# youngers2006/Dreamer

Measured on AMD Instinct MI355X. Metric: imagined latent-steps/sec (B×H) at 64×64 CarRacing, 1/2/4/8 MI355X, higher is better.
Workload: dtype f32; 1 GPU; Dreamer.train_Agent() with AC_epochs=1 (replay sample + warm start S/2 + H-step imagination + actor-critic update), B=256/GPU S=64 H=15 64x64x3, precision=fp32 (north-star batch per GPU); global_batch=256, seq_len=64, horizon=15, parallelism=dp1, precision=fp32

## Files before the change

dreamer_amd/_lib.py:

```python
import ctypes as C
import os

import torch

_HERE = os.path.dirname(os.path.abspath(__file__))
LIB_PATH = os.path.join(_HERE, "libdreamer_hip.so")
if os.environ.get("DREAMER_LIB_VARIANT"):
    LIB_PATH = os.path.join(os.path.dirname(_HERE), "tools", "variants",
                            f"libdreamer_hip_{os.environ['DREAMER_LIB_VARIANT']}.so")

fp = C.c_void_p


class dr_linear(C.Structure):
    _fields_ = [("w", fp), ("b", fp)]


class dr_mlp3(C.Structure):
    _fields_ = [("l0", dr_linear), ("n1", dr_linear), ("l3", dr_linear), ("n4", dr_linear), ("l6", dr_linear)]


DR_DISAG_MAX_MEMBERS = 16


class dr_ensemble(C.Structure):
    _fields_ = [("K", C.c_int), ("W", C.c_int), ("m", dr_mlp3 * DR_DISAG_MAX_MEMBERS)]


class dr_dims(C.Structure):
    _fields_ = [(n, C.c_int) for n in (
        "hidden", "rows", "cols", "action", "img_h", "img_w", "enc_f1", "enc_f2", "enc_hidden",
        "prior_h1", "prior_h2", "rew_h1", "rew_h2", "cont_h1", "cont_h2",
        "actor_h1", "actor_h2", "critic_h1", "critic_h2", "buckets", "dec_f1", "dec_f2", "dec_hidden", "precision", "obs_dim", "enc_depth",
        "launch_form")] + [("fault", fp), ("fault_host", fp)]

DR_MAX_DEPTH = 5


class dr_world_model(C.Structure):
    _fields_ = [("conv", dr_linear * DR_MAX_DEPTH), ("map0", dr_linear), ("map1", dr_linear), ("map3", dr_linear),
                ("w_ih", fp), ("w_hh", fp), ("b_ih", fp), ("b_hh", fp),
                ("prior", dr_mlp3), ("reward", dr_mlp3), ("cont", dr_mlp3), ("buckets_rew", fp)]


class dr_decoder(C.Structure):
    _fields_ = [("up0", dr_linear), ("up1", dr_linear), ("up3", dr_linear), ("convt", dr_linear * DR_MAX_DEPTH)]


class dr_wm_batch(C.Structure):
    _fields_ = [("actions", fp), ("act_sb", C.c_longlong), ("act_st", C.c_longlong), ("rewards", fp),
                ("continues", fp), ("rc_sb", C.c_longlong), ("rc_st", C.c_longlong)]


class dr_wm_loss_cfg(C.Structure):
    _fields_ = [("beta_pred", C.c_float), ("beta_dyn", C.c_float), ("beta_rep", C.c_float)]


class dr_actor(C.Structure):
    _fields_ = [("l0", dr_linear), ("n1", dr_linear), ("l3", dr_linear), ("n4", dr_linear),
                ("mu", dr_linear), ("ls", dr_linear)]


class dr_critic(C.Structure):
    _fields_ = [("net", dr_mlp3), ("buckets", fp)]


class dr_noise(C.Structure):
    _fields_ = [("q", fp), ("eps", fp), ("rng", fp), ("row0", C.c_int), ("stream", C.c_int)]


class dr_frames(C.Structure):
    _fields_ = [("ring", fp), ("ring_cap", C.c_longlong), ("starts", fp), ("obs", fp),
                ("stride_b", C.c_longlong), ("stride_t", C.c_longlong), ("raw255", C.c_int), ("t0", C.c_int)]


class dr_dream_outputs(C.Structure):
    _fields_ = [(n, fp) for n in (
        "R_lambda", "R_mc", "adv", "adv_norm", "weight", "logp", "base_entropy", "saturated",
        "reward_mean", "reward_std", "ret_mean", "ret_std", "logp_mean", "logp_std", "alive", "action_spread",
        "best", "worst", "n_finite")]


_P = C.POINTER
_sz = C.c_size_t
_i = C.c_int
_ll = C.c_longlong
_f = C.c_float
_d = C.c_double

_SIGS = {
    "dr_last_error": (C.c_char_p, []),
    "dr_version": (_i, []),
    "dr_encoder_workspace_bytes": (_sz, [_P(dr_dims), _i]),
    "dr_encoder_features": (_i, [_P(dr_dims), _P(dr_world_model), _P(dr_frames), _i, _i, fp, fp, _sz, fp]),
    "dr_observe_workspace_bytes": (_sz, [_P(dr_dims), _i]),
    "dr_observe_scan": (_i, [_P(dr_dims), _P(dr_world_model), _i, _i, fp, fp, _ll, _ll, fp, fp, dr_noise,
                             fp, fp, fp, fp, _sz, fp]),
    "dr_observe_trace_workspace_bytes": (_sz, [_P(dr_dims), _i, _i]),
    "dr_observe_trace": (_i, [_P(dr_dims), _P(dr_world_model), _i, _i, fp, fp, _ll, _ll, fp, fp, dr_noise,
                              fp, fp, fp, fp, fp, fp, fp, _sz, fp]),
    "dr_latent_stats": (_i, [_i, _i, _i, fp, fp, fp, fp, fp, fp, fp]),
    "dr_replay_returns": (_i, [_i, _i, fp, _ll, fp, _ll, _i, fp, _f, _f, fp, fp, fp, fp]),
    "dr_value_stats": (_i, [_i, _i, _i, _i, fp, _ll, fp, fp, fp, fp, fp, fp]),
    "dr_action_logprob": (_i, [_i, _i, _i, fp, fp, fp, _ll, _ll, fp, fp, fp, fp]),
    "dr_dream_stats": (_i, [_i, _i, _i, _i, fp, fp, fp, fp, fp, fp, fp, _f, _f, fp, _f, _P(dr_dream_outputs), fp]),
    "dr_actor_draws": (_i, [_i, _i, _i, dr_noise, fp, fp]),
    "dr_plan_sample": (_i, [_i, _i, _i, _i, _i, fp, fp, fp, dr_noise, fp, fp]),
    "dr_plan_update": (_i, [_i, _i, _i, _i, _i, fp, fp, fp, _f, _f, _f, _f, _f, fp, fp, fp, fp, fp, fp, fp, fp]),
    "dr_imagine_tape_bytes":(_sz, [_P(dr_dims), _i, _i]),
    "dr_imagine_workspace_bytes": (_sz, [_P(dr_dims), _i, _i]),
    "dr_imagine_fwd": (_i, [_P(dr_dims), _P(dr_world_model), _P(dr_actor), _i, _i, fp, fp, dr_noise, _i,
                            fp, fp, fp, fp, fp, fp, fp, fp, fp, _sz, fp]),
    "dr_imagine_actions_workspace_bytes": (_sz, [_P(dr_dims), _i, _i]),
    "dr_imagine_actions": (_i, [_P(dr_dims), _P(dr_world_model), _i, _i, fp, fp, fp, _ll, _ll, dr_noise,
                                fp, fp, fp, fp, fp, _sz, fp]),
    "dr_imagine_bwd": (_i, [_P(dr_dims), _P(dr_world_model), _P(dr_actor), _i, _i, fp, fp, fp, fp, fp,
                            fp, fp, fp, fp, _P(dr_actor), fp, _sz, fp]),
    "dr_imagine_bwd_prep": (_i, [_P(dr_dims), _P(dr_world_model), _P(dr_actor), _i, _i, fp, fp, fp, fp, _sz, fp]),
    "dr_imagine_bwd_main": (_i, [_P(dr_dims), _P(dr_world_model), _P(dr_actor), _i, _i, fp, fp, fp, fp, fp, _i,
                                 fp, _P(dr_actor), fp, _sz, fp]),
    "dr_step_workspace_bytes": (_sz, [_P(dr_dims), _i]),
    "dr_imagine_step": (_i, [_P(dr_dims), _P(dr_world_model), _i, fp, fp, fp, dr_noise, fp, fp, fp, fp,
                             fp, _sz, fp]),
    "dr_actor_act_workspace_bytes": (_sz, [_P(dr_dims), _i]),
    "dr_actor_act": (_i, [_P(dr_dims), _P(dr_actor), _i, fp, fp, dr_noise, _i, fp, fp, fp, fp, _sz, fp]),
    "dr_act_step_workspace_bytes": (_sz, [_P(dr_dims)]),
    "dr_act_step": (_i, [_P(dr_dims), _P(dr_world_model), _P(dr_actor), fp, _i, fp, fp, fp, dr_noise, _i,
                         fp, fp, fp, fp, fp, fp, fp, fp, _sz, fp]),
    "dr_act_batch_workspace_bytes": (_sz, [_P(dr_dims), _i]),
    "dr_act_batch": (_i, [_P(dr_dims), _P(dr_world_model), _P(dr_actor), _i, fp, fp, fp, fp, fp, dr_noise, _i,
                          fp, fp, fp, fp, fp, fp, fp, fp, _sz, fp]),
    "dr_act_vec_workspace_bytes": (_sz, [_P(dr_dims), _i]),
    "dr_act_vec": (_i, [_P(dr_dims), _P(dr_world_model), _P(dr_actor), _i, fp, fp, fp, fp, fp, dr_noise, _i,
                        fp, fp, fp, fp, fp, fp, fp, fp, _sz, fp]),
    "dr_gru_cell": (_i, [_P(dr_dims), _P(dr_world_model), _i, fp, fp, fp, fp, fp, _sz, fp]),
    "dr_categorical_sample": (_i, [_i, _i, _i, fp, dr_noise, fp, fp, fp, fp]),
    "dr_mlp3_fwd": (_i, [_P(dr_mlp3), _i, _i, fp, _ll, _i, fp, _ll, _i, _i, _i, fp, _ll, fp, _sz, fp]),
    "dr_bucket_value": (_i, [_i, _i, fp, fp, fp, fp]),
    "dr_critic_tape_bytes": (_sz, [_P(dr_dims), _i]),
    "dr_critic_workspace_bytes": (_sz, [_P(dr_dims), _i, _i]),
    "dr_critic_fwd": (_i, [_P(dr_dims), _P(dr_critic), _i, fp, _ll, fp, _ll, fp, fp, fp, fp, _sz, fp]),
    "dr_lambda_returns": (_i, [_i, _i, fp, fp, fp, _f, _f, fp, fp]),
    "dr_update_S": (_i, [_i, fp, fp, fp, fp, _sz, fp]),
    "dr_actor_loss_grad": (_i, [_i, _i, _i, fp, fp, fp, fp, fp, fp, _f, _f, fp, fp, fp, fp]),
    "dr_critic_loss_bwd": (_i, [_P(dr_dims), _P(dr_critic), _i, _i, fp, fp, fp, fp, _f, fp, _P(dr_critic),
                                fp, _sz, fp]),
    "dr_sqnorm": (_i, [_ll, fp, fp, fp]),
    "dr_sqnorm_multi": (_i, [_ll, fp, fp, fp, fp]),
    "dr_clip_stats": (_i, [_ll, fp, _ll, fp, _i, fp, fp, fp, fp, fp]),
    "dr_adamw": (_i, [_ll, fp, fp, fp, fp, fp, _f, _d, _d, _d, _d, _d, fp, fp, fp, fp]),
    "dr_ema": (_i, [_ll, fp, fp, _f, _f, fp, fp]),
    "dr_ac_optimiser_step": (_i, [_ll, fp, fp, fp, fp, fp, fp, _d, _d, _d, _d, _d,
                                  _ll, fp, fp, fp, fp, fp, fp, _d, _d, _d, _d, _d,
                                  _f, fp, _f, _f, _i, fp, fp, fp, fp, fp]),
    "dr_nonfinite": (_i, [_ll, fp, fp, fp]),
    "dr_replay_gather": (_i, [_ll, _i, _i, _i, _i, fp, fp, fp, fp, fp, fp, fp, fp, fp, fp]),
    "dr_replay_sample_workspace_bytes": (_sz, [_ll]),
    "dr_replay_sample": (_i, [_ll, _ll, _ll, _i, _i, fp, _d, fp, fp, _i, fp, fp, fp, _sz, fp]),
    "dr_replay_probabilities": (_i, [_ll, _ll, _ll, _i, fp, _d, fp, fp, _sz, fp]),
    "dr_replay_priority_update": (_i, [_ll, _i, fp, fp, _d, _d, _d, _d, _d, fp, fp, fp]),
    "dr_wm_window_scores": (_i, [_P(dr_dims), _i, _i, dr_wm_loss_cfg, fp, _sz, fp, fp]),
    "dr_disag_workspace_bytes": (_sz, [_i, _i, _i, _i, _i, _i]),
    "dr_disag_fwd": (_i, [_P(dr_ensemble), _i, _i, _i, fp, _ll, fp, fp, fp, _i, _i, _ll, _ll, _f, _f, fp, _sz, fp]),
    "dr_disag_train_grads": (_i, [_P(dr_ensemble), _i, _i, _i, fp, _ll, fp, _ll, _P(dr_ensemble), fp, fp, _sz, fp]),
    "dr_knn_workspace_bytes": (_sz, [_i, _i, _i, _i]),
    "dr_knn": (_i, [_i, _i, _i, fp, _ll, fp, _i, fp, _ll, fp, fp, fp, fp, _sz, fp]),
    "dr_state_entropy_fwd": (_i, [_i, _i, _i, fp, _ll, fp, _i, fp, _ll, fp, fp, fp, fp, fp, _i, _i, _ll, _ll, _f, _f,
                                  fp, _sz, fp]),
    "dr_rng_advance": (_i, [fp, C.c_ulonglong, fp]),
    "dr_persistent_kernels": (_i, [_P(dr_dims), _i, _i, _i]),
    "dr_stream_create_cumask": (_i, [_i, _P(C.c_uint), _P(fp)]),
    "dr_stream_destroy": (_i, [fp]),
    "dr_device_cus": (_i, [_P(_i)]),
    "dr_host_device_ptr": (_i, [fp, _P(fp)]),
    "dr_wm_train_workspace_bytes": (_sz, [_P(dr_dims), _i, _i]),
    "dr_decoder_workspace_bytes": (_sz, [_P(dr_dims), _i]),
    "dr_decoder_fwd": (_i, [_P(dr_dims), _P(dr_decoder), _i, fp, _ll, fp, _ll, fp, fp, _sz, fp]),
    "dr_frame_metrics": (_i, [_P(dr_dims), _i, _i, fp, _P(dr_frames), fp, fp, fp, fp]),
    "dr_frame_ssim": (_i, [_P(dr_dims), _i, _i, fp, _P(dr_frames), fp, fp, fp]),
    "dr_ensemble_metrics": (_i, [_P(dr_dims), _i, _i, _i, fp, _P(dr_frames), fp, fp, fp, fp, fp, fp]),
    "dr_occlude_workspace_bytes": (_sz, [_P(dr_dims), _i]),
    "dr_occlude_frames": (_i, [_P(dr_dims), _P(dr_frames), _i, _i, _i, fp, _i, fp, fp, fp, _sz, fp]),
    "dr_saliency_scores": (_i, [_i, _i, _i, _i, _i, fp, fp, fp, fp, fp, fp, fp, fp, fp, fp]),
    "dr_saliency_map": (_i, [_P(dr_dims), _i, _i, fp, fp, _P(dr_frames), _i, fp, fp, fp]),
    "dr_saliency_draws": (_i, [_i, _i, dr_noise, fp, fp]),
    "dr_wm_train_phase": (_i, [_P(dr_dims), _P(dr_world_model), _P(dr_decoder), _i, _i, _P(dr_frames),
                               _P(dr_wm_batch), dr_noise, dr_wm_loss_cfg, _i, fp, _i, fp, fp, _P(dr_world_model),
                               _P(dr_decoder), fp, fp, fp, fp, _sz, fp]),
    "dr_wm_train_grads": (_i, [_P(dr_dims), _P(dr_world_model), _P(dr_decoder), _i, _i, _P(dr_frames),
                               _P(dr_wm_batch), dr_noise, dr_wm_loss_cfg, fp, fp, _P(dr_world_model),
                               _P(dr_decoder), fp, fp, fp, fp, _sz, fp]),
}

EXPORTED = sorted(_SIGS)

_lib = None
_load_error = None


def load():
    global _lib, _load_error
    if _lib is not None:
        return _lib
    if not os.path.exists(LIB_PATH):
        _load_error = f"{LIB_PATH} not built (run: python -m dreamer_amd.build)"
        raise RuntimeError("dreamer_amd: HIP library missing: " + _load_error)
    lib = C.CDLL(LIB_PATH)
    for name, (res, args) in _SIGS.items():
        fn = getattr(lib, name)
        fn.restype = res
        fn.argtypes = args
    _lib = lib
    return lib


DR_E_INVALID, DR_E_HIP, DR_E_WORKSPACE, DR_E_UNSUPPORTED = 1001, 1002, 1003, 1004
DR_ACT_MAX_ENVS = 16
DR_ACT_VEC_MAX_OBS = 1023
DR_PLAN_MAX_CANDIDATES = 2048
DR_ENSEMBLE_MAX_SAMPLES = 64
DR_DREAM_STATS_MAX_DREAMS = 64
DR_DREAM_STATS_MAX_LDS_FLOATS = 15360
DR_KNN_MAX_K = 32
DR_PLAN_MAX_ELEMS = 1024
DR_SALIENCY_MAX_CELLS = 1024
DR_SALIENCY_MAX_RADIUS = 15


class HipError(RuntimeError):

    def __init__(self, name, code, msg):
        super().__init__(f"{name} failed ({code}): {msg}")
        self.code = code


def call(name, *args):
    lib = load()
    rc = getattr(lib, name)(*args)
    if rc != 0:
        msg = lib.dr_last_error().decode(errors="replace")
        raise HipError(name, rc, msg)


def query(name, *args):
    return getattr(load(), name)(*args)


def ptr(t):
    if t is None:
        return None
    if not t.is_cuda:
        raise RuntimeError("dreamer_amd: tensors must live on the GPU (this framework is MI355X-only)")
    return t.data_ptr()


def stream_ptr(device=None):
    return torch.cuda.current_stream(device).cuda_stream


def require_gpu(t):
    if not (isinstance(t, torch.Tensor) and t.is_cuda):
        raise RuntimeError("dreamer_amd: hot-path ops run only on the GPU (MI355X); "
                           "move the model and tensors to 'cuda'")
```

dreamer_amd/csrc/conv.h:

```cpp
#pragma once
#include "common.h"

extern thread_local const char* dr_conv_form_last;
const char* dr_conv_form(const char* fmt, ...);
#define DR_CONV_NOTE(...)                                  \
  do {                                                     \
    static const char* form_ = dr_conv_form(__VA_ARGS__);  \
    dr_conv_form_last = form_;                             \
  } while (0)

int op_conv_nhwc(int n, int cin, int ih, int iw, int cout, const float* in, const float* wr, const float* bias,
                 float* out, int out_nchw, hipStream_t s);
enum { CONV_EPI_FWD = 0, CONV_EPI_DSILU = 1 };
int op_conv_nhwc_ex(int n, int cin, int ih, int iw, int cout, const float* in, const float* wr, const float* bias,
                    float* out, int out_nchw, float* pre, int epi, hipStream_t s, float* csum = nullptr);
int op_frames_nhwc4(int n, int nb, int h, int w, const dr_frames* src, float* out, hipStream_t s, float pad = 0.0f);
int op_conv1_frames(int n, int nb, int ih, int iw, int cout, const dr_frames* src, const float* wr, const float* bias,
                    float* out, hipStream_t s);
int op_conv_repack_pad(int cout, int cin, int cin_pad, const float* w, float* wr, hipStream_t s);

int op_conv_repack_split3(int cout, int cin, const float* w, void* wr, hipStream_t s);
bool op_conv_split3_supported(int n, int cin, int ih, int iw, int cout);
int op_enc12_s1_bf16(int n, int nb, int h, int w, int c1, int c2, const dr_frames* src, const float* w1,
                     const float* b1, const float* w2, const float* b2, void* wr1, void* wr2, void* out,
                     hipStream_t s, int prepacked = 0);
int op_conv_s1_bf16(int n, int cin, int ih, int iw, int cout, const void* in, const void* wr, const float* bias,
                    void* out, int out_nchw, hipStream_t s);
bool op_conv_glds_bf16_supported(int n, int cin, int ih, int iw, int cout);
int op_conv_glds_s3(int n, int cin, int ih, int iw, int cout, const float* in, const void* wr, const float* bias,
                    float* out, int out_nchw, float* pre, int epi, hipStream_t s);
size_t op_gemm_nt_glds_part_floats(int M, int N, int K);
int op_gemm_nt_glds_bf16(int M, int N, int K, const void* X, int ldx, const void* W, int ldw, const float* bias,
                         float* Y, int ldy, float* part, size_t part_floats, hipStream_t s);
int op_conv_glds_bf16(int n, int cin, int ih, int iw, int cout, const void* in, const void* wr, const float* bias,
                      void* out, int out_nchw, hipStream_t s);
int op_conv_split3(int n, int cin, int ih, int iw, int cout, const float* in, const void* wr, const float* bias,
                   float* out, int out_nchw, hipStream_t s);
int op_conv_split3_ex(int n, int cin, int ih, int iw, int cout, const float* in, const void* wr, const float* bias,
                      float* out, int out_nchw, float* pre, int epi, hipStream_t s, int terms = 3);

size_t op_nt_split3_ws_bytes(int N, int K);
int op_nt_repack_split3(int N, int K, const float* W, int ldw, void* wr, hipStream_t s);
bool op_gemm_nt_split3_supported(int M, int N, int K, const float* A, int lda, const float* A2, int lda2, int ksA,
                                 int ldy);
int op_gemm_nt_split3(int M, int N, int K, const float* A, int lda, const float* A2, int lda2, int ksA, const void* wr,
                      const float* bias, int act, float* Y, int ldy, hipStream_t s);
size_t op_gemm_nt_split3_part_floats(int M, int N);
int op_gemm_nt_split3_sk(int M, int N, int K, const float* A, int lda, const float* A2, int lda2, int ksA,
                         const void* wr, const float* bias, int act, float* Y, int ldy, float* part,
                         size_t part_floats, hipStream_t s, int splits_fixed = 0);
int op_gemm_nt_split3_ex(int M, int N, int K, const float* A, int lda, const float* A2, int lda2, int ksA,
                         const void* wr, const float* bias, int act, float* Y, int ldy, int accumulate, float* Y2,
                         int ldy2, int nsplitY, float* part, size_t part_floats, hipStream_t s, int splits_fixed = 0);

int op_conv_repack_bf16(int cout, int cin, int cin_pad, const float* w, void* wr, hipStream_t s);
int op_to_bf16_2d(int rows, int cols, const float* x, long long ld, void* y, hipStream_t s);
int op_conv1_bf16(int n, int nb, int h, int w, int cout, const dr_frames* src, const void* wr, const float* bias,
                  void* out, hipStream_t s);
bool op_enc12_split3_ok(int n, int h, int w, int c1, int c2, const dr_frames* src);
int op_enc12_split3(int n, int nb, int h, int w, int c1, int c2, const dr_frames* src, const float* w1,
                    const float* b1, const float* w2, const float* b2, void* wr1, void* wr2, float* out,
                    hipStream_t s, int prepacked = 0);
int op_enc12_split3_ex(int n, int nb, int h, int w, int c1, int c2, const dr_frames* src, const float* w1,
                       const float* b1, const float* w2, const float* b2, void* wr1, void* wr2, float* out,
                       float* pre0, float* a0, float* pre1, hipStream_t s, int terms = 3, int prepacked = 0);
enum { RJ_CONV1 = 0, RJ_CONV = 1, RJ_NT = 2, RJ_BF16 = 3 };
struct RepackJob {
  int kind, a, b, c;
  const float* w;
  void* out;
  long long ld;
  long long total;
};
#define DR_RJ_MAX 6
RepackJob rj_conv1(int cout, const float* w, void* wr);
RepackJob rj_conv(int cout, int cin, const float* w, void* wr);
RepackJob rj_nt(int N, int K, const float* W, int ldw, void* wr);
RepackJob rj_bf16(int rows, int cols, const float* x, long long ld, void* y);
int op_repack_multi(const RepackJob* jobs, int n, hipStream_t s);
int op_enc12_bf16(int n, int nb, int h, int w, int c1, int c2, const dr_frames* src, const void* wr1, const float* b1,
                  const void* wr2, const float* b2, void* out, hipStream_t s);
int op_conv_bf16(int n, int cin, int ih, int iw, int cout, const void* in, const void* wr, const float* bias,
                 void* out, int out_nchw, hipStream_t s);
int op_gemm_nt_bf16(int M, int N, int K, const void* X, int ldx, const void* W, const float* bias, float* Y, int ldy,
                    hipStream_t s);

enum { CT_EPI_BIAS = 0, CT_EPI_DSILU = 1, CT_EPI_TANH_MSE = 2 };
struct ConvTArgs {
  int n, cin, h, w, cout;
  const float* in;
  int silu_in;
  const float* wq;
  const float* bias;
  float* out;
  float* out2;
  int silu_out;
  int ldc;
  const float* pre;
  const float* target;
  int tstride;
  const float* coef;
  float* part;
  float* bpart;
};
int op_convT_repack(int cin, int cout, const float* wt, float* wq, hipStream_t s);
int op_convT_nhwc(int epi, const ConvTArgs& a, hipStream_t s);
int op_convT_mse_parts(int h, int w);
int op_convT_out3_repack(int cin, const float* wt, float* wq, hipStream_t s);
int op_convT_out3(const ConvTArgs& a, hipStream_t s);
int op_convT_repack_split3(int cin, int cout, const float* wt, void* wr, hipStream_t s);
bool op_convT_split3_supported(int n, int cin, int h, int w, int cout, int terms = 3);
bool op_convT_cls_supported(int n, int cin, int h, int w, int cout);
int op_convT_split3(int epi, const ConvTArgs& a, const void* wr, hipStream_t s, int terms = 3);
bool op_convT_glds_s3_supported(const ConvTArgs& a, int epi);
int op_convT_glds_s3(int epi, const ConvTArgs& a, const void* wr, hipStream_t s);

size_t op_conv_wgrad_ws_floats(int n, int h, int w, int ca, int cb);
int op_wgrad_reduce(int ca, int cb, int cbo, int nsplit, const float* part, float* dw, float scale, int accumulate,
                    hipStream_t s);
bool op_wgrad_split3_supported(int n, int h, int w, int ca, int cb, int terms = 3);
size_t op_wgrad_split3_ws_floats(int n, int h, int w, int ca, int cb);
int op_wgrad_split3(int n, int h, int w, int ca, int cb, const float* lo, int lda, const float* hi, int ldb,
                    float* dw, int cbo, float scale, int accumulate, float* ws, size_t ws_floats, hipStream_t s,
                    int terms = 3);
int op_conv_wgrad(int n, int h, int w, int ca, int cb, const float* lo, int lda, int lo_silu, const float* hi, int ldb,
                  float* dw, int cbo, float scale, int accumulate, float* ws, size_t ws_floats, hipStream_t s,
                  float* bias_out = nullptr);
size_t op_chan_sum_ws_floats(long long rows, int C);
int op_chan_sum(long long rows, int C, const float* X, int ldx, float* out, int accumulate, float* ws, size_t ws_floats,
                hipStream_t s);
int op_chan_sum_final(int nb, int C, const float* part, float* out, int accumulate, hipStream_t s);

size_t op_gemm_tn_split3_ws_bytes(int M, int N, int K);
bool op_gemm_tn_split3_supported(int M, int N, int K);
int op_gemm_tn_split3(int M, int N, int K, const float* G, long long ldg, const float* X, long long ldx,
                      const float* X2, long long ldx2, int nsplitB, float* Y, long long ldy, int accumulate, void* ws,
                      size_t ws_bytes, hipStream_t s, int terms = 3);
struct TnProblem {
  int M, N, K;
  const float* G;
  long long ldg;
  const float* X;
  long long ldx;
  const float* X2;
  long long ldx2;
  int nsplitB;
  float* Y;
  long long ldy;
  int accumulate;
};
size_t op_gemm_tn_split3_multi_ws_bytes(const TnProblem* p, int n);
int op_gemm_tn_split3_multi(const TnProblem* p, int n, void* ws, size_t ws_bytes, hipStream_t s, int terms);
```

dreamer_amd/csrc/conv_hook.hip:

```cpp
#include <cstdarg>
#include <cstdio>
#include <cstring>

#include "conv.h"

thread_local const char* dr_conv_form_last = nullptr;

const char* dr_conv_form(const char* fmt, ...) {
  char buf[96];
  va_list ap;
  va_start(ap, fmt);
  vsnprintf(buf, sizeof buf, fmt, ap);
  va_end(ap);
  return strdup(buf);
}

enum {
  CV_OP, CV_N, CV_CA, CV_CB, CV_H, CV_W, CV_EPI, CV_NCHW, CV_TERMS, CV_LDA, CV_LDB, CV_LDC, CV_TSTRIDE, CV_CBO,
  CV_SILU_IN, CV_SILU_OUT, CV_LO_SILU, CV_FLAGS, CV_ACC, CV_WS_FLOATS, CV_CIN_RAW, CV_COUNT
};
enum {
  COP_CONV, COP_CONV_S3, COP_CONVT, COP_CONVT_S3, COP_CONVT_OUT3, COP_WGRAD, COP_WGRAD_S3, COP_CHAN_SUM,
  COP_CHAN_SUM_FINAL
};
enum {
  CF_BIAS = 1, CF_PRE = 2, CF_CSUM = 4, CF_OUT2 = 8, CF_TARGET = 16, CF_COEF = 32, CF_PART = 64, CF_BPART = 128,
  CF_BIAS_OUT = 256, CF_NO_REPACK = 512, CF_WS = 1024
};
enum {
  CP_IN, CP_W, CP_WR, CP_BIAS, CP_OUT, CP_PRE, CP_CSUM, CP_OUT2, CP_TARGET, CP_COEF, CP_PART, CP_BPART, CP_WS, CP_HI,
  CP_BIAS_OUT, CP_COUNT
};
enum { CN_SCALE, CN_PAD, CN_COUNT };

extern "C" int dr_internal_conv_run(const int* v, const double* num, void* const* ptrs, void* stream,
                                    long long* ws_need, char* form, int form_cap, char* msg, int msg_cap) {
  hipStream_t s = (hipStream_t)stream;
  if (form && form_cap > 0) form[0] = 0;
  if (msg && msg_cap > 0) msg[0] = 0;
  if (!v) return DR_E_INVALID;
  const int op = v[CV_OP], n = v[CV_N], ca = v[CV_CA], cb = v[CV_CB], h = v[CV_H], w = v[CV_W], fl = v[CV_FLAGS];
  long long need = 0;
  if (op == COP_WGRAD) need = (long long)op_conv_wgrad_ws_floats(n, h, w, ca, cb);
  else if (op == COP_WGRAD_S3) need = (long long)op_wgrad_split3_ws_floats(n, h, w, ca, cb);
  else if (op == COP_CHAN_SUM) need = (long long)op_chan_sum_ws_floats(n, ca);
  if (ws_need) *ws_need = need;
  if (!ptrs) return DR_OK;
  auto P = [&](int slot, int flag) { return !flag || (fl & flag) ? (float*)ptrs[slot] : nullptr; };
  const float* in = P(CP_IN, 0);
  const float* wraw = P(CP_W, 0);
  float* wr = P(CP_WR, 0);
  float* out = P(CP_OUT, 0);
  const bool repack = !(fl & CF_NO_REPACK);
  const float scale = num ? (float)num[CN_SCALE] : 1.0f;
  const size_t ws_floats = (size_t)v[CV_WS_FLOATS];
  dr_conv_form_last = nullptr;
  int rc = DR_OK;
  ConvTArgs a = {};
  a.n = n; a.cin = ca; a.h = h; a.w = w; a.cout = cb;
  a.in = in; a.silu_in = v[CV_SILU_IN]; a.wq = wr; a.bias = P(CP_BIAS, CF_BIAS);
  a.out = out; a.out2 = P(CP_OUT2, CF_OUT2); a.silu_out = v[CV_SILU_OUT]; a.ldc = v[CV_LDC];
  a.pre = P(CP_PRE, CF_PRE); a.target = P(CP_TARGET, CF_TARGET); a.tstride = v[CV_TSTRIDE];
  a.coef = P(CP_COEF, CF_COEF); a.part = P(CP_PART, CF_PART); a.bpart = P(CP_BPART, CF_BPART);
  switch (op) {
    case COP_CONV:
      if (repack) rc = op_conv_repack_pad(cb, v[CV_CIN_RAW] > 0 ? v[CV_CIN_RAW] : ca, ca, wraw, wr, s);
      if (rc == DR_OK)
        rc = op_conv_nhwc_ex(n, ca, h, w, cb, in, wr, P(CP_BIAS, CF_BIAS), out, v[CV_NCHW], P(CP_PRE, CF_PRE), v[CV_EPI],
                             s, P(CP_CSUM, CF_CSUM));
      break;
    case COP_CONV_S3:
      if (repack) rc = op_conv_repack_split3(cb, ca, wraw, wr, s);
      if (rc == DR_OK)
        rc = op_conv_split3_ex(n, ca, h, w, cb, in, wr, P(CP_BIAS, CF_BIAS), out, v[CV_NCHW], P(CP_PRE, CF_PRE),
                               v[CV_EPI], s, v[CV_TERMS]);
      break;
    case COP_CONVT:
      if (repack) rc = op_convT_repack(ca, cb, wraw, wr, s);
      if (rc == DR_OK) rc = op_convT_nhwc(v[CV_EPI], a, s);
      break;
    case COP_CONVT_S3:
      if (repack) rc = op_convT_repack_split3(ca, cb, wraw, wr, s);
      if (rc == DR_OK) rc = op_convT_split3(v[CV_EPI], a, wr, s, v[CV_TERMS]);
      break;
    case COP_CONVT_OUT3:
      if (repack) rc = op_convT_out3_repack(ca, wraw, wr, s);
      if (rc == DR_OK) rc = op_convT_out3(a, s);
      break;
    case COP_WGRAD:
      rc = op_conv_wgrad(n, h, w, ca, cb, in, v[CV_LDA], v[CV_LO_SILU], P(CP_HI, 0), v[CV_LDB], out, v[CV_CBO], scale,
                         v[CV_ACC], P(CP_WS, CF_WS), ws_floats, s, P(CP_BIAS_OUT, CF_BIAS_OUT));
      break;
    case COP_WGRAD_S3:
      rc = op_wgrad_split3(n, h, w, ca, cb, in, v[CV_LDA], P(CP_HI, 0), v[CV_LDB], out, v[CV_CBO], scale, v[CV_ACC],
                           P(CP_WS, CF_WS), ws_floats, s, v[CV_TERMS]);
      break;
    case COP_CHAN_SUM:
      rc = op_chan_sum(n, ca, in, v[CV_LDA], out, v[CV_ACC], P(CP_WS, CF_WS), ws_floats, s);
      break;
    case COP_CHAN_SUM_FINAL:
      rc = op_chan_sum_final(n, ca, in, out, v[CV_ACC], s);
      break;
    default:
      dr_set_error("dr_internal_conv_run: unknown op %d", op);
      rc = DR_E_INVALID;
  }
  if (form && form_cap > 0 && dr_conv_form_last) snprintf(form, form_cap, "%s", dr_conv_form_last);
  if (rc != DR_OK && msg && msg_cap > 0) snprintf(msg, msg_cap, "%s", dr_last_error());
  return rc;
}
```

dreamer_amd/csrc/conv_split.hip:

```cpp
#include "conv.h"

#include <algorithm>
#include <climits>
#include <type_traits>

namespace {
typedef unsigned short u16;
typedef __bf16 bf16x8 __attribute__((ext_vector_type(8)));
typedef unsigned u32x4 __attribute__((ext_vector_type(4)));
typedef unsigned u32x2 __attribute__((ext_vector_type(2)));

__device__ __forceinline__ f32x4 mfma_b16(u32x4 a, u32x4 b, f32x4 c) {
  return __builtin_amdgcn_mfma_f32_16x16x32_bf16(__builtin_bit_cast(bf16x8, a), __builtin_bit_cast(bf16x8, b), c, 0, 0,
                                                  0);
}
__device__ __forceinline__ unsigned b16bits(__bf16 v) { return (unsigned)__builtin_bit_cast(u16, v); }
__device__ __forceinline__ void split3(float x, unsigned& h, unsigned& m, unsigned& l) {
  const __bf16 bh = (__bf16)x;
  const float r1 = x - (float)bh;
  const __bf16 bm = (__bf16)r1;
  const float r2 = r1 - (float)bm;
  h = b16bits(bh);
  m = b16bits(bm);
  l = b16bits((__bf16)r2);
// ... 1821 lines not shown
  const int n = (int)(i / (KC * 32)), k = (int)(i - (long long)n * KC * 32);
  unsigned hh = 0, mm = 0, ll = 0;
  if (n < N && k < K) split3(W[(long long)n * ldw + k], hh, mm, ll);
  const long long plane = (long long)Np * 32;
  const long long base = ((long long)(k >> 5) * 3 * Np + n) * 32 + (k & 31);
  wr[base] = (u16)hh;
  wr[base + plane] = (u16)mm;
  wr[base + 2 * plane] = (u16)ll;
}
__global__ void k_nt_repack_split3(int N, int K, int Np, const float* __restrict__ W, int ldw, u16* __restrict__ wr) {
  const long long i = (long long)blockIdx.x * blockDim.x + threadIdx.x;
  if (i >= (long long)((K + 31) / 32) * 32 * Np) return;
  nt_repack_split3_elem(i, N, K, Np, W, ldw, wr);
}

struct RepackBatch {
  RepackJob j[DR_RJ_MAX];
  int blk0[DR_RJ_MAX + 1];
  int n;
};
__global__ __launch_bounds__(256) void k_repack_multi(RepackBatch b) {
  __shared__ __attribute__((aligned(16))) RepackJob J;
  int z = 0;
#pragma unroll
  for (int i = 1; i < DR_RJ_MAX; ++i)
    if ((int)blockIdx.x >= b.blk0[i]) z = i;
  dr_stage_args(b.j[z], J, threadIdx.x);
  const long long i = (long long)(blockIdx.x - b.blk0[z]) * 256 + threadIdx.x;
  if (i >= J.total) return;
  u16* out = static_cast<u16*>(J.out);
  switch (J.kind) {
    case RJ_CONV1: conv1_repack_split3_elem((int)i, J.a, J.w, out); break;
    case RJ_CONV: conv_repack_split3_elem((int)i, J.a, J.b, J.w, out); break;
    case RJ_NT: nt_repack_split3_elem(i, J.a, J.b, J.c, J.w, J.ld, out); break;
    default: {
      const int rr = (int)(i / J.b), cc = (int)(i - (long long)rr * J.b);
      out[i] = __builtin_bit_cast(u16, (__bf16)J.w[(long long)rr * J.ld + cc]);
    }
  }
}

RepackJob rj_conv1(int cout, const float* w, void* wr) { return {RJ_CONV1, cout, 0, 0, w, wr, 0, (long long)cout * 64}; }
RepackJob rj_conv(int cout, int cin, const float* w, void* wr) {
  return {RJ_CONV, cout, cin, 0, w, wr, 0, (long long)cout * 16 * cin};
}
RepackJob rj_nt(int N, int K, const float* W, int ldw, void* wr) {
  const int Np = (N + 127) / 128 * 128;
  return {RJ_NT, N, K, Np, W, wr, ldw, (long long)((K + 31) / 32) * 32 * Np};
}
RepackJob rj_bf16(int rows, int cols, const float* x, long long ld, void* y) {
  return {RJ_BF16, rows, cols, 0, x, y, ld, (long long)rows * cols};
}

int op_repack_multi(const RepackJob* jobs, int n, hipStream_t s) {
  if (n < 0 || n > DR_RJ_MAX) {
    dr_set_error("repack_multi: %d jobs (at most %d)", n, DR_RJ_MAX);
    return DR_E_INVALID;
  }
  if (n == 0) return DR_OK;
  RepackBatch b = {};
  int tot = 0;
  for (int i = 0; i < DR_RJ_MAX; ++i) {
    b.blk0[i] = tot;
    if (i < n) {
      b.j[i] = jobs[i];
      tot += (int)((jobs[i].total + 255) / 256);
    }
  }
  b.blk0[DR_RJ_MAX] = tot;
  b.n = n;
  hipLaunchKernelGGL(k_repack_multi, dim3((unsigned)tot), dim3(256), 0, s, b);
  return dr_check_launch("repack_multi");
}

static int s3_np(int N) { return (N + 127) / 128 * 128; }
size_t op_nt_split3_ws_bytes(int N, int K) {
  return (size_t)((K + 31) / 32) * 32 * 3 * s3_np(N) * sizeof(u16);
}
int op_nt_repack_split3(int N, int K, const float* W, int ldw, void* wr, hipStream_t s) {
  const int Np = s3_np(N);
  const long long total = (long long)((K + 31) / 32) * 32 * Np;
  hipLaunchKernelGGL(k_nt_repack_split3, dim3((unsigned)((total + 255) / 256)), dim3(256), 0, s, N, K, Np, W, ldw,
                     (u16*)wr);
  return dr_check_launch("nt_repack_split3");
}
bool op_gemm_nt_split3_supported(int M, int N, int K, const float* A, int lda, const float* A2, int lda2, int ksA,
                                 int ldy) {
  const bool seg = ksA < K;
  return M > 0 && N > 0 && N % 4 == 0 && ldy % 4 == 0 && K % 4 == 0 && lda % 4 == 0 && !((uintptr_t)A & 15) &&
         (!seg || (ksA % 4 == 0 && lda2 % 4 == 0 && A2 && !((uintptr_t)A2 & 15))) &&
         (long long)M * lda < (1LL << 31) && (!seg || (long long)M * lda2 < (1LL << 31));
}
size_t op_gemm_nt_split3_part_floats(int M, int N) { return (size_t)DR_S3_SPLITS * M * N; }

int op_gemm_nt_split3(int M, int N, int K, const float* A, int lda, const float* A2, int lda2, int ksA, const void* wr,
                      const float* bias, int act, float* Y, int ldy, hipStream_t s) {
  return op_gemm_nt_split3_sk(M, N, K, A, lda, A2, lda2, ksA, wr, bias, act, Y, ldy, nullptr, 0, s);
}

int op_gemm_nt_split3_sk(int M, int N, int K, const float* A, int lda, const float* A2, int lda2, int ksA,
                         const void* wr, const float* bias, int act, float* Y, int ldy, float* part,
                         size_t part_floats, hipStream_t s, int splits_fixed) {
  return op_gemm_nt_split3_ex(M, N, K, A, lda, A2, lda2, ksA, wr, bias, act, Y, ldy, 0, nullptr, 0, INT_MAX, part,
                              part_floats, s, splits_fixed);
}

int op_gemm_nt_split3_ex(int M, int N, int K, const float* A, int lda, const float* A2, int lda2, int ksA,
                         const void* wr, const float* bias, int act, float* Y, int ldy, int accumulate, float* Y2,
                         int ldy2, int nsplitY, float* part, size_t part_floats, hipStream_t s, int splits_fixed) {
  const bool y2 = nsplitY < N;
  if (!op_gemm_nt_split3_supported(M, N, K, A, lda, A2, lda2, ksA, ldy) || ((uintptr_t)Y & 15) ||
      (bias && ((uintptr_t)bias & 15)) || ((uintptr_t)part & 15) || splits_fixed < 0 ||
      splits_fixed > DR_S3_SPLITS || (splits_fixed > 1 && (!part || (size_t)splits_fixed * M * N > part_floats)) ||
      (y2 && (!Y2 || ((uintptr_t)Y2 & 15) || ldy2 % 4 || nsplitY % 4 || nsplitY < 0))) {
    dr_set_error("gemm_nt_split3: unsupported problem (M=%d N=%d K=%d)", M, N, K);
    return DR_E_INVALID;
  }
  GemmS3 g = {M, N, K, ksA < K ? ksA : K, lda, lda2, ldy, act, s3_np(N), A, A2, (const u16*)wr, bias, Y, 1, part,
              accumulate ? 1 : 0, ldy2, y2 ? nsplitY : INT_MAX, 0, Y2};
  auto tl = [&](int bm, int bn) { return ((M + bm - 1) / bm) * ((N + bn - 1) / bn); };
  auto waves = [&](int bm, int bn) { return (long long)tl(bm, bn) * (bm / 32); };
  const int nch = (K + 31) / 32;
  auto splits_for = [&](int bm, int bn) {
    if (splits_fixed > 0) return splits_fixed;
    int sp = 1;
    while (part && sp < DR_S3_SPLITS && waves(bm, bn) * sp < 2048 && nch / (2 * sp) >= 8 &&
           (size_t)(2 * sp) * M * N <= part_floats)
      sp *= 2;
    return sp;
  };
  const int shapes[5][2] = {{256, 128}, {256, 64}, {128, 128}, {128, 64}, {64, 64}};
  int pick = 4;
  for (int c = 0; c < 5; ++c) {
    if (waves(shapes[c][0], shapes[c][1]) * splits_for(shapes[c][0], shapes[c][1]) >= 2048) {
      pick = c;
      break;
    }
  }
  g.splits = splits_for(shapes[pick][0], shapes[pick][1]);
  const unsigned gy = (unsigned)g.splits;
  switch (pick) {
    case 0: hipLaunchKernelGGL((k_gemm_split3<256, 128>), dim3(dr_xcd_grid(tl(256, 128)), gy), dim3(512), 0, s, g); break;
    case 1: hipLaunchKernelGGL((k_gemm_split3<256, 64>), dim3(dr_xcd_grid(tl(256, 64)), gy), dim3(512), 0, s, g); break;
    case 2: hipLaunchKernelGGL((k_gemm_split3<128, 128>), dim3(dr_xcd_grid(tl(128, 128)), gy), dim3(256), 0, s, g); break;
    case 3: hipLaunchKernelGGL((k_gemm_split3<128, 64>), dim3(dr_xcd_grid(tl(128, 64)), gy), dim3(256), 0, s, g); break;
    default: hipLaunchKernelGGL((k_gemm_split3<64, 64>), dim3(dr_xcd_grid(tl(64, 64)), gy), dim3(128), 0, s, g); break;
  }
  DR_TRY(dr_check_launch("gemm_nt_split3"));
  if (g.splits > 1) {
    hipLaunchKernelGGL(k_s3_finish, dim3((unsigned)(((long long)M * (N / 4) + 255) / 256)), dim3(256), 0, s, g);
    DR_TRY(dr_check_launch("s3_finish"));
  }
  return DR_OK;
}

static int s3_pad(int n) { return (n + 127) / 128 * 128; }

struct KnRepack {
  int K, N, P, nsplit;
  const float* X;
  const float* X2;
  long long ldx, ldx2;
  u16* wr;
  long long pad_;
};

template <int TERMS>
__device__ __forceinline__ void kn_repack_body(int K, int N, int P, const float* __restrict__ X, long long ldx,
                                               const float* __restrict__ X2, long long ldx2, int nsplit,
                                               u16* __restrict__ wr) {
  const int n = blockIdx.x * 256 + threadIdx.x, kc = blockIdx.y;
  if (n >= P) return;
  const bool seg2 = n >= nsplit;
  const float* src = seg2 ? X2 : X;
  const long long ld = seg2 ? ldx2 : ldx;
  const int nn = seg2 ? n - nsplit : n;
  float v[32];
  const bool nok = n < N;
  const float* col = src + (nok ? nn : 0);
#pragma unroll
  for (int k = 0; k < 32; ++k) {
    const int kk = 32 * kc + k;
    const bool ok = nok && kk < K;
    const float t = col[ok ? (long long)kk * ld : 0LL];
    v[k] = ok ? t : 0.f;
  }
  u32x4* o = reinterpret_cast<u32x4*>(wr + (((long long)kc * 3) * P + n) * 32);
  if constexpr (TERMS == 1) {
#pragma unroll
    for (int u = 0; u < 4; ++u) {
      u32x4 h;
#pragma unroll
      for (int e = 0; e < 4; ++e) h[e] = pack_bf16x2(v[8 * u + 2 * e], v[8 * u + 2 * e + 1]);
      o[u] = h;
    }
    return;
  }
  u32x4 h[4], m[4], l[4];
#pragma unroll
  for (int u = 0; u < 4; ++u)
#pragma unroll
    for (int e = 0; e < 4; ++e) {
      unsigned hh, mm, ll;
      split3_pair(v[8 * u + 2 * e], v[8 * u + 2 * e + 1], hh, mm, ll);
      h[u][e] = hh;
      m[u][e] = mm;
      l[u][e] = ll;
    }
  const long long pl = (long long)P * 32 / 8;
#pragma unroll
  for (int u = 0; u < 4; ++u) {
    o[u] = h[u];
    o[pl + u] = m[u];
    o[2 * pl + u] = l[u];
  }
}

struct GemmPP {
  int M, N, K, Mp, Np, splits, accumulate, tiles;
  long long ldy;
  const u16* wa;
  const u16* wb;
  float* Y;
  float* part;
  long long pad_;
};

#define DR_TN_MAX 4
struct TnBatch {
  KnRepack r[2 * DR_TN_MAX];
  GemmPP g[DR_TN_MAX];
  int blk0[DR_TN_MAX + 1];
  int fin0[DR_TN_MAX + 1];
  int n, nrep, pad_[2];
};

template <int TERMS>
__global__ __launch_bounds__(256) void k_kn_repack_multi(TnBatch b) {
  __shared__ __attribute__((aligned(16))) KnRepack s;
  dr_stage_args(b.r[blockIdx.z], s, threadIdx.x);
  const int P = dr_uni(s.P), K = dr_uni(s.K);
  if ((int)blockIdx.x * 256 >= P || (int)blockIdx.y * 32 >= K) return;
  kn_repack_body<TERMS>(K, dr_uni(s.N), P, dr_uni(s.X), s.ldx, dr_uni(s.X2), s.ldx2, dr_uni(s.nsplit), dr_uni(s.wr));
}

__device__ __forceinline__ int tn_find(const int* blk0, int flat) {
  int z = 0;
#pragma unroll
  for (int i = 1; i < DR_TN_MAX; ++i)
    if (flat >= blk0[i]) z = i;
  return z;
}

template <int BM, int BN, int TERMS = 3>
__global__ __launch_bounds__(BM * 2) void k_gemm_pp_multi(TnBatch b) {
  constexpr int NT = BM * 2;
  constexpr int WTN = BN / 2, FM = 4, FN = WTN / 16;
  constexpr int AU = TERMS * BM * 4, BU = TERMS * BN * 4;
  constexpr int APT = (AU + NT - 1) / NT, BPT = (BU + NT - 1) / NT;
  static_assert(FN >= 1 && BM % 64 == 0 && (TERMS == 1 || TERMS == 3), "gemm_pp tile");
  __shared__ __attribute__((aligned(16))) u32x4 As[2][TERMS][BM][4];
  __shared__ __attribute__((aligned(16))) u32x4 Bs[2][TERMS][BN][4];
  __shared__ __attribute__((aligned(16))) GemmPP s_g;
  const int flat = dr_xcd_tile(blockIdx.x, b.blk0[DR_TN_MAX]);
  if (flat < 0) return;
  const int z = tn_find(b.blk0, flat);
  dr_stage_args(b.g[z], s_g, threadIdx.x);
  const int M = dr_uni(s_g.M), N = dr_uni(s_g.N), Mp = dr_uni(s_g.Mp), Np = dr_uni(s_g.Np);
  const int tiles = dr_uni(s_g.tiles), splits = dr_uni(s_g.splits);
  const int local = flat - b.blk0[z];
  const int split = local / tiles, lt = local - split * tiles;
  const int tiles_n = (N + BN - 1) / BN;
  const int m0 = (lt / tiles_n) * BM, n0 = (lt % tiles_n) * BN;
  const DR_GLOBAL u16* wa = dr_g(dr_uni(s_g.wa));
  const DR_GLOBAL u16* wb = dr_g(dr_uni(s_g.wb));
  const int tid = threadIdx.x, wave = tid >> 6, lane = tid & 63, r = lane & 15, q = lane >> 4;
  const int NCH = (dr_uni(s_g.K) + 31) / 32;
  const int per = (NCH + splits - 1) / splits;
  const int c0 = min(NCH, split * per), c1 = min(NCH, c0 + per);
  u32x4 ra0[APT], ra1[APT], rb0[BPT], rb1[BPT];
  auto load = [&](int c, auto slot) __attribute__((always_inline)) {
    u32x4* ra = decltype(slot)::value == 0 ? ra0 : ra1;
    u32x4* rb = decltype(slot)::value == 0 ? rb0 : rb1;
#pragma unroll
    for (int j = 0; j < APT; ++j) {
      const int e = tid + NT * j;
      if (AU % NT == 0 || e < AU) {
        const int pl = e / (BM * 4), rm = e - pl * BM * 4, row = rm >> 2, u = rm & 3;
        ra[j] = *reinterpret_cast<const DR_GLOBAL u32x4*>(wa + (((long long)c * 3 + pl) * Mp + m0 + row) * 32 + 8 * u);
      }
    }
#pragma unroll
    for (int j = 0; j < BPT; ++j) {
      const int e = tid + NT * j;
      if (BU % NT == 0 || e < BU) {
        const int pl = e / (BN * 4), rm = e - pl * BN * 4, row = rm >> 2, u = rm & 3;
        rb[j] = *reinterpret_cast<const DR_GLOBAL u32x4*>(wb + (((long long)c * 3 + pl) * Np + n0 + row) * 32 + 8 * u);
      }
    }
  };
  auto store = [&](auto slot, int buf) __attribute__((always_inline)) {
    const u32x4* ra = decltype(slot)::value == 0 ? ra0 : ra1;
    const u32x4* rb = decltype(slot)::value == 0 ? rb0 : rb1;
#pragma unroll
    for (int j = 0; j < APT; ++j) {
      const int e = tid + NT * j;
// ... 211 lines not shown
```

dreamer_amd/csrc/engine.hip:

```cpp
#include "engine_util.h"
#include "scan.h"
#include "dream.h"
#include "bptt.h"


static bool s3_first_layer(const dr_dims* d, int M, int N, const float* h, long long ldh, const float* z,
                           long long ldz) {
  return d->precision != DR_PREC_BF16 && M >= 1024 && ldh < INT_MAX && ldz < INT_MAX &&
         op_gemm_nt_split3_supported(M, N, d->hidden + latent(d), h, (int)ldh, z, (int)ldz, d->hidden, N);
}

struct EncWs {
  float *x0, *a[DR_MAX_DEPTH], *wr[DR_MAX_DEPTH], *sk;
  long long sk_n;
  void* wproj;
  void* s3proj;
  float* s3part;
  size_t s3part_n;
};

static void enc_carve(Carve& c, const dr_dims* d, int n, EncWs& w) {
  memset(&w, 0, sizeof(w));
  if (d->obs_dim > 0) {
    const int F = enc_feat_dim(d);
// ... 415 lines not shown
  w.wst = c.f((long long)2 * A * d->actor_h2);
  w.bst = c.f((long long)2 * A);
  w.idx[0] = c.i(2 * Bl * d->rows);
  w.idx[1] = c.i(2 * Bl * d->rows);
  w.tl6p = c.f((long long)L * d->prior_h2);
  w.tl3p = c.f((long long)d->prior_h2 * d->prior_h1);
  w.tl0p = c.f((long long)d->prior_h1 * Hd);
  w.twhh = c.f((long long)3 * Hd * Hd);
  w.thead = c.f((long long)2 * A * d->actor_h2);
  w.tl3a = c.f((long long)d->actor_h2 * d->actor_h1);
  w.tl0a = c.f((long long)d->actor_h1 * (Hd + L));
  w.gH = c.f(B1 * Hd);
  w.gZ = c.f(B1 * L);
  w.gA = c.f(BH * A);
  w.glog = c.f(Bl * L);
  w.gx2 = c.f(Bl * d->prior_h2);
  w.gp2 = c.f(Bl * d->prior_h2);
  w.gx1 = c.f(Bl * d->prior_h1);
  w.gp1 = c.f(Bl * d->prior_h1);
  w.ggi = c.f(Bl * 3 * Hd);
  w.ggh = c.f(Bl * 3 * Hd);
  w.ggi16 = (unsigned short*)c.raw(sizeof(unsigned short) * Bl * 3 * Hd);
  w.ggh16 = (unsigned short*)c.raw(sizeof(unsigned short) * Bl * 3 * Hd);
  w.gheads = c.f(BH * 2 * A);
  w.gx2a = c.f(Bl * d->actor_h2);
  w.gpre2a = c.f(BH * d->actor_h2);
  w.gy2a = c.f(BH * d->actor_h2);
  w.xh2a = c.f(BH * d->actor_h2);
  w.gx1a = c.f(Bl * d->actor_h1);
  w.gpre1a = c.f(BH * d->actor_h1);
  w.gpre1a16 = (unsigned short*)c.raw(sizeof(unsigned short) * BH * d->actor_h1);
  w.gy1a = c.f(BH * d->actor_h1);
  w.xh1a = c.f(BH * d->actor_h1);
  w.hcat = c.f(BH * Hd);
  w.zcat = c.f(BH * L);
  w.sk_n = splitk_floats(d->actor_h1, Hd + L) + splitk_floats(d->actor_h2, d->actor_h1) +
           2 * splitk_floats(A, d->actor_h2);
  w.sk = c.f(w.sk_n);
  const int BHi = (int)BH;
  w.tn_bytes = op_gemm_tn_split3_ws_bytes(d->actor_h1, Hd + L, BHi) +
               op_gemm_tn_split3_ws_bytes(d->actor_h2, d->actor_h1, BHi) +
               2 * op_gemm_tn_split3_ws_bytes(A, d->actor_h2, BHi);
  w.tn = c.raw(w.tn_bytes);
  w.pd = c.raw(op_pdream_ws_bytes(d, B, H));
  w.pb = c.raw(op_pbptt_ws_bytes(d, B, H));
}

extern "C" size_t dr_imagine_workspace_bytes(const dr_dims* d, int B, int H) {
  Carve c(nullptr);
  ImWs w;
  imws_carve(c, d, B, H, w);
  return c.off;
}

static int imagine_heads(const dr_dims* d, const dr_world_model* wm, int B, int H, const float* latents,
                         const float* hiddens, float* rewards, float* continues, ImWs& w, hipStream_t s,
                         bool keep0 = false);

static int imagine_launch_form(const dr_dims* d, const dr_world_model* wm, const dr_actor* ac, int B, int H,
                               const dr_noise& noise, const dr_noise& nq, int deterministic, float* latents,
                               float* hiddens, float* actions, float* mus, float* sigmas, const Tape& tp, ImWs& w,
                               bool split_gru, bool zg, hipStream_t s) {
  const int L = latent(d), Hd = d->hidden, A = d->action, a1 = d->actor_h1, a2 = d->actor_h2;
  const long long ldH = (long long)(H + 1) * Hd, ldL = (long long)(H + 1) * L, ldA = (long long)H * A;
  const long long lda1 = (long long)H * a1, lda2 = (long long)H * a2;
  const bool planes = split_gru && H > 1 && Hd % 8 == 0;
  const bool a16 = planes && d->precision == DR_PREC_BF16;
  if (planes) {
    DR_TRY(split_planes(d->prior_h1, Hd, wm->prior.l0.w, Hd, w.s3p0, s));
    if (zg) DR_TRY(split_planes(a1, Hd, ac->l0.w, Hd + L, w.s3a0, s));
    DR_TRY(split_planes(3 * Hd, Hd, wm->w_hh, Hd, w.s3whh, s));
  }

  {
    DR_TRY(run(G_NT, AM_PLAIN, lin2(B, a1, hiddens, ldH, Hd, latents, ldL, L, ac->l0.w, ac->l0.b, tp.pre1a, lda1), s));
    GemmArgs g = lin_ln(B, a2, a1, tp.pre1a, lda1, ac->n1, ac->l3.w, ac->l3.b, tp.pre2a, lda2);
    g.a_out = tp.x1a; g.ld_aout = lda1;
    DR_TRY(run(G_NT, AM_LNSILU, g, s));
  }
  DR_TRY(stack_heads(ac, A, a2, w.wst, w.bst, s));
  {
    GemmArgs h = lin_ln(B, 2 * A, a2, tp.pre2a, lda2, ac->n4, w.wst, w.bst, nullptr, 0);
    h.a_out = tp.x2a; h.ld_aout = lda2;
    with_actor_head(h, A, noise, 0, deterministic, actions, ldA, mus, ldA, sigmas, ldA, tp.eps, tp.ls_raw, ldA);
    DR_TRY(run(G_NT, AM_LNSILU, h, s));
  }
  for (int t = 0; t < H; ++t) {
    const long long hb = (long long)Hd * B * t;
    float* h_t = hiddens + (long long)t * Hd;
    float* h_n = hiddens + (long long)(t + 1) * Hd;
    float* z_t = latents + (long long)t * L;
    float* z_n = latents + (long long)(t + 1) * L;
    unsigned short* h_n16 = a16 ? w.hid16 + (long long)(t + 1) * Hd : nullptr;
    DR_TRY(gru_onehot(d, wm, B, w.idx[t & 1], actions + (long long)t * A, ldA, h_t, ldH, h_n, ldH, w.wt,
                      tp.r + hb, tp.u + hb, tp.n + hb, tp.ghn + hb, s, z_t, ldL, w.gh, split_gru && t > 0, h_n16));
    float* p1 = tp.pre1p + (long long)t * B * d->prior_h1;
    float* p2 = tp.pre2p + (long long)t * B * d->prior_h2;
    {
      const bool more = t + 1 < H;
      GemmArgs p[3];
      int np = 0;
      p[np] = lin(B, d->prior_h1, Hd, h_n, ldH, wm->prior.l0.w, Hd, wm->prior.l0.b, p1, d->prior_h1);
      if (planes) wplanes(p[np], w.s3p0);
      ++np;
      if (more && zg) {
        p[np] = lin(B, a1, Hd, h_n, ldH, ac->l0.w, Hd + L, ac->l0.b, w.hpart, a1);
        if (planes) wplanes(p[np], w.s3a0);
        ++np;
      }
      if (more && split_gru) {
        p[np] = lin(B, 3 * Hd, Hd, h_n, ldH, wm->w_hh, Hd, wm->b_hh, w.gh, 3 * Hd);
        if (planes) wplanes(p[np], w.s3whh);
        ++np;
      }
      for (int i = 0; i < np; ++i) {
        if (!planes) p[i].bf16 = 0;
        p[i].A16 = h_n16;
      }
      DR_TRY(gemm_launch(G_NT, AM_PLAIN, p, np, s));
    }
    DR_TRY(run(G_NT, AM_LNSILU, lin_ln(B, d->prior_h2, d->prior_h1, p1, d->prior_h1, wm->prior.n1, wm->prior.l3.w,
                                       wm->prior.l3.b, p2, d->prior_h2), s));
    GemmArgs g = lin_ln(B, L, d->prior_h2, p2, d->prior_h2, wm->prior.n4, wm->prior.l6.w, wm->prior.l6.b, nullptr, 0);
    with_sampler(g, d, nq, t, z_n, ldL, w.idx[(t + 1) & 1], tp.soft + (long long)t * B * L, L);
    DR_TRY(run(G_NT, AM_LNSILU, g, s));
    if (t + 1 < H) {
      const long long o1 = (long long)(t + 1) * a1, o2 = (long long)(t + 1) * a2, o = (long long)(t + 1) * A;
      if (zg) {
        int* ix = w.idx[(t + 1) & 1];
        DR_TRY(op_zgather_add(B, a1, d->rows, d->cols, ix, onehot_vals(ix, B, d->rows), z_n, ldL,
                              w.tl0f + (long long)Hd * a1, a1, w.hpart, a1, tp.pre1a + o1, lda1, s));
      } else {
        DR_TRY(run(G_NT, AM_PLAIN, lin2(B, a1, h_n, ldH, Hd, z_n, ldL, L, ac->l0.w, ac->l0.b, tp.pre1a + o1, lda1), s));
      }
      GemmArgs g3 = lin_ln(B, a2, a1, tp.pre1a + o1, lda1, ac->n1, ac->l3.w, ac->l3.b, tp.pre2a + o2, lda2);
      g3.a_out = tp.x1a + o1;
      g3.ld_aout = lda1;
      DR_TRY(run(G_NT, AM_LNSILU, g3, s));
      GemmArgs hd = lin_ln(B, 2 * A, a2, tp.pre2a + o2, lda2, ac->n4, w.wst, w.bst, nullptr, 0);
      hd.a_out = tp.x2a + o2;
      hd.ld_aout = lda2;
      with_actor_head(hd, A, noise, t + 1, deterministic, actions + o, ldA, mus + o, ldA, sigmas + o, ldA,
                      tp.eps + (long long)(t + 1) * B * A, tp.ls_raw + o, ldA);
      DR_TRY(run(G_NT, AM_LNSILU, hd, s));
    }
  }
  return DR_OK;
}

extern "C" int dr_imagine_fwd(const dr_dims* d, const dr_world_model* wm, const dr_actor* ac, int B, int H,
                              const float* z0, const float* h0, dr_noise noise, int deterministic, float* latents,
                              float* hiddens, float* actions, float* rewards, float* continues, float* mus,
                              float* sigmas, void* tape, void* ws, size_t ws_bytes, hipStream_t s) {
  DR_REQUIRE(d && wm && ac && z0 && h0 && latents && hiddens && actions && rewards && continues && mus && sigmas &&
                 tape && B > 0 && H > 0,
             "null argument or empty batch");
  DR_TRY(dims_envelope(__func__, d, ENV_GRU | ENV_SAMPLER | ENV_ACTOR));
  GemmBf16Scope bf16_scope(d->precision == DR_PREC_BF16);
  Carve c(ws);
  ImWs w;
  imws_carve(c, d, B, H, w);
  WS_CHECK(c, ws_bytes);
  Carve ct(tape);
  Tape tp;
  tape_carve(ct, d, B, H, tp);
  const int L = latent(d), Hd = d->hidden, A = d->action, a1 = d->actor_h1, a2 = d->actor_h2;
  const long long ldH = (long long)(H + 1) * Hd, ldL = (long long)(H + 1) * L, ldA = (long long)H * A;
  const long long lda1 = (long long)H * a1, lda2 = (long long)H * a2;
  {
    const Copy2dJob cj[2] = {{latents, ldL, z0, L, L, B}, {hiddens, ldH, h0, Hd, Hd, B}};
    DR_TRY(op_copy2d_multi(cj, 2, s));
  }
  dr_noise nq = noise;
  nq.stream += 65536;
  const bool split_gru = B >= 128;
  const bool zg = d->rows <= 32 && a1 % 4 == 0;
  {
    TransposeJob tj[2] = {{3 * Hd, L + A, 3 * Hd, wm->w_ih, w.wt}, {a1, Hd + L, a1, ac->l0.w, w.tl0f}};
    DR_TRY(op_transpose_multi(tj, zg ? 2 : 1, s));
  }
  DR_TRY(op_onehot_index(B, d->rows, d->cols, latents, ldL, w.idx[0], onehot_vals(w.idx[0], B, d->rows), s));

  bool unrolled = false;
  if (zg && op_pdream_supported(d, B, H, A)) {
    const PDreamTape pt = {tp.eps, tp.ls_raw, tp.pre1a, tp.x1a, tp.pre2a, tp.x2a, tp.r, tp.u, tp.n, tp.ghn,
                           tp.pre1p, tp.pre2p, tp.soft};
    const int rc = op_pdream(d, wm, ac, B, H, w.wt, w.tl0f + (long long)Hd * a1, w.idx[0], noise, nq, deterministic,
                             latents, hiddens, actions, mus, sigmas, pt, w.pd, s);
    if (rc != DR_E_UNSUPPORTED && rc != DR_OK) return rc;
    unrolled = rc == DR_OK;
  }
  if (!unrolled) DR_TRY(imagine_launch_form(d, wm, ac, B, H, noise, nq, deterministic, latents, hiddens, actions, mus,
                                            sigmas, tp, w, split_gru, zg, s));
  return imagine_heads(d, wm, B, H, latents, hiddens, rewards, continues, w, s);
}

static int imagine_heads(const dr_dims* d, const dr_world_model* wm, int B, int H, const float* latents,
                         const float* hiddens, float* rewards, float* continues, ImWs& w, hipStream_t s, bool keep0) {
  const int L = latent(d), Hd = d->hidden;
  {
    const int M1 = B * (H + 1);
    GemmArgs p[2];
    if (s3_first_layer(d, M1, d->rew_h1, hiddens, Hd, latents, L) &&
        s3_first_layer(d, M1, d->cont_h1, hiddens, Hd, latents, L)) {
      DR_TRY(op_nt_repack_split3(d->rew_h1, Hd + L, wm->reward.l0.w, Hd + L, w.s3r, s));
      DR_TRY(op_nt_repack_split3(d->cont_h1, Hd + L, wm->cont.l0.w, Hd + L, w.s3c, s));
      DR_TRY(op_gemm_nt_split3_sk(M1, d->rew_h1, Hd + L, hiddens, Hd, latents, L, Hd, w.s3r, wm->reward.l0.b, 0,
                                  w.p1r, d->rew_h1, w.s3part, w.s3part_n, s));
      DR_TRY(op_gemm_nt_split3_sk(M1, d->cont_h1, Hd + L, hiddens, Hd, latents, L, Hd, w.s3c, wm->cont.l0.b, 0,
                                  w.p1c, d->cont_h1, w.s3part, w.s3part_n, s));
    } else {
      p[0] = lin2(M1, d->rew_h1, hiddens, Hd, Hd, latents, L, L, wm->reward.l0.w, wm->reward.l0.b, w.p1r, d->rew_h1);
      p[1] = lin2(M1, d->cont_h1, hiddens, Hd, Hd, latents, L, L, wm->cont.l0.w, wm->cont.l0.b, w.p1c, d->cont_h1);
      DR_TRY(gemm_launch(G_NT, AM_PLAIN, p, 2, s));
    }
    p[0] = lin_ln(M1, d->buckets, d->rew_h2, w.p2r, d->rew_h2, wm->reward.n4, wm->reward.l6.w, wm->reward.l6.b, w.rlog,
                  d->buckets);
    p[1] = lin_ln(M1, 1, d->cont_h2, w.p2c, d->cont_h2, wm->cont.n4, wm->cont.l6.w, wm->cont.l6.b, w.clog, 1);
    p[1].act = 2;
    Mlp2Args m2[2];
    {
      const float* x1[2] = {w.p1r, w.p1c};
      const dr_mlp3* hm[2] = {&wm->reward, &wm->cont};
      const int k1[2] = {d->rew_h1, d->cont_h1}, k2[2] = {d->rew_h2, d->cont_h2};
      for (int i = 0; i < 2; ++i) {
        memset(&m2[i], 0, sizeof(Mlp2Args));
        m2[i].M = M1; m2[i].K1 = k1[i]; m2[i].K2 = k2[i];
        m2[i].X = x1[i]; m2[i].ldx = k1[i];
        m2[i].ln1_g = hm[i]->n1.w; m2[i].ln1_b = hm[i]->n1.b;
        m2[i].W3 = hm[i]->l3.w; m2[i].b3 = hm[i]->l3.b;
        m2[i].ln4_g = hm[i]->n4.w; m2[i].ln4_b = hm[i]->n4.b;
        m2[i].e = p[i];
        m2[i].e.A = nullptr;
      }
    }
    if (mlp2_ok(m2[0]) && mlp2_ok(m2[1])) {
      DR_TRY(mlp2_launch(m2, 2, s));
    } else {
      GemmArgs q[2];
      q[0] = lin_ln(M1, d->rew_h2, d->rew_h1, w.p1r, d->rew_h1, wm->reward.n1, wm->reward.l3.w, wm->reward.l3.b, w.p2r,
                    d->rew_h2);
      q[1] = lin_ln(M1, d->cont_h2, d->cont_h1, w.p1c, d->cont_h1, wm->cont.n1, wm->cont.l3.w, wm->cont.l3.b, w.p2c,
                    d->cont_h2);
      DR_TRY(gemm_launch(G_NT, AM_LNSILU, q, 2, s));
      DR_TRY(gemm_launch(G_NT, AM_LNSILU, p, 2, s));
    }
    DR_TRY(op_bucket_value(M1, d->buckets, w.rlog, d->buckets, wm->buckets_rew, w.rval, 1, s));
    const int k0 = keep0 ? 0 : 1, Ho = H + 1 - k0;
    const Copy2dJob cj[2] = {{rewards, Ho, w.rval + k0, H + 1, Ho, B}, {continues, Ho, w.clog + k0, H + 1, Ho, B}};
    DR_TRY(op_copy2d_multi(cj, 2, s));
  }
  return DR_OK;
}

struct ImActWs {
  ImWs w;
  float *p1, *p2;
};
static void imact_carve(Carve& c, const dr_dims* d, int B, int H, ImActWs& a) {
  const long long Bl = B, B1 = (long long)B * (H + 1);
  const int L = latent(d), Hd = d->hidden, A = d->action;
  ImWs& w = a.w;
  memset(&w, 0, sizeof(w));
  w.gh = c.f(Bl * 3 * Hd);
  w.wt = c.f((long long)(L + A) * 3 * Hd);
  w.hid16 = (unsigned short*)c.raw(sizeof(unsigned short) * B1 * Hd);
  w.s3p0 = c.raw(op_nt_split3_ws_bytes(d->prior_h1, Hd));
  w.s3whh = c.raw(op_nt_split3_ws_bytes(3 * Hd, Hd));
  w.idx[0] = c.i(2 * Bl * d->rows);
  w.idx[1] = c.i(2 * Bl * d->rows);
  a.p1 = c.f(Bl * d->prior_h1);
  a.p2 = c.f(Bl * d->prior_h2);
  w.p1r = c.f(B1 * d->rew_h1);
  w.p1c = c.f(B1 * d->cont_h1);
  w.p2r = c.f(B1 * d->rew_h2);
  w.p2c = c.f(B1 * d->cont_h2);
  w.rlog = c.f(B1 * d->buckets);
  w.clog = c.f(B1);
  w.rval = c.f(B1);
  w.s3r = c.raw(op_nt_split3_ws_bytes(d->rew_h1, Hd + L));
  w.s3c = c.raw(op_nt_split3_ws_bytes(d->cont_h1, Hd + L));
  w.s3part_n = op_gemm_nt_split3_part_floats((int)B1, std::max(d->rew_h1, d->cont_h1));
  w.s3part = c.f((long long)w.s3part_n);
}

extern "C" size_t dr_imagine_actions_workspace_bytes(const dr_dims* d, int B, int H) {
  if (!d || B <= 0 || H <= 0) return 0;
  Carve c(nullptr);
  ImActWs a;
  imact_carve(c, d, B, H, a);
  return c.off;
}

extern "C" int dr_imagine_actions(const dr_dims* d, const dr_world_model* wm, int B, int H, const float* z0,
                                  const float* h0, const float* actions, long long act_sb, long long act_st,
                                  dr_noise noise, float* latents, float* hiddens, float* rewards, float* continues,
                                  void* ws, size_t ws_bytes, hipStream_t s) {
  DR_REQUIRE(d && wm && z0 && h0 && actions && latents && hiddens && rewards && continues && ws && B > 0 && H > 0,
             "null argument or empty batch");
  DR_REQUIRE(wm->w_ih && wm->w_hh && wm->b_ih && wm->b_hh, "GRU weights required");
  DR_TRY(dims_envelope(__func__, d, ENV_GRU | ENV_SAMPLER));
  GemmBf16Scope bf16_scope(d->precision == DR_PREC_BF16);
  Carve c(ws);
  ImActWs a;
  imact_carve(c, d, B, H, a);
  WS_CHECK(c, ws_bytes);
  ImWs& w = a.w;
  const int L = latent(d), Hd = d->hidden, A = d->action;
  const long long ldH = (long long)(H + 1) * Hd, ldL = (long long)(H + 1) * L;
  {
    const Copy2dJob cj[2] = {{latents, ldL, z0, L, L, B}, {hiddens, ldH, h0, Hd, Hd, B}};
    DR_TRY(op_copy2d_multi(cj, 2, s));
  }
  const bool split_gru = B >= 128;
  const bool planes = split_gru && H > 1 && Hd % 8 == 0;
  const bool a16 = planes && d->precision == DR_PREC_BF16;
  DR_TRY(op_transpose(3 * Hd, L + A, wm->w_ih, w.wt, s));
  DR_TRY(op_onehot_index(B, d->rows, d->cols, latents, ldL, w.idx[0], onehot_vals(w.idx[0], B, d->rows), s));
  if (planes) {
    DR_TRY(split_planes(d->prior_h1, Hd, wm->prior.l0.w, Hd, w.s3p0, s));
    DR_TRY(split_planes(3 * Hd, Hd, wm->w_hh, Hd, w.s3whh, s));
  }
  for (int t = 0; t < H; ++t) {
    float* h_t = hiddens + (long long)t * Hd;
    float* h_n = hiddens + (long long)(t + 1) * Hd;
    float* z_t = latents + (long long)t * L;
    float* z_n = latents + (long long)(t + 1) * L;
    unsigned short* h_n16 = a16 ? w.hid16 + (long long)(t + 1) * Hd : nullptr;
    DR_TRY(gru_onehot(d, wm, B, w.idx[t & 1], actions + (long long)t * act_st, act_sb, h_t, ldH, h_n, ldH, w.wt,
                      nullptr, nullptr, nullptr, nullptr, s, z_t, ldL, w.gh, split_gru && t > 0, h_n16));
    {
      GemmArgs p[2];
      int np = 0;
      p[np] = lin(B, d->prior_h1, Hd, h_n, ldH, wm->prior.l0.w, Hd, wm->prior.l0.b, a.p1, d->prior_h1);
      if (planes) wplanes(p[np], w.s3p0);
      ++np;
      if (t + 1 < H && split_gru) {
        p[np] = lin(B, 3 * Hd, Hd, h_n, ldH, wm->w_hh, Hd, wm->b_hh, w.gh, 3 * Hd);
        if (planes) wplanes(p[np], w.s3whh);
        ++np;
      }
      for (int i = 0; i < np; ++i) {
        if (!planes) p[i].bf16 = 0;
        p[i].A16 = h_n16;
      }
      DR_TRY(gemm_launch(G_NT, AM_PLAIN, p, np, s));
    }
    DR_TRY(run(G_NT, AM_LNSILU, lin_ln(B, d->prior_h2, d->prior_h1, a.p1, d->prior_h1, wm->prior.n1, wm->prior.l3.w,
                                       wm->prior.l3.b, a.p2, d->prior_h2), s));
    GemmArgs g = lin_ln(B, L, d->prior_h2, a.p2, d->prior_h2, wm->prior.n4, wm->prior.l6.w, wm->prior.l6.b, nullptr, 0);
    with_sampler(g, d, noise, t, z_n, ldL, w.idx[(t + 1) & 1], nullptr, 0);
    DR_TRY(run(G_NT, AM_LNSILU, g, s));
  }
  return imagine_heads(d, wm, B, H, latents, hiddens, rewards, continues, w, s);
}

static int imagine_bwd_impl(const dr_dims* d, const dr_world_model* wm, const dr_actor* ac, int B, int H,
                            const float* latents, const float* hiddens, const float* actions,
                            const float* g_mus, const float* g_sigmas,
                            const float* g_actions, const float* g_latents, const float* g_hiddens,
                            const void* tape, const dr_actor* gr, void* ws, size_t ws_bytes, hipStream_t s,
                            bool do_prep, bool do_main);

extern "C" int dr_imagine_bwd(const dr_dims* d, const dr_world_model* wm, const dr_actor* ac, int B, int H,
                              const float* latents, const float* hiddens, const float* actions,
                              const float* g_mus, const float* g_sigmas,
                              const float* g_actions, const float* g_latents, const float* g_hiddens,
                              const void* tape, const dr_actor* gr, void* ws, size_t ws_bytes, hipStream_t s) {
// ... 70 lines not shown
      DR_TRY(split_planes(Hd, 3 * Hd, w.twhh, 3 * Hd, w.s3twhh, s));
      if (d->actor_h1 % 8 == 0) DR_TRY(split_planes(Hd + L, d->actor_h1, w.tl0a, d->actor_h1, w.s3tl0a, s));
    }
  }
  }
  const bool planes = B >= 128 && (3 * Hd) % 8 == 0;
  if (!do_main) return DR_OK;

  bool looped = false;
  if (op_pbptt_supported(d, B, H, A)) {
    const PBpttIO io = {w.tl6p, w.tl3p, w.tl0p, w.wt, w.twhh, w.thead, w.tl3a, w.tl0a,
                        tp.soft, tp.pre2p, tp.pre1p, tp.r, tp.u, tp.n, tp.ghn, tp.pre2a, tp.pre1a, tp.ls_raw, tp.eps,
                        hiddens, actions, g_mus, g_sigmas, w.gH, w.gZ, w.gA,
                        w.gheads, w.gpre2a, w.gy2a, w.xh2a, w.gpre1a, w.gy1a, w.xh1a};
    const int rc = op_pbptt(d, wm, ac, B, H, io, w.pb, s);
    if (rc != DR_E_UNSUPPORTED && rc != DR_OK) return rc;
    looped = rc == DR_OK;
  }
  for (int t = H - 1; t >= 0 && !looped; --t) {
    const long long hb = (long long)Hd * B * t;
    float* gH_t = w.gH + (long long)t * Hd;
    float* gH_n = w.gH + (long long)(t + 1) * Hd;
    float* gZ_t = w.gZ + (long long)t * L;
    float* gZ_n = w.gZ + (long long)(t + 1) * L;
    const bool state_grad = upstream_state || t < H - 1;
    if (state_grad) {
      const int h1 = d->prior_h1, h2 = d->prior_h2;
      GemmArgs g = bwd_nt(B, h2, L, gZ_n, ldL, w.tl6p, w.gx2, h2, 0);
      g.pre = tp.soft + (long long)t * B * L;
      g.ld_pre = L;
      g.C = d->cols;
      const GemmPlan pl = gemm_plan(G_NT, AM_STEBWD, &g, 1);
      if (gemm_bwd_fusable(pl)) {
        DR_TRY(gemm_run(pl, &g, 1, s));
      } else {
        DR_TRY(op_softmax_ste_bwd(B, d->rows, d->cols, gZ_n, ldL, tp.soft + (long long)t * B * L, L, w.glog, s));
        DR_TRY(run(G_NT, AM_PLAIN, bwd_nt(B, h2, L, w.glog, L, w.tl6p, w.gx2, h2, 0), s));
      }
      DR_TRY(lnbwd_nt(B, h1, h2, w.gx2, h2, tp.pre2p + (long long)t * B * h2, h2, wm->prior.n4, w.tl3p, w.gx1, h1, 0,
                      w.gp2, h2, nullptr, nullptr, nullptr, 0, INT_MAX, s));
      GruBwdEpi ge;
      memset(&ge, 0, sizeof(ge));
      ge.h = hiddens + (long long)t * Hd; ge.ldh = ldH;
      ge.r = tp.r + hb; ge.u = tp.u + hb; ge.n = tp.n + hb; ge.ghn = tp.ghn + hb;
      ge.gi = w.ggi; ge.gh = w.ggh; ge.ho = gH_t; ge.ldo = ldH; ge.Hd = Hd;
      const bool a16 = planes && d->precision == DR_PREC_BF16;
      if (a16) {
        ge.gi16 = w.ggi16;
        ge.gh16 = w.ggh16;
      }
      DR_TRY(lnbwd_nt(B, Hd, h1, w.gx1, h1, tp.pre1p + (long long)t * B * h1, h1, wm->prior.n1, w.tl0p, gH_n, ldH, 1,
                      w.gp1, h1, nullptr, nullptr, nullptr, 0, INT_MAX, s, &ge));
      if (t > 0) {
        GemmArgs p[2];
        p[0] = bwd_nt(B, L + A, 3 * Hd, w.ggi, 3 * Hd, w.wt, gZ_t, ldL, 1);
        p[0].Y2 = w.gA + (long long)t * A; p[0].ldy2 = ldA; p[0].nsplitY = L;
        p[1] = bwd_nt(B, Hd, 3 * Hd, w.ggh, 3 * Hd, w.twhh, gH_t, ldH, 1);
        if (planes) {
          wplanes(p[0], w.s3wt);
          wplanes(p[1], w.s3twhh);
        }
        if (a16) {
          p[0].A16 = w.ggi16;
          p[1].A16 = w.ggh16;
        }
        DR_TRY(gemm_launch(G_NT, AM_PLAIN, p, 2, s));
      } else {
        DR_TRY(run(G_NT, AM_PLAIN, bwd_nt(B, A, 3 * Hd, w.ggi, 3 * Hd, w.wt + (long long)L * 3 * Hd, w.gA, ldA, 1), s));
      }
    }
    const long long ot = (long long)t * A;
    float* gh_t = w.gheads + (long long)t * 2 * A;
    const long long o2 = (long long)t * a2, o1 = (long long)t * a1;
    DR_TRY(op_actor_head_bwd_x(B, A, a2, w.gA + ot, ldA, g_mus ? g_mus + ot : nullptr,
                               g_sigmas ? g_sigmas + ot : nullptr, ldA, actions + ot, ldA, tp.ls_raw + ot, ldA,
                               tp.eps + (long long)t * B * A, gh_t, (long long)H * 2 * A, w.thead, w.gx2a, a2, s));
    DR_TRY(lnbwd_nt(B, a1, a2, w.gx2a, a2, tp.pre2a + o2, lda2, ac->n4, w.tl3a, w.gx1a, a1, 0, w.gpre2a + o2, lda2,
                    w.gy2a + o2, w.xh2a + o2, nullptr, 0, INT_MAX, s));
    if (t > 0 && planes && a1 % 8 == 0) {
      const bool a16 = d->precision == DR_PREC_BF16 && lda1 % 8 == 0;
      DR_TRY(op_ln_silu_bwd(B, a1, w.gx1a, a1, tp.pre1a + o1, lda1, ac->n1.w, ac->n1.b, w.gpre1a + o1, lda1,
                            w.gy1a + o1, w.xh1a + o1, s, a16 ? w.gpre1a16 + o1 : nullptr));
      GemmArgs g = bwd_nt(B, Hd + L, a1, w.gpre1a + o1, lda1, w.tl0a, gH_t, ldH, 1);
      if (a16) g.A16 = w.gpre1a16 + o1;
      g.Y2 = gZ_t; g.ldy2 = ldL; g.nsplitY = Hd;
      wplanes(g, w.s3tl0a);
      DR_TRY(run(G_NT, AM_PLAIN, g, s));
    } else if (t > 0) {
      DR_TRY(lnbwd_nt(B, Hd + L, a1, w.gx1a, a1, tp.pre1a + o1, lda1, ac->n1, w.tl0a, gH_t, ldH, 1, w.gpre1a + o1,
                      lda1, w.gy1a + o1, w.xh1a + o1, gZ_t, ldL, Hd, s));
    } else {
      DR_TRY(op_ln_silu_bwd(B, a1, w.gx1a, a1, tp.pre1a + o1, lda1, ac->n1.w, ac->n1.b, w.gpre1a + o1, lda1,
                            w.gy1a + o1, w.xh1a + o1, s));
    }
  }
  {
    const Copy2dJob cj[2] = {{w.hcat, (long long)H * Hd, hiddens, ldH, (long long)H * Hd, B},
                             {w.zcat, (long long)H * L, latents, ldL, (long long)H * L, B}};
    DR_TRY(op_copy2d_multi(cj, 2, s));
  }
  {
    GemmArgs p[4];
    p[0] = bwd_w(a1, Hd + L, BH, w.gpre1a, a1, w.hcat, Hd, gr->l0.w);
    p[0].W2 = w.zcat; p[0].ldb2 = L; p[0].nsplitB = Hd;
    p[1] = bwd_w(a2, a1, BH, w.gpre2a, a2, tp.x1a, a1, gr->l3.w);
    p[2] = bwd_w(A, a2, BH, w.gheads, 2 * A, tp.x2a, a2, gr->mu.w);
    p[3] = bwd_w(A, a2, BH, w.gheads + A, 2 * A, tp.x2a, a2, gr->ls.w);
    float* sk = w.sk;
    long long skn = w.sk_n;
    for (int i = 0; i < 4; ++i) give_splitk(p[i], sk, skn);
    DR_TRY(tn_launch(p, 4, w.tn, w.tn_bytes, s, d->precision == DR_PREC_BF16 ? 1 : 3));
  }
  {
    ColsumJob cj[8] = {
        {a1, w.gpre1a, a1, nullptr, 0, gr->l0.b}, {a1, w.gy1a, a1, w.xh1a, a1, gr->n1.w},
        {a1, w.gy1a, a1, nullptr, 0, gr->n1.b},   {a2, w.gpre2a, a2, nullptr, 0, gr->l3.b},
        {a2, w.gy2a, a2, w.xh2a, a2, gr->n4.w},   {a2, w.gy2a, a2, nullptr, 0, gr->n4.b},
        {A, w.gheads, 2 * A, nullptr, 0, gr->mu.b}, {A, w.gheads + A, 2 * A, nullptr, 0, gr->ls.b},
    };
    DR_TRY(op_colsum_multi(BH, cj, 8, s));
  }
  return DR_OK;
}

struct CTape {
  float *pre1, *x1, *pre2, *x2, *logits;
};
static void ctape_carve(Carve& c, const dr_dims* d, int M, CTape& t) {
  t.pre1 = c.f((long long)M * d->critic_h1);
  t.x1 = c.f((long long)M * d->critic_h1);
  t.pre2 = c.f((long long)M * d->critic_h2);
  t.x2 = c.f((long long)M * d->critic_h2);
  t.logits = c.f((long long)M * d->buckets);
}

extern "C" size_t dr_critic_tape_bytes(const dr_dims* d, int M) {
  Carve c(nullptr);
  CTape t;
  ctape_carve(c, d, M, t);
  return c.off;
}

static size_t critic_ws_bytes(const dr_dims* d, int M) {
  Carve c(nullptr);
  CTape t;
  ctape_carve(c, d, M, t);
  c.f(splitk_floats(M, d->critic_h1));
  c.raw(op_nt_split3_ws_bytes(d->critic_h1, d->hidden + latent(d)));
  c.f((long long)op_gemm_nt_split3_part_floats(M, d->critic_h1));
  return c.off + 256;
}


extern "C" int dr_critic_fwd(const dr_dims* d, const dr_critic* cr, int M, const float* h, long long ldh,
                             const float* z, long long ldz, float* logits, float* values, void* tape, void* ws,
                             size_t ws_bytes, hipStream_t s) {
  DR_REQUIRE(d && cr && h && z && M > 0, "null argument or empty batch");
  GemmBf16Scope bf16_scope(d->precision == DR_PREC_BF16);
  CTape t;
  float* sk = nullptr;
  long long skn = 0;
  void* s3w = nullptr;
  float* s3part = nullptr;
  size_t s3part_n = 0;
  if (tape) {
    Carve c(tape);
    ctape_carve(c, d, M, t);
  }
  if (ws) {
    Carve c(ws);
    CTape tw;
    ctape_carve(c, d, M, tw);
    if (!tape) {
      t = tw;
      WS_CHECK(c, ws_bytes);
    }
    const long long want = splitk_floats(M, d->critic_h1);
    if (c.off + (size_t)want * sizeof(float) + 256 <= ws_bytes) {
      skn = want;
      sk = c.f(skn);
      const size_t pb = op_nt_split3_ws_bytes(d->critic_h1, d->hidden + latent(d));
      if (c.off + pb + 256 <= ws_bytes) s3w = c.raw(pb);
      const size_t pn = op_gemm_nt_split3_part_floats(M, d->critic_h1);
      if (s3w && c.off + pn * sizeof(float) + 256 <= ws_bytes) {
        s3part = c.f((long long)pn);
        s3part_n = pn;
      }
    }
  }
  DR_REQUIRE(tape || ws, "dr_critic_fwd needs a tape or a workspace");
  const int L = latent(d), Hd = d->hidden, c1 = d->critic_h1, c2 = d->critic_h2, nb = d->buckets;
  if (s3w && s3_first_layer(d, M, c1, h, ldh, z, ldz)) {
    DR_TRY(op_nt_repack_split3(c1, Hd + L, cr->net.l0.w, Hd + L, s3w, s));
    DR_TRY(op_gemm_nt_split3_sk(M, c1, Hd + L, h, (int)ldh, z, (int)ldz, Hd, s3w, cr->net.l0.b, 0, t.pre1, c1,
                                s3part, s3part_n, s));
  } else {
    GemmArgs g1 = lin2(M, c1, h, ldh, Hd, z, ldz, L, cr->net.l0.w, cr->net.l0.b, t.pre1, c1);
    give_splitk(g1, sk, skn);
    DR_TRY(run(G_NT, AM_PLAIN, g1, s));
  }
  GemmArgs g2 = lin_ln(M, c2, c1, t.pre1, c1, cr->net.n1, cr->net.l3.w, cr->net.l3.b, t.pre2, c2);
  g2.a_out = t.x1; g2.ld_aout = c1;
  DR_TRY(run(G_NT, AM_LNSILU, g2, s));
  float* lg = logits ? logits : t.logits;
  GemmArgs g3 = lin_ln(M, nb, c2, t.pre2, c2, cr->net.n4, cr->net.l6.w, cr->net.l6.b, lg, nb);
  g3.a_out = t.x2; g3.ld_aout = c2;
  DR_TRY(run(G_NT, AM_LNSILU, g3, s));
  if (tape && logits && logits != t.logits) DR_TRY(copy2d(t.logits, nb, logits, nb, nb, M, s));
  if (values) DR_TRY(op_bucket_value(M, nb, lg, nb, cr->buckets, values, 1, s));
  return DR_OK;
}

struct CBws {
  float *row_loss, *glog, *gx2, *gp2, *gy2, *xh2, *gx1, *gp1, *gy1, *xh1;
  float *tl6, *tl3;
  float* sk;
  long long sk_n;
  void* tn;
  size_t tn_bytes;
};
static void cbws_carve(Carve& c, const dr_dims* d, int B, int H, CBws& w) {
  const long long M = (long long)B * (H + 1);
  w.tn_bytes = op_gemm_tn_split3_ws_bytes(d->buckets, d->critic_h2, (int)M) +
               op_gemm_tn_split3_ws_bytes(d->critic_h2, d->critic_h1, (int)M) +
               op_gemm_tn_split3_ws_bytes(d->critic_h1, d->hidden + latent(d), (int)M);
  w.tn = c.raw(w.tn_bytes);
  w.row_loss = c.f((long long)B * H);
  w.sk_n = splitk_floats(d->buckets, d->critic_h2) + splitk_floats(d->critic_h2, d->critic_h1) +
           splitk_floats(d->critic_h1, d->hidden + latent(d));
  w.sk = c.f(w.sk_n);
  w.tl6 = c.f((long long)d->buckets * d->critic_h2);
  w.tl3 = c.f((long long)d->critic_h2 * d->critic_h1);
  w.glog = c.f(M * d->buckets);
  w.gx2 = c.f(M * d->critic_h2);
  w.gp2 = c.f(M * d->critic_h2);
  w.gy2 = c.f(M * d->critic_h2);
  w.xh2 = c.f(M * d->critic_h2);
  w.gx1 = c.f(M * d->critic_h1);
  w.gp1 = c.f(M * d->critic_h1);
  w.gy1 = c.f(M * d->critic_h1);
  w.xh1 = c.f(M * d->critic_h1);
}

extern "C" size_t dr_critic_workspace_bytes(const dr_dims* d, int B, int H) {
  Carve c(nullptr);
  CBws w;
  cbws_carve(c, d, B, H, w);
  const size_t a = c.off, b = critic_ws_bytes(d, B * (H + 1));
  return a > b ? a : b;
}

extern "C" int dr_critic_loss_bwd(const dr_dims* d, const dr_critic* cr, int B, int H, const float* hiddens,
                                  const float* latents, const float* R, const void* tape, float scale,
                                  float* loss_out, const dr_critic* gr, void* ws, size_t ws_bytes, hipStream_t s) {
  DR_REQUIRE(d && cr && hiddens && latents && R && tape && loss_out && gr && B > 0 && H > 0, "null argument");
  GemmBf16Scope bf16_scope(d->precision == DR_PREC_BF16);
  Carve c(ws);
  CBws w;
  cbws_carve(c, d, B, H, w);
  WS_CHECK(c, ws_bytes);
  const int M = B * (H + 1);
  Carve ct((void*)tape);
  CTape t;
  ctape_carve(ct, d, M, t);
  const int L = latent(d), Hd = d->hidden, c1 = d->critic_h1, c2 = d->critic_h2, nb = d->buckets;
  DR_TRY(op_critic_ce(B, H, nb, t.logits, R, cr->buckets, scale, w.row_loss, w.glog, s));
  DR_TRY(op_mean(B * H, w.row_loss, loss_out, s));
  {
    TransposeJob tj[2] = {{nb, c2, nb, cr->net.l6.w, w.tl6}, {c2, c1, c2, cr->net.l3.w, w.tl3}};
    DR_TRY(op_transpose_multi(tj, 2, s));
  }
  DR_TRY(run(G_NT, AM_PLAIN, bwd_nt(M, c2, nb, w.glog, nb, w.tl6, w.gx2, c2, 0), s));
  DR_TRY(lnbwd_nt(M, c1, c2, w.gx2, c2, t.pre2, c2, cr->net.n4, w.tl3, w.gx1, c1, 0, w.gp2, c2, w.gy2, w.xh2, nullptr,
                  0, INT_MAX, s));
  DR_TRY(op_ln_silu_bwd(M, c1, w.gx1, c1, t.pre1, c1, cr->net.n1.w, cr->net.n1.b, w.gp1, c1, w.gy1, w.xh1, s));
  {
    GemmArgs p[3];
    p[0] = bwd_w(nb, c2, M, w.glog, nb, t.x2, c2, gr->net.l6.w);
    p[1] = bwd_w(c2, c1, M, w.gp2, c2, t.x1, c1, gr->net.l3.w);
    p[2] = bwd_w(c1, Hd + L, M, w.gp1, c1, hiddens, Hd, gr->net.l0.w);
    p[2].W2 = latents; p[2].ldb2 = L; p[2].nsplitB = Hd;
    float* sk = w.sk;
    long long skn = w.sk_n;
    for (int i = 0; i < 3; ++i) give_splitk(p[i], sk, skn);
    DR_TRY(tn_launch(p, 3, w.tn, w.tn_bytes, s, d->precision == DR_PREC_BF16 ? 1 : 3));
  }
  {
    ColsumJob cj[7] = {
        {nb, w.glog, nb, nullptr, 0, gr->net.l6.b}, {c2, w.gp2, c2, nullptr, 0, gr->net.l3.b},
        {c2, w.gy2, c2, w.xh2, c2, gr->net.n4.w},   {c2, w.gy2, c2, nullptr, 0, gr->net.n4.b},
        {c1, w.gp1, c1, nullptr, 0, gr->net.l0.b},  {c1, w.gy1, c1, w.xh1, c1, gr->net.n1.w},
        {c1, w.gy1, c1, nullptr, 0, gr->net.n1.b},
    };
    DR_TRY(op_colsum_multi(M, cj, 7, s));
  }
  return DR_OK;
}

static size_t step_ws(const dr_dims* d, int B) {
  Carve c(nullptr);
  c.f((long long)B * 3 * d->hidden);
  c.f((long long)B * 3 * d->hidden);
  c.f((long long)B * latent(d));
  const int mx = d->prior_h1 > d->rew_h1 ? d->prior_h1 : d->rew_h1;
  c.f((long long)B * (mx > d->actor_h1 ? mx : d->actor_h1) * 2);
  c.f((long long)B * (d->buckets + 8) * 2);
  return c.off;
}

extern "C" size_t dr_step_workspace_bytes(const dr_dims* d, int B) { return step_ws(d, B) + 4096; }

static int mlp3(const dr_mlp3& m, int M, int in_h, const float* h, long long ldh, int in_z, const float* z,
                long long ldz, int h1, int h2, int n_out, float* out, long long ldo, float* p1, float* p2,
                hipStream_t s) {
  GemmArgs g = in_z ? lin2(M, h1, h, ldh, in_h, z, ldz, in_z, m.l0.w, m.l0.b, p1, h1)
                    : lin(M, h1, in_h, h, ldh, m.l0.w, in_h, m.l0.b, p1, h1);
  DR_TRY(run(G_NT, AM_PLAIN, g, s));
  DR_TRY(run(G_NT, AM_LNSILU, lin_ln(M, h2, h1, p1, h1, m.n1, m.l3.w, m.l3.b, p2, h2), s));
  return run(G_NT, AM_LNSILU, lin_ln(M, n_out, h2, p2, h2, m.n4, m.l6.w, m.l6.b, out, ldo), s);
}

extern "C" int dr_mlp3_fwd(const dr_mlp3* m, int M, int in_h, const float* h, long long ldh, int in_z,
                           const float* z, long long ldz, int h1, int h2, int n_out, float* out, long long ldo,
                           void* ws, size_t ws_bytes, hipStream_t s) {
  DR_REQUIRE(m && h && out && M > 0 && h1 > 0 && h2 > 0 && n_out > 0, "null argument or bad widths");
  Carve c(ws);
  float* p1 = c.f((long long)M * h1);
  float* p2 = c.f((long long)M * h2);
  WS_CHECK(c, ws_bytes);
  return mlp3(*m, M, in_h, h, ldh, in_z, z, ldz, h1, h2, n_out, out, ldo, p1, p2, s);
}

struct TraceWs {
  ObsWs o;
  float *zc, *zl;
  int* idxl;
  float *p1, *p2;
  ImWs w;
};
static void trace_carve(Carve& c, const dr_dims* d, int B, int T, TraceWs& a) {
  const long long BT = (long long)B * T;
  const int L = latent(d), Hd = d->hidden;
  obs_carve(c, d, B, a.o);
  a.zc = c.f((long long)B * L);
  a.zl = c.f((long long)B * L);
  a.idxl = c.i(2LL * B * d->rows);
  a.p1 = c.f(BT * d->prior_h1);
  a.p2 = c.f(BT * d->prior_h2);
  ImWs& w = a.w;
  memset(&w, 0, sizeof(w));
  w.p1r = c.f(BT * d->rew_h1);
  w.p1c = c.f(BT * d->cont_h1);
  w.p2r = c.f(BT * d->rew_h2);
  w.p2c = c.f(BT * d->cont_h2);
  w.rlog = c.f(BT * d->buckets);
  w.clog = c.f(BT);
  w.rval = c.f(BT);
  w.s3r = c.raw(op_nt_split3_ws_bytes(d->rew_h1, Hd + L));
  w.s3c = c.raw(op_nt_split3_ws_bytes(d->cont_h1, Hd + L));
  w.s3part_n = op_gemm_nt_split3_part_floats((int)BT, std::max(d->rew_h1, d->cont_h1));
  w.s3part = c.f((long long)w.s3part_n);
}

// ... 126 lines not shown
```

dreamer_amd/csrc/gemm.h:

```cpp
#pragma once
#include "common.h"

enum { AM_PLAIN = 0, AM_LNSILU = 1, AM_CONV = 2, AM_CONV_SRC = 3, AM_LNBWD = 4, AM_STEBWD = 5 };

struct GruBwdEpi {
  const float* h; long long ldh;
  const float *r, *u, *n, *ghn;
  float *gi, *gh;
  float* ho; long long ldo;
  int Hd, pad_;
  unsigned short *gi16, *gh16;
};

struct alignas(16) GemmArgs {
  int M, N, K;
  const float* A; long long lda;
  const float* A2; long long lda2; int ksplitA;
  const float* ln_g; const float* ln_b;
  float* a_out; long long ld_aout;
  const float* pre; long long ld_pre;
  float* splitk_ws; long long splitk_floats;
  float* sv_gy; float* sv_xh; long long ld_sv;
  int cin, ih, iw, oh, ow;
  dr_frames src;
  int nb;
  const float* W; long long ldb;
  const float* W2; long long ldb2; int ksplitB; int nsplitB;
  const float* bias; const float* addend; long long ld_add;
  float* Y; long long ldy;
  float* Y2; long long ldy2; int nsplitY;
  int accumulate, act, out_conv;
  float alpha;
  int epi;
  dr_noise noise; int step;
  int R, C; float unimix;
  float* z_out; long long ldz; int* idx_out; float* soft_out; long long ld_soft;
  float* zval_out;
  int na, det;
  float* act_out; long long ld_act; float* mu_out; long long ld_mu; float* sig_out; long long ld_sig;
  float* eps_save; float* ls_save; long long ld_ls;
  int bf16;
  GruBwdEpi gb;
  const unsigned short* wsplit; int wsplit_np, pad2_;
  const unsigned short* A16;
};

enum { EPI_NONE = 0, EPI_SAMPLE = 1, EPI_ACTOR = 2 };

enum GemmLayout { G_NT = 0, G_NN = 1, G_TN = 2 };

GemmArgs gemm_args();
struct GemmBf16Scope {
  explicit GemmBf16Scope(bool on);
  ~GemmBf16Scope();
  int prev;
};
int gemm_launch(GemmLayout lay, int amode, const GemmArgs* probs, int count, hipStream_t s);

enum GemmFamily {
  GF_LEGACY = 0,
  GF_SKINNY,
  GF_TILE,
  GF_TILE_B16,
  GF_WK,
  GF_WKS3,
  GF_LN_SAMPLE,
  GF_S3_TALL,
  GF_LN_ROWS,
  GF_SPLITK_FINISH
};
struct GemmStep {
  int family, bm, bn, kc, nw, amode, a_km, b_kn, vec, epi, bf16, a16;
  int mask;
  int gx, gy, gz, block, lds;
  int splits, npack, no_ws;
};
struct GemmPlan {
  int rc; char err[192];
  int ln_pre, nsteps;
  GemmStep step[10];
};
GemmPlan gemm_plan(GemmLayout lay, int amode, const GemmArgs* probs, int count);
int gemm_run(const GemmPlan& pl, const GemmArgs* probs, int count, hipStream_t s);
int gemm_bwd_fusable(const GemmPlan& pl);

struct alignas(16) Mlp2Args {
  int M, K1, K2, pad_;
  const float* X; long long ldx;
  const float* ln1_g; const float* ln1_b;
  const float* W3; const float* b3;
  const float* ln4_g; const float* ln4_b;
  float* a1_out; long long ld_a1;
  float* pre2; long long ld_pre2;
  float* a2_out; long long ld_a2;
  GemmArgs e;
};
bool mlp2_ok(const Mlp2Args& a);
int mlp2_launch(const Mlp2Args* probs, int count, hipStream_t s);
```

dreamer_amd/csrc/gemm.hip:

```cpp
#include <limits.h>
#include <stdarg.h>
#include <stdio.h>
#include <stdlib.h>
#include <stdint.h>
#include <string.h>

#include "gemm.h"
#include "conv.h"

#include <algorithm>

#define BK 32
#define LDS_K (BK + 2)

struct GemmBatch {
  GemmArgs p[4];
};

template <int BM, int BN>
__device__ __forceinline__ int dr_pack_tile(const GemmBatch& gb, int npack, int& z) {
  z = blockIdx.z;
  if (npack <= 0) return -2;
  int tot = 0;
  for (int i = 0; i < npack; ++i) tot += ((gb.p[i].M + BM - 1) / BM) * ((gb.p[i].N + BN - 1) / BN);
// ... 1752 lines not shown
      for (int j = 0; j < FN; ++j) {
        const unsigned e = (unsigned)((c * 3 + p) * Np) * 32u + ob[j];
        rb[sl][p][j] = *(const DR_GLOBAL wk_u32x4*)((const DR_GLOBAL char*)wr + (e << 1));
      }
  };
  constexpr int NA = 1;
  f32x4 acc[NA][FM][FN];
#pragma unroll
  for (int a3 = 0; a3 < NA; ++a3)
#pragma unroll
    for (int i = 0; i < FM; ++i)
#pragma unroll
      for (int j = 0; j < FN; ++j) acc[a3][i][j] = (f32x4){0.f, 0.f, 0.f, 0.f};
#pragma unroll
  for (int u = 0; u < D; ++u) load(min(c0 + u, clast), u);
  const int ncw = c1 - c0;
  for (int cc = 0; cc < ncw; cc += D) {
#pragma unroll
    for (int u = 0; u < D; ++u) {
      if (cc + u >= ncw) break;
      const int c = c0 + cc + u;
      const bool kin = 32 * c + 8 * q < K;
      wk_u32x4 a[NTP][FM];
#pragma unroll
      for (int i = 0; i < FM; ++i) {
        if constexpr (A16) {
          a[0][i] = kin ? ra16[u][i] : (wk_u32x4){0u, 0u, 0u, 0u};
          continue;
        }
        f32x4 x0 = ra[A16 ? 0 : u][i][0], x1 = ra[A16 ? 0 : u][i][1];
        if (!kin) x0 = x1 = (f32x4){0.f, 0.f, 0.f, 0.f};
        if constexpr (NTP == 3) {
          unsigned h[4], m[4], l[4];
          split3_pair(x0[0], x0[1], h[0], m[0], l[0]);
          split3_pair(x0[2], x0[3], h[1], m[1], l[1]);
          split3_pair(x1[0], x1[1], h[2], m[2], l[2]);
          split3_pair(x1[2], x1[3], h[3], m[3], l[3]);
          a[0][i] = (wk_u32x4){h[0], h[1], h[2], h[3]};
          a[1 % NTP][i] = (wk_u32x4){m[0], m[1], m[2], m[3]};
          a[2 % NTP][i] = (wk_u32x4){l[0], l[1], l[2], l[3]};
        } else {
          a[0][i] = (wk_u32x4){wk_pack_rne(x0[0], x0[1]), wk_pack_rne(x0[2], x0[3]), wk_pack_rne(x1[0], x1[1]),
                               wk_pack_rne(x1[2], x1[3])};
        }
      }
#define DR_WK3(PA, PB, X)                        \
  _Pragma("unroll") for (int i = 0; i < FM; ++i) _Pragma("unroll") for (int j = 0; j < FN; ++j) acc[X][i][j] = \
      wk_mfma(rb[u][PB][j], a[PA][i], acc[X][i][j]);
      if constexpr (NTP == 3) {
        DR_WK3(2 % NTP, 0, 0)
        DR_WK3(1 % NTP, 1 % NTP, 0)
        DR_WK3(0, 2 % NTP, 0)
        DR_WK3(1 % NTP, 0, 0)
        DR_WK3(0, 1 % NTP, 0)
      }
      DR_WK3(0, 0, 0)
#undef DR_WK3
      load(min(c + D, clast), u);
    }
  }
  {
#pragma unroll
    for (int i = 0; i < FM; ++i)
#pragma unroll
      for (int j = 0; j < FN; ++j) {
        const f32x4 v = acc[0][i][j];
#pragma unroll
        for (int e = 0; e < 4; ++e) red[wave][(i * FN + j) * 4 + e][lane] = v[e];
      }
  }
  __syncthreads();
#pragma unroll
  for (int ii = 0; ii < NEPI; ++ii) {
    const int x = tid + NTH * ii;
    if (x >= NT4) break;
    const int l = x & 63, e = (x >> 6) & 3, tj = x >> 8;
    float v = 0.f;
#pragma unroll
    for (int w = 0; w < NW; ++w) v += red[w][tj * 4 + e][l];
    const int t = tj / FN, j = tj - t * FN;
    const int m = m0 + t * 16 + (l & 15), n = n0 + j * 16 + 4 * (l >> 4) + e;
    if (m >= M || n >= N) continue;
    epilogue_store_b(g, m, n, v, ebias[ii]);
  }
}

__global__ __launch_bounds__(256) void k_splitk_finish(GemmBatch gb, int splits) {
  __shared__ GemmArgs s_args;
  dr_stage_args(gb.p[blockIdx.z], s_args, threadIdx.x);
  const GemmArgs& g = s_args;
  const long long MN = (long long)g.M * g.N;
  const long long i = (long long)blockIdx.x * 256 + threadIdx.x;
  if (i >= MN) return;
  float v = 0.f;
  for (int sp = 0; sp < splits; ++sp) v += dr_g(g.splitk_ws)[sp * MN + i];
  const int m = (int)(i / g.N), n = (int)(i - (long long)m * g.N);
  epilogue_store(g, m, n, v);
}

#define MLP2_KMAX 208
#define MLP2_NC 128
struct Mlp2Batch {
  Mlp2Args p[3];
};

__device__ __forceinline__ float4 mlp2_ln_silu(float4 x, bool ok, int K, const float* gam, const float* bet, int k) {
  const float mean = wave_sum(ok ? (x.x + x.y) + (x.z + x.w) : 0.f) / (float)K;
  float sq = 0.f;
  if (ok) {
    const float dx = x.x - mean, dy = x.y - mean, dz = x.z - mean, dw = x.w - mean;
    sq = (dx * dx + dy * dy) + (dz * dz + dw * dw);
  }
  const float rstd = 1.0f / sqrtf(wave_sum(sq) / (float)K + 1e-5f);
  if (!ok) return make_float4(0.f, 0.f, 0.f, 0.f);
  const float4 gv = dr_ld4(gam, (unsigned)k), bv = dr_ld4(bet, (unsigned)k);
  return make_float4(dr_silu_fast((x.x - mean) * rstd * gv.x + bv.x), dr_silu_fast((x.y - mean) * rstd * gv.y + bv.y),
                     dr_silu_fast((x.z - mean) * rstd * gv.z + bv.z), dr_silu_fast((x.w - mean) * rstd * gv.w + bv.w));
}

#define MLP2_KS (MLP2_KMAX / 16)
__device__ __forceinline__ void mlp2_wload(float4 (&wv)[MLP2_KS], const float* W, int ldw, int n, bool nok, int K,
                                           int q) {
  const int ks = (K + 15) >> 4;
#pragma unroll
  for (int s = 0; s < MLP2_KS; ++s) {
    const int k = 16 * s + 4 * q;
    const bool ok = s < ks && nok && k < K;
    wv[s] = dr_ld4(W, ok ? (unsigned)(n * ldw + k) : 0u);
    if (!ok) wv[s] = make_float4(0.f, 0.f, 0.f, 0.f);
  }
}
template <int LP>
__device__ __forceinline__ f32x4 mlp2_tile(const float (*ys)[LP], const float4 (&wv)[MLP2_KS], int K, int r, int q) {
  const int ks = (K + 15) >> 4;
  f32x4 c[4];
#pragma unroll
  for (int j = 0; j < 4; ++j) c[j] = (f32x4){0.f, 0.f, 0.f, 0.f};
#pragma unroll
  for (int s = 0; s < MLP2_KS; ++s) {
    if (s < ks) {
      const float4 a = *reinterpret_cast<const float4*>(&ys[r][16 * s + 4 * q]);
      c[s & 3] = __builtin_amdgcn_mfma_f32_16x16x4f32(a.x, wv[s].x, c[s & 3], 0, 0, 0);
      c[s & 3] = __builtin_amdgcn_mfma_f32_16x16x4f32(a.y, wv[s].y, c[s & 3], 0, 0, 0);
      c[s & 3] = __builtin_amdgcn_mfma_f32_16x16x4f32(a.z, wv[s].z, c[s & 3], 0, 0, 0);
      c[s & 3] = __builtin_amdgcn_mfma_f32_16x16x4f32(a.w, wv[s].w, c[s & 3], 0, 0, 0);
    }
  }
  f32x4 o;
#pragma unroll
  for (int e = 0; e < 4; ++e) o[e] = (c[0][e] + c[1][e]) + (c[2][e] + c[3][e]);
  return o;
}

__global__ __launch_bounds__(512) void k_mlp2_tail(Mlp2Batch mb) {
  __shared__ Mlp2Args s_a;
  dr_stage_args(mb.p[blockIdx.z], s_a, threadIdx.x);
  const Mlp2Args& a = s_a;
  const GemmArgs& g = a.e;
  const int M = dr_uni(a.M), K1 = dr_uni(a.K1), K2 = dr_uni(a.K2), N = dr_uni(g.N);
  const int n0 = blockIdx.x * MLP2_NC, m0 = blockIdx.y * 16;
  if (n0 >= N || m0 >= M) return;
  const int tid = threadIdx.x, wave = tid >> 6, lane = tid & 63;
  const int r = lane & 15, q = lane >> 4;
  constexpr int LP = MLP2_KMAX + 8;
  __shared__ __attribute__((aligned(16))) float ys[16][LP];
  __shared__ __attribute__((aligned(16))) float hs[16][LP];
  __shared__ float so[16][MLP2_NC + 1];
  const bool c0 = blockIdx.x == 0;
  const int k = 4 * lane;
  const int ncols = min(MLP2_NC, N - n0);
  const float* X = dr_uni(a.X);
  const int ldx = dr_uni((int)a.ldx);
  float4 xr[2];
#pragma unroll
  for (int i = 0; i < 2; ++i) {
    const int m = m0 + wave + 8 * i;
    const bool ok = m < M && k < K1;
    xr[i] = dr_ld4(X, ok ? (unsigned)(m * ldx + k) : 0u);
  }
  const int nt3 = (K2 + 15) >> 4;
  float4 w3[2][MLP2_KS];
#pragma unroll
  for (int i = 0; i < 2; ++i) {
    const int n = (wave + 8 * i) * 16 + r;
    mlp2_wload(w3[i], a.W3, K1, n, wave + 8 * i < nt3 && n < K2, K1, q);
  }
  const int ntd = (ncols + 15) >> 4;
  float4 w6[MLP2_KS];
  {
    const int nl = wave * 16 + r;
    mlp2_wload(w6, dr_uni(g.W), dr_uni((int)g.ldb), n0 + nl, wave < ntd && nl < ncols, K2, q);
  }

  {
    const int KP = (K1 + 15) & ~15;
#pragma unroll
    for (int i = 0; i < 2; ++i) {
      const int rr = wave + 8 * i, m = m0 + rr;
      const bool ok = m < M && k < K1;
      const float4 y = mlp2_ln_silu(xr[i], ok, K1, a.ln1_g, a.ln1_b, k);
      if (k < KP) *reinterpret_cast<float4*>(&ys[rr][k]) = y;
      if (c0 && a.a1_out && ok) dr_st4(a.a1_out, (unsigned)(m * a.ld_a1 + k), y);
    }
  }
  __syncthreads();
#pragma unroll
  for (int i = 0; i < 2; ++i) {
    const int tj = wave + 8 * i;
    if (tj < nt3) {
      const int n = tj * 16 + r;
      const f32x4 acc = mlp2_tile<LP>(ys, w3[i], K1, r, q);
      const float bv = (n < K2 && a.b3) ? dr_ld1(a.b3, (unsigned)n) : 0.f;
#pragma unroll
      for (int e = 0; e < 4; ++e) {
        const int ml = 4 * q + e, m = m0 + ml;
        const float v = (n < K2) ? acc[e] + bv : 0.f;
        hs[ml][n] = v;
        if (c0 && a.pre2 && m < M && n < K2) dr_g(a.pre2)[(long long)m * a.ld_pre2 + n] = v;
      }
    }
  }
  __syncthreads();
  {
    const int KP = (K2 + 15) & ~15;
    for (int rr = wave; rr < 16; rr += 8) {
      const int m = m0 + rr;
      const bool ok = k < K2;
      float4 x = ok ? *reinterpret_cast<const float4*>(&hs[rr][k]) : make_float4(0.f, 0.f, 0.f, 0.f);
      float4 y = mlp2_ln_silu(x, ok, K2, a.ln4_g, a.ln4_b, k);
      if (m >= M) y = make_float4(0.f, 0.f, 0.f, 0.f);
      if (k < KP) *reinterpret_cast<float4*>(&ys[rr][k]) = y;
      if (c0 && a.a2_out && ok && m < M) dr_st4(a.a2_out, (unsigned)(m * a.ld_a2 + k), y);
    }
  }
  __syncthreads();
  if (wave < ntd) {
    const int nl = wave * 16 + r, n = n0 + nl;
    const f32x4 acc = mlp2_tile<LP>(ys, w6, K2, r, q);
    const float bv = (nl < ncols && g.bias) ? dr_ld1(g.bias, (unsigned)n) : 0.f;
#pragma unroll
    for (int e = 0; e < 4; ++e) so[4 * q + e][nl] = acc[e] + bv;
  }
  __syncthreads();
  if (g.epi == EPI_SAMPLE) {
    const int C = g.C;
    int W = 1;
    while (W < C) W <<= 1;
    const int gpr = ncols / C, npairs = 16 * gpr, per_wave = 64 / W;
    for (int pbase = wave * per_wave; pbase < npairs; pbase += 8 * per_wave) {
      const int pidx = pbase + lane / W, c = lane % W;
      const bool valid = pidx < npairs;
      const int ml = valid ? pidx / gpr : 0, gl = valid ? pidx - ml * gpr : 0;
      const int m = m0 + ml, grp = (n0 / C) + gl;
      const bool act = valid && c < C && m < M;
      const float x = act ? so[ml][gl * C + c] : -INFINITY;
      if (act && g.Y) dr_g(g.Y)[(long long)m * g.ldy + n0 + gl * C + c] = x;
      const float mx = group_max(x, W);
      const float ex = act ? expf(x - mx) : 0.0f;
      const float se = group_sum(ex, W);
      const float p = ex / se;
      const float pu = act ? (0.99f * p + g.unimix) : 0.0f;
      const float sp = group_sum(pu, W);
      const float ph = pu / sp;
      float qv = 1.0f;
      const int Rg = g.R;
      if (act) {
        if (g.noise.q) qv = dr_g(g.noise.q)[((long long)g.step * M * Rg + (long long)m * Rg + grp) * C + c];
        else qv = dr_exp1(g.noise.rng, (uint32_t)(g.noise.stream + g.step), (uint32_t)(g.noise.row0 + m),
                          (uint32_t)(grp * C + c));
      }
      float best = act ? ph / qv : -INFINITY;
      int bi = act ? c : 0x7fffffff;
      group_argmax(best, bi, W);
      if (act) {
        dr_g(g.z_out)[(long long)m * g.ldz + grp * C + c] = (c == bi) ? ((1.0f + pu) - pu) : 0.0f;
        if (g.soft_out) dr_g(g.soft_out)[(long long)m * g.ld_soft + grp * C + c] = p;
        if (g.idx_out && c == 0) dr_g(g.idx_out)[m * Rg + grp] = bi;
        if (g.zval_out && c == bi) dr_g(g.zval_out)[m * Rg + grp] = (1.0f + pu) - pu;
      }
    }
  } else if (g.epi == EPI_ACTOR) {
    const int A = g.na;
    for (int x = tid; x < 16 * A; x += 512) {
      const int ml = x / A, i = x - ml * A, m = m0 + ml;
      if (m >= M) continue;
      const float muv = so[ml][i];
      const float lr = so[ml][A + i];
      const float ls = fminf(fmaxf(lr, -5.0f), 2.0f);
      const float sg = dr_softplus(ls) + 1e-3f;
      float av;
      if (g.det) {
        av = tanhf(muv);
      } else {
        float e;
        if (g.noise.eps) e = dr_g(g.noise.eps)[((long long)g.step * M + m) * A + i];
        else e = dr_normal(g.noise.rng, (uint32_t)(g.noise.stream + g.step), (uint32_t)(g.noise.row0 + m),
                           (uint32_t)i);
        if (g.eps_save) dr_g(g.eps_save)[(long long)m * A + i] = e;
        av = tanhf(muv + e * sg);
      }
      if (g.act_out) dr_g(g.act_out)[(long long)m * g.ld_act + i] = av;
      if (g.mu_out) dr_g(g.mu_out)[(long long)m * g.ld_mu + i] = muv;
      if (g.sig_out) dr_g(g.sig_out)[(long long)m * g.ld_sig + i] = sg;
      if (g.ls_save) dr_g(g.ls_save)[(long long)m * g.ld_ls + i] = lr;
    }
  } else {
    for (int x = tid; x < 16 * ncols; x += 512) {
      const int ml = x / ncols, nl = x - ml * ncols, m = m0 + ml;
      if (m >= M) continue;
      dr_g(g.Y)[(long long)m * g.ldy + n0 + nl] = epi_act(g, so[ml][nl]);
    }
  }
}

bool mlp2_ok(const Mlp2Args& a) {
  const GemmArgs& g = a.e;
  const bool al = !(((uintptr_t)a.X | (uintptr_t)a.W3 | (uintptr_t)g.W | (uintptr_t)a.ln1_g | (uintptr_t)a.ln1_b |
                     (uintptr_t)a.ln4_g | (uintptr_t)a.ln4_b) & 15) &&
                  !((uintptr_t)a.a1_out & 15) && !((uintptr_t)a.a2_out & 15);
  return !(a.M < 1 || a.K1 < 4 || a.K2 < 4 || a.K1 > MLP2_KMAX || a.K2 > MLP2_KMAX || a.K1 % 4 || a.K2 % 4 ||
           a.ldx % 4 || g.ldb % 4 || a.ld_a1 % 4 || a.ld_a2 % 4 || g.K != a.K2 || g.N < 1 || !al ||
           (g.epi == EPI_SAMPLE && (g.C < 1 || g.C > 32 || 32 % g.C != 0 || MLP2_NC % g.C != 0)) ||
           (g.epi == EPI_ACTOR && (g.N != 2 * g.na || g.N > 16)) || (g.epi == EPI_NONE && !g.Y) ||
           g.accumulate || g.addend || g.alpha != 1.0f);
}

int mlp2_launch(const Mlp2Args* probs, int count, hipStream_t s) {
  if (count < 1 || count > 3) {
    dr_set_error("mlp2_launch: bad problem count %d", count);
    return DR_E_INVALID;
  }
  Mlp2Batch mb;
  int gx = 1, gy = 1;
  for (int i = 0; i < count; ++i) {
    const Mlp2Args& a = probs[i];
    const GemmArgs& g = a.e;
    if (!mlp2_ok(a)) {
      dr_set_error("mlp2_launch: unsupported problem (M=%d K1=%d K2=%d N=%d epi=%d)", a.M, a.K1, a.K2, g.N, g.epi);
      return DR_E_INVALID;
    }
    mb.p[i] = a;
    gx = std::max(gx, dr_cdiv(g.N, MLP2_NC));
    gy = std::max(gy, dr_cdiv(a.M, 16));
  }
  hipLaunchKernelGGL(k_mlp2_tail, dim3(gx, gy, count), dim3(512), 0, s, mb);
  return dr_check_launch("mlp2_tail");
}


template <int LNV>
__global__ __launch_bounds__(256) void k_ln_silu_rows(int M, int K, const float* __restrict__ X, int ldx,
                                                      const float* __restrict__ gam, const float* __restrict__ bet,
                                                      float* __restrict__ Y, int ldy) {
  const int wave = threadIdx.x >> 6, lane = threadIdx.x & 63;
  const int m = blockIdx.x * 4 + wave;
  if (m >= M) return;
  const int K4 = K >> 2;
  float4 xv[LNV], gv[LNV], bv[LNV];
#pragma unroll
  for (int i = 0; i < LNV; ++i) {
    const int k4 = lane + 64 * i;
    const bool ok = k4 < K4;
    xv[i] = ok ? *reinterpret_cast<const float4*>(X + (long long)m * ldx + 4 * k4) : make_float4(0.f, 0.f, 0.f, 0.f);
    gv[i] = ok ? *reinterpret_cast<const float4*>(gam + 4 * k4) : make_float4(0.f, 0.f, 0.f, 0.f);
    bv[i] = ok ? *reinterpret_cast<const float4*>(bet + 4 * k4) : make_float4(0.f, 0.f, 0.f, 0.f);
  }
  float sm = 0.f;
#pragma unroll
  for (int i = 0; i < LNV; ++i) sm += (xv[i].x + xv[i].y) + (xv[i].z + xv[i].w);
  const float mean = wave_sum(sm) / (float)K;
  float sq = 0.f;
#pragma unroll
  for (int i = 0; i < LNV; ++i) {
    if (lane + 64 * i < K4) {
      const float dx = xv[i].x - mean, dy = xv[i].y - mean, dz = xv[i].z - mean, dw = xv[i].w - mean;
      sq += (dx * dx + dy * dy) + (dz * dz + dw * dw);
    }
  }
  const float rstd = 1.0f / sqrtf(wave_sum(sq) / (float)K + 1e-5f);
#pragma unroll
  for (int i = 0; i < LNV; ++i) {
    const int k4 = lane + 64 * i;
    if (k4 < K4) {
      float4 y;
      y.x = dr_silu_fast((xv[i].x - mean) * rstd * gv[i].x + bv[i].x);
      y.y = dr_silu_fast((xv[i].y - mean) * rstd * gv[i].y + bv[i].y);
      y.z = dr_silu_fast((xv[i].z - mean) * rstd * gv[i].z + bv[i].z);
      y.w = dr_silu_fast((xv[i].w - mean) * rstd * gv[i].w + bv[i].w);
      *reinterpret_cast<float4*>(Y + (long long)m * ldy + 4 * k4) = y;
    }
  }
}

static bool aligned16(const void* p) { return ((uintptr_t)p & 15) == 0; }
struct PlanProbs {
  const GemmArgs* p[4];
  int mask = 0, n = 0;
  void add(const GemmArgs* g, int i) { p[n++] = g; mask |= 1 << i; }
  const GemmArgs& operator[](int i) const { return *p[i]; }
};
static void plan_fail(GemmPlan& pl, const char* fmt, ...) {
  va_list ap;
  va_start(ap, fmt);
  vsnprintf(pl.err, sizeof(pl.err), fmt, ap);
  va_end(ap);
  pl.rc = DR_E_INVALID;
}
static GemmStep& plan_step(GemmPlan& pl, int family, int mask, int gx, int gy, int gz, int block) {
  GemmStep& st = pl.step[pl.nsteps++] = GemmStep{};
  st.family = family; st.mask = mask; st.gx = gx; st.gy = gy; st.gz = gz; st.block = block;
  return st;
}
static bool rows_aligned(const GemmArgs& g, int kq, bool a, bool w) {
  if (a && (g.K % kq != 0 || g.lda % 4 != 0 || !aligned16(g.A))) return false;
  if (a && g.ksplitA < g.K && (g.ksplitA % kq != 0 || g.lda2 % 4 != 0 || !aligned16(g.A2))) return false;
  return !w || (g.ldb % 4 == 0 && aligned16(g.W));
}
struct TileCount { int maxt, tot; bool ws; int maxM, minK; };
static TileCount tile_count(const PlanProbs& q, int bm, int bn) {
  TileCount c = {0, 0, true, 0, 1 << 30};
  for (int i = 0; i < q.n; ++i) {
    const int t = dr_cdiv(q[i].M, bm) * dr_cdiv(q[i].N, bn);
    c.maxt = std::max(c.maxt, t);
    c.tot += t;
    c.ws = c.ws && q[i].splitk_ws != nullptr;
    c.maxM = std::max(c.maxM, q[i].M);
    c.minK = std::min(c.minK, q[i].K);
  }
  return c;
}
static int splitk_count(const PlanProbs& q, int tot, int kc) {
  int nch = 1 << 30;
  for (int i = 0; i < q.n; ++i) nch = std::min(nch, dr_cdiv(q[i].K, kc));
  int splits = std::max(1, std::min(DR_TILE_SPLITS, dr_cdiv(512, tot)));
  splits = std::min(splits, std::max(1, nch / 2));
  for (int i = 0; i < q.n; ++i)
    while (splits > 1 && (long long)splits * q[i].M * q[i].N > q[i].splitk_floats) --splits;
  return splits;
}

static bool skinny_offsets_ok(const GemmArgs& g, bool b_kn) {
  const long long lim = 1LL << 30;
  return (long long)g.M * g.lda < lim && (long long)g.M * g.lda2 < lim && (long long)(b_kn ? g.K : g.N) * g.ldb < lim &&
         !(g.W2 && (long long)(g.K + g.N) * g.ldb2 >= lim) && !(g.a_out && (long long)g.M * g.ld_aout >= lim);
}

static int skinny_tile_rows(const PlanProbs& q, int amode, int maxM, bool sample) {
  if (maxM <= 64) return 16;
  if (amode != AM_PLAIN && amode != AM_LNSILU && amode != AM_LNBWD && amode != AM_STEBWD) return 64;
  return tile_count(q, 16, sample ? 32 : 16).tot <= 640 ? 16 : 64;
}

static bool plan_skinny(GemmPlan& pl, const PlanProbs& q, int amode, bool b_kn) {
  int maxM = 0, epi = EPI_NONE;
  bool vec = true;
  for (int i = 0; i < q.n; ++i) {
    const GemmArgs& g = q[i];
    if (g.out_conv) return false;
    if ((g.epi == EPI_SAMPLE) != (q[0].epi == EPI_SAMPLE)) return false;
    if (g.epi != EPI_NONE) epi = g.epi;
    maxM = g.M > maxM ? g.M : maxM;
    if (!skinny_offsets_ok(g, b_kn)) return false;
    vec = vec && rows_aligned(g, 4, true, !b_kn);
  }
  if (maxM > (epi == EPI_NONE ? (1 << 20) : 4096)) return false;
  const int mt = skinny_tile_rows(q, amode, maxM, epi == EPI_SAMPLE);
  bool wide = mt == 16 && tile_count(q, 16, 16).tot > 256;
  bool wide48 = false;
  if (amode == AM_LNBWD && epi == EPI_NONE && wide && vec) {
    const int t32 = tile_count(q, 16, 32).tot;
    wide48 = t32 > 256 && t32 < 512 && tile_count(q, 16, 48).tot <= 256;
    for (int i = 0; i < q.n; ++i) wide48 = wide48 && sk_staged(amode, 16, 48, q[i].K, vec, b_kn);
  }
  const bool bwd = amode == AM_LNBWD || amode == AM_STEBWD;
  if (bwd && wide && !wide48 && epi != EPI_SAMPLE)
    for (int i = 0; i < q.n; ++i) wide = wide && sk_staged(amode, 16, 32, q[i].K, vec, b_kn);
  const int nt = epi == EPI_SAMPLE ? 32 : (epi == EPI_ACTOR || mt == 64) ? 16 : wide48 ? 48 : wide ? 32 : 16;
  int lds = 0;
  for (int i = 0; i < q.n; ++i) {
    if (bwd && !sk_staged(amode, mt, nt, q[i].K, vec, b_kn)) return false;
    lds = std::max(lds, sk_lds_floats(amode, mt, nt, q[i].K, vec, b_kn));
  }
  const TileCount tc = tile_count(q, mt, nt);
  if (tc.maxt == 0) return true;
  const int npack = q.n > 1 ? q.n : 0;
  GemmStep& st =
      plan_step(pl, GF_SKINNY, q.mask, dr_xcd_grid(npack ? tc.tot : tc.maxt), 1, npack ? 1 : q.n, 64 * DR_SKW);
  st.bm = mt; st.bn = nt; st.amode = amode; st.b_kn = b_kn; st.vec = vec; st.epi = epi; st.npack = npack;
  st.lds = lds * (int)sizeof(float);
  return true;
}

static void plan_tile(GemmPlan& pl, const PlanProbs& q, int family, int bm, int bn, int kc, int nw, bool a_km,
                      bool b_kn, bool no_ws) {
  const TileCount tc = tile_count(q, bm, bn);
  if (tc.maxt == 0) return;
  const bool b16 = family == GF_TILE_B16;
  long long maxMN = 0;
  bool vec = true;
// ... 435 lines not shown
```

dreamer_amd/engine.py:

```python
import contextlib
import gc

import numpy as np

import torch

from . import _lib as L
from . import hip

WARM_STREAM = 1 << 24
DREAM_STREAM = 2 << 24
_CU_STREAMS = {}


@contextlib.contextmanager
def _no_gc():
    enabled = gc.isenabled()
    gc.collect()
    gc.disable()
    try:
        yield
    finally:
        if enabled:
            gc.enable()


def cu_mask_words(n_cus, fraction):
    keep = max(1, min(n_cus, int(round(n_cus * fraction))))
    words = [0] * ((n_cus + 31) // 32)
    for i in range(keep):
        words[i // 32] |= 1 << (i % 32)
    return words


class ImaginationEngine:
    def __init__(self, dreamer, B=None, world=None, use_graph=True):
        self.dr = dreamer
        self.dev = dreamer.device
        self.B = int(B or dreamer.batch_size)
        self.S = int(dreamer.sequence_length)
        self.H = int(dreamer.horizon)
        self.T = self.S // 2
        self.world = world
        self.rank = world[0] if world else 0
        self.wsize = world[1] if world else 1
        self.dp = world is not None
        self.use_graph = use_graph
        self.graph = None
        self.graph_key = None
        self.side = torch.cuda.Stream(self.dev)
        self.chunks = [(0, self.T)]
        mode = getattr(dreamer, "explore", "none")
        self.explorer = dreamer.explorer if mode == "disagreement" else None
        self.entropy = mode == "entropy"
        if mode != "none" and world is not None:
            raise ValueError(f"explore = {mode!r} is not supported under data parallelism")
        if self.explorer is not None:
            self.explorer._ensure_flat()
        self._alloc()
    @staticmethod
    def warm_chunks(T, size=8):
        return [(t0, min(T, t0 + size)) for t0 in range(0, T, size)]

    def dims(self):
        return self.dr.world_model.dims(self.dr.agent)

    def _alloc(self):
        d = self.dims()
        self.d = d
        B, H, T = self.B, self.H, self.T
        L_ = d.rows * d.cols
        dev = self.dev
        f = lambda *s: torch.zeros(*s, device=dev)
        self.starts = torch.zeros(B, dtype=torch.int64, device=dev)
        self.starts_host = [torch.zeros(B, dtype=torch.int64).pin_memory() for _ in range(2)]
        self.copy_ev = [None, None]
        self.epochs = 0
        self.act_win = f(B, self.S, d.action)
        self.feat = f(T * B, d.enc_hidden)
        self.z0, self.h0 = f(B, L_), f(B, d.hidden)
        self.latents, self.hiddens = f(B, H + 1, L_), f(B, H + 1, d.hidden)
        self.actions, self.mus, self.sigmas = f(B, H, d.action), f(B, H, d.action), f(B, H, d.action)
        self.rewards, self.continues = f(B, H), f(B, H)
        self.V_t, self.V_c = f(B, H + 1), f(B, H + 1)
        self.R = f(B, H)
        self.R_all = f(self.wsize * B, H) if self.dp else self.R
        self.norm = f(1)
        self.loss_a = f(1 + B * H)
        self.g_mu, self.g_sig = f(B, H, d.action), f(B, H, d.action)
        self.sq = f(2)
        self.skip = torch.zeros(1, dtype=torch.int32, device=dev)
        M = B * (H + 1)
        self.ws_enc = hip.workspace(dev).get("e_enc", L.query("dr_encoder_workspace_bytes", d, T * B))
        self.ws_obs = hip.workspace(dev).get("e_obs", L.query("dr_observe_workspace_bytes", d, B))
        self.tape = torch.zeros(L.query("dr_imagine_tape_bytes", d, B, H), dtype=torch.uint8, device=dev)
        self.ws_im = hip.workspace(dev).get("e_im", L.query("dr_imagine_workspace_bytes", d, B, H))
        self.ctape = torch.zeros(L.query("dr_critic_tape_bytes", d, M), dtype=torch.uint8, device=dev)
        self.ws_cr = hip.workspace(dev).get("e_cr", L.query("dr_critic_workspace_bytes", d, B, H))
        self.ws_cr2 = hip.workspace(dev).get("e_cr2", L.query("dr_critic_workspace_bytes", d, B, H))
        self.rng = hip.rng(dev)
        if self.explorer is not None:
            ex = self.explorer
            n = L.query("dr_disag_workspace_bytes", ex.members, ex.width, d.hidden, L_, M, 0)
            self.ws_disag = torch.empty(max(int(n), 256), dtype=torch.uint8, device=dev)
        if self.entropy:
            row = torch.arange(M, dtype=torch.int32, device=dev)
            self.knn_groups = row // (H + 1) if self.dr.explore_knn_exclude == "dream" else row
            n = L.query("dr_knn_workspace_bytes", M, M, d.hidden, self.dr.explore_knn)
            self.ws_knn = torch.empty(max(int(n), 256), dtype=torch.uint8, device=dev)

    def encode_and_warm(self, frames, noise_q=None):
        d, st = self.d, hip.stream()
        wm = self.dr.world_model.packed()
        L.call("dr_encoder_features", d, wm, frames, self.B, self.T, L.ptr(self.feat), L.ptr(self.ws_enc),
               self.ws_enc.numel(), st)
        if noise_q is not None:
            nz = hip.explicit_noise(q=noise_q, device=self.dev)
        else:
            nz = L.dr_noise(None, None, self.rng.state.data_ptr(), self.rank * self.B, WARM_STREAM)
        A = d.action
        L.call("dr_observe_scan", d, wm, self.B, self.T, L.ptr(self.feat), L.ptr(self.act_win), self.S * A, A, None,
               None, nz, L.ptr(self.z0), L.ptr(self.h0), None, L.ptr(self.ws_obs), self.ws_obs.numel(), st)

    def imagine(self, eps=None, q=None, deterministic=False, z0=None, h0=None, d=None):
        d = self.d if d is None else d
        z0 = self.z0 if z0 is None else z0
        h0 = self.h0 if h0 is None else h0
        if eps is not None or q is not None:
            nz = hip.explicit_noise(q=q, eps=eps, device=self.dev)
        else:
            nz = L.dr_noise(None, None, self.rng.state.data_ptr(), self.rank * self.B, DREAM_STREAM)
        L.call("dr_imagine_fwd", d, self.dr.world_model.packed(), self.dr.agent.actor_struct(), self.B, self.H,
               L.ptr(z0), L.ptr(h0), nz, int(deterministic), L.ptr(self.latents), L.ptr(self.hiddens),
               L.ptr(self.actions), L.ptr(self.rewards), L.ptr(self.continues), L.ptr(self.mus),
               L.ptr(self.sigmas), L.ptr(self.tape), L.ptr(self.ws_im), self.ws_im.numel(), hip.stream())

    def returns(self):
        ag, d, st = self.dr.agent, self.d, hip.stream()
        M = self.B * (self.H + 1)
        L_ = d.rows * d.cols
        if self.explorer is not None:
            dr = self.dr
            L.call("dr_disag_fwd", self.explorer.struct(), d.hidden, L_, M, L.ptr(self.hiddens), d.hidden, None, None,
                   L.ptr(self.rewards), self.H + 1, 1, self.H, 1, dr.explore_extrinsic, dr.explore_scale,
                   L.ptr(self.ws_disag), self.ws_disag.numel(), st)
        if self.entropy:
            dr, g = self.dr, L.ptr(self.knn_groups)
            L.call("dr_state_entropy_fwd", d.hidden, dr.explore_knn, M, L.ptr(self.hiddens), d.hidden, g, M,
                   L.ptr(self.hiddens), d.hidden, g, None, None, None, L.ptr(self.rewards), self.H + 1, 1, self.H, 1,
                   dr.explore_extrinsic, dr.explore_scale, L.ptr(self.ws_knn), self.ws_knn.numel(), st)
        L.call("dr_critic_fwd", d, ag.critic_struct(target=True), M, L.ptr(self.hiddens), d.hidden,
               L.ptr(self.latents), L_, None, L.ptr(self.V_t), None, L.ptr(self.ws_cr), self.ws_cr.numel(), st)
        L.call("dr_lambda_returns", self.B, self.H, L.ptr(self.rewards), L.ptr(self.continues), L.ptr(self.V_t),
               ag.gamma, ag.lambda_, L.ptr(self.R), st)

    def losses_and_grads(self, fork=True):
        ag, d = self.dr.agent, self.d
        main = torch.cuda.current_stream(self.dev)
        st = main.cuda_stream
        B, H = self.B, self.H
        M = B * (H + 1)
        L_ = d.rows * d.cols
        scale = 1.0 / float(B * self.wsize * H)
        L.call("dr_critic_fwd", d, ag.critic_struct(), M, L.ptr(self.hiddens), d.hidden, L.ptr(self.latents), L_,
               None, L.ptr(self.V_c), L.ptr(self.ctape), L.ptr(self.ws_cr), self.ws_cr.numel(), st)
        critic_args = (d, ag.critic_struct(), B, H, L.ptr(self.hiddens), L.ptr(self.latents), L.ptr(self.R),
                       L.ptr(self.ctape), scale, L.ptr(ag.loss_slot(1)), ag.critic_struct(grad=True),
                       L.ptr(self.ws_cr), self.ws_cr.numel())
        if fork:
            self.side.wait_stream(main)
            L.call("dr_critic_loss_bwd", *critic_args, self.side.cuda_stream)
        L.call("dr_update_S", self.R_all.numel(), L.ptr(self.R_all), L.ptr(ag.S_dev), L.ptr(self.norm), None, 0, st)
        L.call("dr_actor_loss_grad", B, H, d.action, L.ptr(self.mus), L.ptr(self.sigmas), L.ptr(self.actions),
               L.ptr(self.R), L.ptr(self.V_c), L.ptr(self.norm), ag.nu, scale, L.ptr(self.loss_a), L.ptr(self.g_mu),
               L.ptr(self.g_sig), st)
        if not fork:
            L.call("dr_critic_loss_bwd", *critic_args, st)
        L.call("dr_imagine_bwd", d, self.dr.world_model.packed(), ag.actor_struct(), B, H, L.ptr(self.latents),
               L.ptr(self.hiddens), L.ptr(self.actions), L.ptr(self.g_mu), L.ptr(self.g_sig), None, None, None,
               L.ptr(self.tape), ag.actor_struct(grad=True), L.ptr(self.ws_im), self.ws_im.numel(), st)
        ag.loss_slot(0).copy_(self.loss_a[0:1])
        if fork:
            main.wait_stream(self.side)

    def _x_critic_fwd_and_prep(self):
        ag, d, st = self.dr.agent, self.d, hip.stream()
        M = self.B * (self.H + 1)
        L.call("dr_critic_fwd", d, ag.critic_struct(), M, L.ptr(self.hiddens), d.hidden, L.ptr(self.latents),
               d.rows * d.cols, None, L.ptr(self.V_c), L.ptr(self.ctape), L.ptr(self.ws_cr2), self.ws_cr2.numel(),
               st)
        L.call("dr_imagine_bwd_prep", d, self.dr.world_model.packed(), ag.actor_struct(), self.B, self.H, None,
               None, None, L.ptr(self.ws_im), self.ws_im.numel(), st)

    def _actor_loss(self):
        ag, d, st = self.dr.agent, self.d, hip.stream()
        B, H = self.B, self.H
        scale = 1.0 / float(B * self.wsize * H)
        L.call("dr_update_S", self.R_all.numel(), L.ptr(self.R_all), L.ptr(ag.S_dev), L.ptr(self.norm), None, 0, st)
        L.call("dr_actor_loss_grad", B, H, d.action, L.ptr(self.mus), L.ptr(self.sigmas), L.ptr(self.actions),
               L.ptr(self.R), L.ptr(self.V_c), L.ptr(self.norm), ag.nu, scale, L.ptr(self.loss_a), L.ptr(self.g_mu),
               L.ptr(self.g_sig), st)

    def _x_critic_bwd(self):
        ag, d = self.dr.agent, self.d
        B, H = self.B, self.H
        scale = 1.0 / float(B * self.wsize * H)
        L.call("dr_critic_loss_bwd", d, ag.critic_struct(), B, H, L.ptr(self.hiddens), L.ptr(self.latents),
               L.ptr(self.R), L.ptr(self.ctape), scale, L.ptr(ag.loss_slot(1)), ag.critic_struct(grad=True),
               L.ptr(self.ws_cr2), self.ws_cr2.numel(), hip.stream())

    def _bptt(self, d=None):
        ag, d = self.dr.agent, (self.d if d is None else d)
        L.call("dr_imagine_bwd_main", d, self.dr.world_model.packed(), ag.actor_struct(), self.B, self.H,
               L.ptr(self.latents), L.ptr(self.hiddens), L.ptr(self.actions), L.ptr(self.g_mu), L.ptr(self.g_sig),
               0, L.ptr(self.tape), ag.actor_struct(grad=True), L.ptr(self.ws_im), self.ws_im.numel(), hip.stream())
        ag.loss_slot(0).copy_(self.loss_a[0:1])

    def optimise(self):
        self.dr.agent.fused_optimiser_step(self.sq, self.skip)

    def _encode_chunk(self, t0, t1, stream_ptr):
        d = self.d
        fr = self.dr.buffer.frames_struct(self.starts)
        fr.t0 = t0
        off = t0 * self.B * d.enc_hidden * 4
        L.call("dr_encoder_features", d, self.dr.world_model.packed(), fr, self.B, t1 - t0,
               L.ptr(self.feat) + off, L.ptr(self.ws_enc), self.ws_enc.numel(), stream_ptr)

    def _scan_chunk(self, t0, t1, stream_ptr):
        d, A = self.d, self.d.action
        nz = L.dr_noise(None, None, self.rng.state.data_ptr(), self.rank * self.B, WARM_STREAM + t0)
        feat = L.ptr(self.feat) + t0 * self.B * d.enc_hidden * 4
        if t0 == 0:
            acts, zi, hi = L.ptr(self.act_win), None, None
        else:
            acts, zi, hi = L.ptr(self.act_win) + (t0 - 1) * A * 4, L.ptr(self.z0), L.ptr(self.h0)
        L.call("dr_observe_scan", d, self.dr.world_model.packed(), self.B, t1 - t0, feat, acts, self.S * A, A,
               hi, zi, nz, L.ptr(self.z0), L.ptr(self.h0), None, L.ptr(self.ws_obs), self.ws_obs.numel(),
               stream_ptr)

    def _ph_encwarm(self):
        main = torch.cuda.current_stream(self.dev)
        self.dr.buffer.gather_actions(self.starts, self.act_win)
        self.side.wait_stream(main)
        done = []
        with torch.cuda.stream(self.side):
            for t0, t1 in self.chunks:
                self._encode_chunk(t0, t1, self.side.cuda_stream)
                ev = torch.cuda.Event()
                ev.record(self.side)
                done.append(ev)
        for (t0, t1), ev in zip(self.chunks, done):
            main.wait_event(ev)
            self._scan_chunk(t0, t1, main.cuda_stream)

    def time_encoder(self, reps=5):
        st = torch.cuda.current_stream(self.dev)
        for t0, t1 in self.chunks:
            self._encode_chunk(t0, t1, st.cuda_stream)
        a, b = torch.cuda.Event(enable_timing=True), torch.cuda.Event(enable_timing=True)
        a.record(st)
        for _ in range(reps):
            for t0, t1 in self.chunks:
                self._encode_chunk(t0, t1, st.cuda_stream)
        b.record(st)
        b.synchronize()
        return a.elapsed_time(b) / reps

    def _ph_update(self):
        self.losses_and_grads(fork=False)

    def _ph_optim(self):
        self.optimise()
        L.call("dr_rng_advance", self.rng.state.data_ptr(), 1, hip.stream())

    def phases(self):
        ph = [("encwarm", self._ph_encwarm, None), ("imagine", self.imagine, None),
              ("returns", self.returns, self._allgather_R if self.dp else None),
              ("update", self._ph_update, self._allreduce_grads if self.dp else None),
              ("optim", self._ph_optim, None)]
        if self.dp and not self.persistent_bptt():
            ph[3:4] = [("critic", self._ph_critic, self._allreduce_critic_async),
                       ("actor", self._ph_actor, self._allreduce_actor)]
        return ph

    def persistent_chain(self):
        return bool(L.query("dr_persistent_kernels", self.d, self.B, self.T, self.H) & 2)

    def persistent_bptt(self):
        return bool(L.query("dr_persistent_kernels", self.d, self.B, self.T, self.H) & 4)

    def check_faults(self, wait=True):
        h, _ = self.dr.agent.fault_host()
        if wait:
            torch.cuda.current_stream(self.dev).synchronize()
        if int(h[0]) != 0:
            self._on_fault()

    def _on_fault(self):
        ag = self.dr.agent
        torch.cuda.synchronize(self.dev)
        ag.fault_slot().zero_()
        ag.fault_host()[0][0] = 0
        ag.persistent_ok = False
        self.d = self.dims()
        self.graph, self.graph_key, self._pipe = None, None, None
        raise RuntimeError("dreamer_amd: a persistent kernel (posterior scan / imagination unroll / BPTT) timed out "
                           "waiting on another workgroup (not every workgroup was resident, e.g. other work held "
                           "CUs); its outputs were NaN and that epoch's actor-critic update was skipped. Every "
                           "later epoch runs the launch form.")

    def _ph_critic(self):
        ag, d, st = self.dr.agent, self.d, hip.stream()
        B, H = self.B, self.H
        M = B * (H + 1)
        scale = 1.0 / float(B * self.wsize * H)
        L.call("dr_critic_fwd", d, ag.critic_struct(), M, L.ptr(self.hiddens), d.hidden, L.ptr(self.latents),
               d.rows * d.cols, None, L.ptr(self.V_c), L.ptr(self.ctape), L.ptr(self.ws_cr), self.ws_cr.numel(), st)
        self._actor_loss()
        L.call("dr_critic_loss_bwd", d, ag.critic_struct(), B, H, L.ptr(self.hiddens), L.ptr(self.latents),
               L.ptr(self.R), L.ptr(self.ctape), scale, L.ptr(ag.loss_slot(1)), ag.critic_struct(grad=True),
               L.ptr(self.ws_cr), self.ws_cr.numel(), st)
        ag.loss_slot(0).copy_(self.loss_a[0:1])

    def _ph_actor(self):
        ag, d = self.dr.agent, self.d
        L.call("dr_imagine_bwd", d, self.dr.world_model.packed(), ag.actor_struct(), self.B, self.H,
               L.ptr(self.latents), L.ptr(self.hiddens), L.ptr(self.actions), L.ptr(self.g_mu), L.ptr(self.g_sig),
               None, None, None, L.ptr(self.tape), ag.actor_struct(grad=True), L.ptr(self.ws_im), self.ws_im.numel(),
               hip.stream())

    def epoch_body(self):
        for _, body, coll in self.phases():
            body()
            if coll is not None:
                coll()

    def _allgather_R(self):
        import torch.distributed as dist
        parts = list(self.R_all.view(self.wsize, self.B, self.H).unbind(0))
        dist.all_gather(parts, self.R, group=self.world[2])

    def _allreduce_grads(self):
        import torch.distributed as dist
        ag = self.dr.agent
        dist.all_reduce(ag.grad_buffer, op=dist.ReduceOp.SUM, group=self.world[2])
        ag.loss_buffer.div_(self.wsize)

    def _allreduce_critic_async(self):
        import torch.distributed as dist
        ag = self.dr.agent
        na = ag.fa.grad.numel()
        self._critic_work = dist.all_reduce(ag.grad_buffer[na:], op=dist.ReduceOp.SUM, group=self.world[2],
                                            async_op=True)

    def _allreduce_actor(self):
        import torch.distributed as dist
        ag = self.dr.agent
        na = ag.fa.grad.numel()
        dist.all_reduce(ag.grad_buffer[:na], op=dist.ReduceOp.SUM, group=self.world[2])
        self._critic_work.wait()
        self._critic_work = None
        ag.loss_buffer.div_(self.wsize)

    def _graph_key(self):
        key = (self.dr.agent.params_key(), self.dr.world_model.params_key(), self.dr.buffer.device_key())
        if self.explorer is not None:
            key += (self.explorer.params_key(), self.dr.explore_extrinsic, self.dr.explore_scale)
        if self.entropy:
            key += ("entropy", self.dr.explore_knn, self.dr.explore_knn_exclude, self.dr.explore_extrinsic,
                    self.dr.explore_scale)
        return key

    def run(self, starts_np, timing=False):
        self.check_faults(wait=False)
        if isinstance(starts_np, torch.Tensor) and starts_np.is_cuda:
            if starts_np.dtype != torch.int64 or tuple(starts_np.shape) != tuple(self.starts.shape):
                raise ValueError(f"device starts must be int64 of shape {tuple(self.starts.shape)}")
            self.starts.copy_(starts_np)
        else:
            i = self.epochs & 1
            if self.copy_ev[i] is not None:
                self.copy_ev[i].synchronize()
            self.starts_host[i].copy_(torch.from_numpy(np.asarray(starts_np, dtype=np.int64)))
            self.starts.copy_(self.starts_host[i], non_blocking=True)
            self.copy_ev[i] = torch.cuda.Event()
            self.copy_ev[i].record()
        self.epochs += 1
        ag = self.dr.agent
        key = self._graph_key()
        if self.use_graph and (self.graph is None or self.graph_key != key):
            self._capture(key)
        evs = [torch.cuda.Event(enable_timing=True)] if timing else None
        if evs:
            evs[0].record()
        for k, (name, body, coll) in enumerate(self.phases()):
            if self.use_graph:
                self.graph[k].replay()
            else:
                body()
            if coll is not None:
                coll()
            if evs:
                e = torch.cuda.Event(enable_timing=True)
                e.record()
                evs.append(e)
        self.last_events = evs
        return ag.loss_slot(0), ag.loss_slot(1)

    def phase_ms(self):
        names = [p[0] for p in self.phases()]
        ev = self.last_events
        return {n: ev[k].elapsed_time(ev[k + 1]) for k, n in enumerate(names)}

    def warm_stream(self, cu_fraction=None):
        import ctypes
        import os
        if cu_fraction is None:
            cu_fraction = float(os.environ.get("DREAMER_WARM_CUS", "0.875"))
        if not 0.0 < cu_fraction < 1.0:
            return torch.cuda.Stream(self.dev)
        n = ctypes.c_int(0)
        with torch.cuda.device(self.dev):
            L.call("dr_device_cus", ctypes.byref(n))
            words = cu_mask_words(n.value, cu_fraction)
            ck = (torch.device(self.dev).index, tuple(words))
            h = _CU_STREAMS.get(ck)
            if h is None:
                mask = (ctypes.c_uint * len(words))(*words)
                h = ctypes.c_void_p()
                L.call("dr_stream_create_cumask", len(words), mask, ctypes.byref(h))
                _CU_STREAMS[ck] = h
        return torch.cuda.ExternalStream(h.value, device=self.dev)

    def _pipe_capture(self, key):
        dev, B, H = self.dev, self.B, self.H
        if getattr(self, "_pipe", None) is None:
            self._pipe = dict(
                stream=self.warm_stream(), side=torch.cuda.Stream(dev),
                rng=torch.zeros(2, dtype=torch.int64, device=dev),
                z0=[self.z0, torch.zeros_like(self.z0)],
                h0=[self.h0, torch.zeros_like(self.h0)],
                key=None)
        P = self._pipe
        if P["key"] == key:
            return P
        d, A = self.d, self.d.action
        dw = L.dr_dims.from_buffer_copy(d)
        dw.launch_form = 1

        def warm(s):
            st = torch.cuda.current_stream(dev).cuda_stream
            self.dr.buffer.gather_actions(self.starts, self.act_win)
            self._encode_chunk(0, self.T, st)
            nz = L.dr_noise(None, None, P["rng"].data_ptr(), self.rank * B, WARM_STREAM)
            L.call("dr_observe_scan", dw, self.dr.world_model.packed(), B, self.T, L.ptr(self.feat),
                   L.ptr(self.act_win), self.S * A, A, None, None, nz, L.ptr(P["z0"][s]), L.ptr(P["h0"][s]), None,
                   L.ptr(self.ws_obs), self.ws_obs.numel(), st)
            L.call("dr_rng_advance", P["rng"].data_ptr(), 1, st)

        cs = torch.cuda.Stream(dev)
        cs.wait_stream(torch.cuda.current_stream(dev))
        graphs = {}
        with _no_gc(), torch.cuda.stream(cs):
            for s in (0, 1):
                for name, body in (("warm", lambda s=s: warm(s)),
                                   ("imagine", lambda s=s: self.imagine(z0=P["z0"][s], h0=P["h0"][s], d=dw))):
                    g = torch.cuda.CUDAGraph()
                    with torch.cuda.graph(g, stream=cs):
                        body()
                    graphs[(name, s)] = g
# ... 119 lines not shown
```

include/dreamer_hip.h:

```cpp
#ifndef DREAMER_HIP_H
#define DREAMER_HIP_H

#include <hip/hip_runtime.h>
#include <stddef.h>

#ifdef __cplusplus
extern "C" {
#endif

#define DR_OK 0
#define DR_E_INVALID 1001
#define DR_E_HIP 1002
#define DR_E_WORKSPACE 1003
#define DR_E_UNSUPPORTED 1004

typedef struct { float* w; float* b; } dr_linear;

typedef struct { dr_linear l0, n1, l3, n4, l6; } dr_mlp3;

typedef struct {
  int hidden;
  int rows, cols;
  int action;
  int img_h, img_w;
  int enc_f1, enc_f2;
  int enc_hidden;
  int prior_h1, prior_h2, rew_h1, rew_h2, cont_h1, cont_h2;
  int actor_h1, actor_h2, critic_h1, critic_h2;
  int buckets;
  int dec_f1, dec_f2;
  int dec_hidden;
  int precision;
  int obs_dim;
  int enc_depth;
  int launch_form;
  float* fault;
  unsigned* fault_host;
} dr_dims;
#define DR_MAX_DEPTH 5
#define DR_PREC_FP32 0
#define DR_PREC_BF16 1

typedef struct {
  dr_linear conv[DR_MAX_DEPTH];
  dr_linear map0, map1, map3;
  float *w_ih, *w_hh, *b_ih, *b_hh;
  dr_mlp3 prior;
  dr_mlp3 reward;
  dr_mlp3 cont;
  float* buckets_rew;
} dr_world_model;

typedef struct {
  dr_linear up0, up1, up3;
  dr_linear convt[DR_MAX_DEPTH];
} dr_decoder;

typedef struct { dr_linear l0, n1, l3, n4, mu, ls; } dr_actor;

typedef struct { dr_mlp3 net; float* buckets; } dr_critic;

typedef struct {
  const float* q;
  const float* eps;
  const unsigned long long* rng;
  int row0;
  int stream;
} dr_noise;

typedef struct {
  const unsigned char* ring;
  long long ring_cap;
  const long long* starts;
  const float* obs;
  long long stride_b, stride_t;
  int raw255;
  int t0;
} dr_frames;

const char* dr_last_error(void);
int dr_version(void);

int dr_stream_create_cumask(int n_words, const unsigned* mask, hipStream_t* out);
int dr_stream_destroy(hipStream_t s);
int dr_device_cus(int* out);
int dr_host_device_ptr(void* host, void** dev);

size_t dr_encoder_workspace_bytes(const dr_dims* d, int n_frames);
int dr_encoder_features(const dr_dims* d, const dr_world_model* wm, const dr_frames* src, int B, int T,
                        float* feat, void* ws, size_t ws_bytes, hipStream_t stream);

size_t dr_observe_workspace_bytes(const dr_dims* d, int B);
int dr_observe_scan(const dr_dims* d, const dr_world_model* wm, int B, int T, const float* feat,
                    const float* actions, long long act_sb, long long act_st, const float* h_init,
                    const float* z_init, dr_noise noise, float* z_out, float* h_out, float* logits_out,
                    void* ws, size_t ws_bytes, hipStream_t stream);

size_t dr_observe_trace_workspace_bytes(const dr_dims* d, int B, int T);
int dr_observe_trace(const dr_dims* d, const dr_world_model* wm, int B, int T, const float* feat,
                     const float* actions, long long act_sb, long long act_st, const float* h_init,
                     const float* z_init, dr_noise noise, float* latents, float* hiddens, float* post_logits,
                     float* prior_logits, float* rewards, float* continues, void* ws, size_t ws_bytes,
                     hipStream_t stream);

size_t dr_imagine_tape_bytes(const dr_dims* d, int B, int H);
size_t dr_imagine_workspace_bytes(const dr_dims* d, int B, int H);
int dr_imagine_fwd(const dr_dims* d, const dr_world_model* wm, const dr_actor* actor, int B, int H,
                   const float* z0, const float* h0, dr_noise noise, int deterministic, float* latents,
                   float* hiddens, float* actions, float* rewards, float* continues, float* mus,
                   float* sigmas, void* tape, void* ws, size_t ws_bytes, hipStream_t stream);

size_t dr_imagine_actions_workspace_bytes(const dr_dims* d, int B, int H);
int dr_imagine_actions(const dr_dims* d, const dr_world_model* wm, int B, int H, const float* z0, const float* h0,
                       const float* actions, long long act_sb, long long act_st, dr_noise noise, float* latents,
                       float* hiddens, float* rewards, float* continues, void* ws, size_t ws_bytes,
                       hipStream_t stream);

int dr_imagine_bwd(const dr_dims* d, const dr_world_model* wm, const dr_actor* actor, int B, int H,
                   const float* latents, const float* hiddens, const float* actions, const float* g_mus,
                   const float* g_sigmas,
                   const float* g_actions, const float* g_latents, const float* g_hiddens,
                   const void* tape, const dr_actor* grad, void* ws, size_t ws_bytes, hipStream_t stream);
int dr_imagine_bwd_prep(const dr_dims* d, const dr_world_model* wm, const dr_actor* actor, int B, int H,
                        const float* g_actions, const float* g_latents, const float* g_hiddens, void* ws,
                        size_t ws_bytes, hipStream_t stream);
int dr_imagine_bwd_main(const dr_dims* d, const dr_world_model* wm, const dr_actor* actor, int B, int H,
                        const float* latents, const float* hiddens, const float* actions, const float* g_mus,
                        const float* g_sigmas, int upstream_state, const void* tape, const dr_actor* grad, void* ws,
                        size_t ws_bytes, hipStream_t stream);

int dr_imagine_step(const dr_dims* d, const dr_world_model* wm, int B, const float* h, const float* z,
                    const float* a, dr_noise noise, float* h_out, float* z_out, float* r_out, float* c_out,
                    void* ws, size_t ws_bytes, hipStream_t stream);
size_t dr_actor_act_workspace_bytes(const dr_dims* d, int B);
int dr_actor_act(const dr_dims* d, const dr_actor* actor, int B, const float* h, const float* z,
                 dr_noise noise, int deterministic, float* a_out, float* mu_out, float* sigma_out, void* ws,
                 size_t ws_bytes, hipStream_t stream);
size_t dr_act_step_workspace_bytes(const dr_dims* d);
int dr_act_step(const dr_dims* d, const dr_world_model* wm, const dr_actor* actor, const unsigned char* frame,
                int has_prev, const float* z_prev, const float* h, const float* a_prev, dr_noise noise,
                int deterministic, float* z_out, float* h_out, float* a_out, float* mu_out, float* sigma_out,
                float* logits_out, int* status, void* ws, size_t ws_bytes, hipStream_t stream);
#define DR_ACT_MAX_ENVS 16
size_t dr_act_batch_workspace_bytes(const dr_dims* d, int n_env);
int dr_act_batch(const dr_dims* d, const dr_world_model* wm, const dr_actor* actor, int n_env,
                 const unsigned char* frames, const unsigned char* first, const float* z_prev, const float* h,
                 const float* a_prev, dr_noise noise, int deterministic, float* z_out, float* h_out, float* a_out,
                 float* mu_out, float* sigma_out, float* logits_out, int* status, void* ws, size_t ws_bytes,
                 hipStream_t stream);
#define DR_ACT_VEC_MAX_OBS 1023
size_t dr_act_vec_workspace_bytes(const dr_dims* d, int n_env);
int dr_act_vec(const dr_dims* d, const dr_world_model* wm, const dr_actor* actor, int n_env, const float* obs,
               const unsigned char* first, const float* z_prev, const float* h, const float* a_prev, dr_noise noise,
               int deterministic, float* z_out, float* h_out, float* a_out, float* mu_out, float* sigma_out,
               float* logits_out, int* status, void* ws, size_t ws_bytes, hipStream_t stream);

int dr_gru_cell(const dr_dims* d, const dr_world_model* wm, int B, const float* z, const float* h,
                const float* a, float* h_out, void* ws, size_t ws_bytes, hipStream_t stream);
int dr_categorical_sample(int M, int R, int C, const float* logits, dr_noise noise, float* z_out,
                          int* idx_out, float* soft_out, hipStream_t stream);
int dr_mlp3_fwd(const dr_mlp3* m, int M, int in_h, const float* h, long long ldh, int in_z, const float* z,
                long long ldz, int h1, int h2, int n_out, float* out, long long ldo, void* ws, size_t ws_bytes,
                hipStream_t stream);
size_t dr_step_workspace_bytes(const dr_dims* d, int B);
int dr_bucket_value(int M, int nb, const float* logits, const float* buckets, float* out, hipStream_t stream);

size_t dr_critic_tape_bytes(const dr_dims* d, int M);
size_t dr_critic_workspace_bytes(const dr_dims* d, int B, int H);
int dr_critic_fwd(const dr_dims* d, const dr_critic* c, int M, const float* h, long long ldh, const float* z,
                  long long ldz, float* logits, float* values, void* tape, void* ws, size_t ws_bytes,
                  hipStream_t stream);
int dr_lambda_returns(int B, int H, const float* r, const float* c, const float* V, float gamma, float lam,
                      float* R, hipStream_t stream);
int dr_update_S(int n, const float* R, float* S, float* norm_out, void* ws, size_t ws_bytes,
                hipStream_t stream);
int dr_actor_loss_grad(int B, int H, int A, const float* mus, const float* sigmas, const float* actions,
                       const float* R, const float* V, const float* norm, float nu, float scale,
                       float* loss_out, float* g_mus, float* g_sigmas, hipStream_t stream);
int dr_critic_loss_bwd(const dr_dims* d, const dr_critic* c, int B, int H, const float* hiddens,
                       const float* latents, const float* R, const void* tape, float scale, float* loss_out,
                       const dr_critic* grad, void* ws, size_t ws_bytes, hipStream_t stream);

int dr_sqnorm(long long n, const float* g, float* acc, hipStream_t stream);
int dr_sqnorm_multi(long long n, const float* g, float* acc, float* scratch, hipStream_t stream);
#define DR_CLIP_SCRATCH_FLOATS 1024
int dr_clip_stats(long long na, const float* ga, long long nb, const float* gb, int nloss, const float* loss,
                  float* sq, int* skip, void* scratch, hipStream_t stream);
int dr_adamw(long long n, float* p, float* g, float* m, float* v, const float* sqnorm, float max_norm,
             double lr, double b1, double b2, double eps, double wd, int* step, float* hyper, const int* skip,
             hipStream_t stream);
int dr_ema(long long n, float* target, const float* src, float keep, float tau, const int* skip,
           hipStream_t stream);
int dr_ac_optimiser_step(long long na, float* pa, float* ga, float* ma, float* va, int* step_a, float* hyper_a,
                         double lr_a, double b1_a, double b2_a, double eps_a, double wd_a, long long nc, float* pc,
                         float* gc, float* mc, float* vc, int* step_c, float* hyper_c, double lr_c, double b1_c,
                         double b2_c, double eps_c, double wd_c, float max_norm, float* target, float ema_keep,
                         float tau, int nloss, const float* loss, float* sq, int* skip, void* scratch,
                         hipStream_t stream);
int dr_nonfinite(long long n, const float* x, int* flag, hipStream_t stream);

typedef struct {
  const float* actions; long long act_sb, act_st;
  const float* rewards; const float* continues; long long rc_sb, rc_st;
} dr_wm_batch;
typedef struct { float beta_pred, beta_dyn, beta_rep; } dr_wm_loss_cfg;
size_t dr_wm_train_workspace_bytes(const dr_dims* d, int B, int T);
#define DR_WM_PREP 1
#define DR_WM_FWD 2
#define DR_WM_BWD 4
#define DR_WM_BWD_HEADS 8
#define DR_WM_BWD_SCAN 16
#define DR_WM_BWD_ENC 32
int dr_wm_train_phase(const dr_dims* d, const dr_world_model* wm, const dr_decoder* dec, int B, int T,
                      const dr_frames* src, const dr_wm_batch* batch, dr_noise noise, dr_wm_loss_cfg cfg, int phases,
                      float* stats, int rows_global, float* losses, int* skip, const dr_world_model* g_wm,
                      const dr_decoder* g_dec, float* hiddens_out, float* latents_out, float* post_logits_out,
                      void* ws, size_t ws_bytes, hipStream_t stream);
int dr_wm_train_grads(const dr_dims* d, const dr_world_model* wm, const dr_decoder* dec, int B, int T,
                      const dr_frames* src, const dr_wm_batch* batch, dr_noise noise, dr_wm_loss_cfg cfg,
                      float* losses, int* skip, const dr_world_model* g_wm, const dr_decoder* g_dec,
                      float* hiddens_out, float* latents_out, float* post_logits_out, void* ws, size_t ws_bytes,
                      hipStream_t stream);

int dr_wm_window_scores(const dr_dims* d, int B, int T, dr_wm_loss_cfg cfg, void* ws, size_t ws_bytes,
                        float* scores_out, hipStream_t stream);

size_t dr_decoder_workspace_bytes(const dr_dims* d, int M);
int dr_decoder_fwd(const dr_dims* d, const dr_decoder* dec, int M, const float* h, long long ldh, const float* z,
                   long long ldz, float* mu, void* ws, size_t ws_bytes, hipStream_t stream);

int dr_frame_metrics(const dr_dims* d, int B, int T, const float* mu, const dr_frames* truth, float* sqerr,
                     unsigned char* pred_u8, unsigned char* true_u8, hipStream_t stream);

int dr_frame_ssim(const dr_dims* d, int B, int T, const float* mu, const dr_frames* truth, float* ssim,
                  float* ssim_ch, hipStream_t stream);

int dr_ensemble_metrics(const dr_dims* d, int B, int M, int T, const float* mu, const dr_frames* truth,
                        float* sqerr_mean, float* spread, unsigned char* mean_u8, unsigned char* std_u8,
                        float* mean_f32, hipStream_t stream);

int dr_latent_stats(int M, int R, int C, const float* post_logits, const float* prior_logits, float* kl,
                    float* post_entropy, float* prior_entropy, float* kl_groups, hipStream_t stream);

int dr_replay_returns(int B, int T, const float* rewards, long long rew_sb, const float* continues,
                      long long cont_sb, int rewards_symlog, const float* V, float gamma, float lam,
                      float* R_lambda, float* R_mc, float* td, hipStream_t stream);
int dr_value_stats(int B, int T, int Tt, int nb, const float* logits, long long ldl, const float* buckets,
                   const float* target, float* entropy, float* std_symlog, float* ce, hipStream_t stream);
int dr_action_logprob(int B, int T, int A, const float* mu, const float* sigma, const float* actions,
                      long long act_sb, long long act_st, float* logp, float* logp_dims, float* base_entropy,
                      hipStream_t stream);

#define DR_DREAM_STATS_MAX_DREAMS 64
#define DR_DREAM_STATS_MAX_LDS_FLOATS 15360
typedef struct {
  float *R_lambda, *R_mc, *adv, *adv_norm, *weight, *logp, *base_entropy;
  int* saturated;
  float *reward_mean, *reward_std, *ret_mean, *ret_std, *logp_mean, *logp_std, *alive, *action_spread;
  int *best, *worst, *n_finite;
} dr_dream_outputs;
int dr_dream_stats(int B, int M, int H, int A, const float* rewards, const float* continues,
                   const float* V_target, const float* V_online, const float* mus, const float* sigmas,
                   const float* actions, float gamma, float lam, const float* norm, float sat,
                   const dr_dream_outputs* out, hipStream_t stream);
int dr_actor_draws(int steps, int rows, int A, dr_noise noise, float* eps, hipStream_t stream);

size_t dr_occlude_workspace_bytes(const dr_dims* d, int F);
int dr_occlude_frames(const dr_dims* d, const dr_frames* src, int F, int s, int fill, const float* wb, int rb,
                      const float* gm, unsigned char* out, void* ws, size_t ws_bytes, hipStream_t stream);
int dr_saliency_scores(int F, int G, int A, int R, int C, const float* mu, const float* V, const float* logits,
                       const float* z, float* actor, float* value, float* value_delta, float* posterior_kl,
                       int* latent_flips, hipStream_t stream);
int dr_saliency_map(const dr_dims* d, int F, int s, const float* scores, const float* scale,
                    const dr_frames* frames, int ch, float* map, unsigned char* overlay, hipStream_t stream);
int dr_saliency_draws(int rows, int C, dr_noise noise, float* q, hipStream_t stream);

#define DR_PLAN_MAX_CANDIDATES 2048
#define DR_PLAN_MAX_ELEMS 1024
int dr_plan_sample(int E, int N, int N_pi, int H, int A, const float* mean, const float* std,
                   const float* policy_actions, dr_noise noise, float* actions, hipStream_t stream);
int dr_plan_update(int E, int N, int H, int A, int K, const float* rewards, const float* continues,
                   const float* v_last, float gamma, float temperature, float momentum, float std_min,
                   float std_max, const float* actions, float* mean, float* std, float* scores, int* elite_idx,
                   float* elite_w, int* n_elite, hipStream_t stream);

int dr_replay_gather(long long cap, int B, int S, int frame_elems, int A, const unsigned char* frames,
                     const float* actions, const float* rewards, const float* continues,
                     const long long* starts, float* obs_out, float* act_out, float* rew_out,
                     float* cont_out, hipStream_t stream);

size_t dr_replay_sample_workspace_bytes(long long cap);
int dr_replay_sample(long long cap, long long size, long long next_idx, int S, int B, const float* priority,
                     double p_floor, const double* u, const unsigned long long* rng, int stream_id,
                     long long* starts_out, float* prob_out, void* ws, size_t ws_bytes, hipStream_t stream);
int dr_replay_probabilities(long long cap, long long size, long long next_idx, int S, const float* priority,
                            double p_floor, float* prob_out, void* ws, size_t ws_bytes, hipStream_t stream);
int dr_replay_priority_update(long long cap, int B, const long long* starts, const float* scores, double c,
                              double beta, double alpha, double eps, double p_new, float* priority, int* visits,
                              hipStream_t stream);

#define DR_DISAG_MAX_MEMBERS 16
typedef struct {
  int K, W;
  dr_mlp3 m[DR_DISAG_MAX_MEMBERS];
} dr_ensemble;
size_t dr_disag_workspace_bytes(int K, int W, int Hd, int L, int M, int train);
int dr_disag_fwd(const dr_ensemble* e, int Hd, int L, int M, const float* h, long long ldh, float* pred_out,
                 float* disag_out, float* rew, int rew_T, int rew_skip, long long rew_sb, long long rew_st,
                 float w_ext, float w_int, void* ws, size_t ws_bytes, hipStream_t stream);
int dr_disag_train_grads(const dr_ensemble* e, int Hd, int L, int M, const float* h, long long ldh, const float* z,
                         long long ldz, const dr_ensemble* g, float* losses, void* ws, size_t ws_bytes,
                         hipStream_t stream);

#define DR_KNN_MAX_K 32
size_t dr_knn_workspace_bytes(int Mq, int Nb, int D, int k);
int dr_knn(int D, int k, int Mq, const float* q, long long ldq, const int* qg, int Nb, const float* bank,
           long long ldb, const int* bg, float* d2_out, int* idx_out, void* ws, size_t ws_bytes, hipStream_t stream);
int dr_state_entropy_fwd(int D, int k, int Mq, const float* q, long long ldq, const int* qg, int Nb, const float* bank,
                         long long ldb, const int* bg, float* d2_out, int* idx_out, float* ent_out, float* rew,
                         int rew_T, int rew_skip, long long rew_sb, long long rew_st, float w_ext, float w_int,
                         void* ws, size_t ws_bytes, hipStream_t stream);

int dr_persistent_kernels(const dr_dims* d, int B, int T, int H);

// ... 7 lines not shown
```

Baseline: 630,400 imagined latent-steps/s.

## Fuse reward, continue and critic heads into grouped GEMM and tail kernels

Adds a dr_heads_fwd path that runs the first layers of the reward, continue, target-critic and online-critic heads as one grouped split3 GEMM over the shared (hidden, latent) input. It then runs their LayerNorm/MLP tails in a single multi-head tail kernel. Imagination skips its own reward/continue heads when the fused path is enabled, and later critic_fwd calls are skipped. The aim is fewer launches and less re-reading of the imagined hiddens and latents, at the cost of a large new code path and an extra weight repack per call.

```diff
diff --git a/dreamer_amd/_lib.py b/dreamer_amd/_lib.py
--- a/dreamer_amd/_lib.py
+++ b/dreamer_amd/_lib.py
@@ -140,6 +140,10 @@
     "dr_critic_tape_bytes": (_sz, [_P(dr_dims), _i]),
     "dr_critic_workspace_bytes": (_sz, [_P(dr_dims), _i, _i]),
     "dr_critic_fwd": (_i, [_P(dr_dims), _P(dr_critic), _i, fp, _ll, fp, _ll, fp, fp, fp, fp, _sz, fp]),
+    "dr_heads_supported": (_i, [_P(dr_dims), _i, _i]),
+    "dr_heads_workspace_bytes": (_sz, [_P(dr_dims), _i, _i]),
+    "dr_heads_fwd": (_i, [_P(dr_dims), _P(dr_world_model), _P(dr_critic), _P(dr_critic), _i, _i, fp, fp, fp, fp,
+                          fp, fp, fp, fp, _sz, fp, _sz, fp, _sz, fp]),
     "dr_lambda_returns": (_i, [_i, _i, fp, fp, fp, _f, _f, fp, fp]),
     "dr_update_S": (_i, [_i, fp, fp, fp, fp, _sz, fp]),
     "dr_actor_loss_grad": (_i, [_i, _i, _i, fp, fp, fp, fp, fp, fp, _f, _f, fp, fp, fp, fp]),
diff --git a/dreamer_amd/csrc/conv.h b/dreamer_amd/csrc/conv.h
--- a/dreamer_amd/csrc/conv.h
+++ b/dreamer_amd/csrc/conv.h
@@ -52,6 +52,22 @@
 int op_gemm_nt_split3_ex(int M, int N, int K, const float* A, int lda, const float* A2, int lda2, int ksA,
                          const void* wr, const float* bias, int act, float* Y, int ldy, int accumulate, float* Y2,
                          int ldy2, int nsplitY, float* part, size_t part_floats, hipStream_t s, int splits_fixed = 0);
+#define DR_S3_HEADS 4
+#define DR_S3_HEADS_SPLITS 4
+struct S3Head {
+  const float* W;
+  int ldw, N;
+  const float* bias;
+  float* Y;
+  int ldy;
+};
+int op_s3_heads_splits(int M, int K);
+bool op_gemm_nt_split3_heads_supported(int M, int K, const float* A, int lda, const float* A2, int lda2, int ksA,
+                                       const S3Head* heads, int nh);
+size_t op_nt_split3_heads_ws_bytes(const int* widths, int nh, int K);
+size_t op_gemm_nt_split3_heads_part_floats(int M, const int* widths, int nh, int K);
+int op_gemm_nt_split3_heads(int M, int K, const float* A, int lda, const float* A2, int lda2, int ksA,
+                            const S3Head* heads, int nh, void* wr, float* part, size_t part_floats, hipStream_t s);
 
 int op_conv_repack_bf16(int cout, int cin, int cin_pad, const float* w, void* wr, hipStream_t s);
 int op_to_bf16_2d(int rows, int cols, const float* x, long long ld, void* y, hipStream_t s);
diff --git a/dreamer_amd/csrc/conv_hook.hip b/dreamer_amd/csrc/conv_hook.hip
--- a/dreamer_amd/csrc/conv_hook.hip
+++ b/dreamer_amd/csrc/conv_hook.hip
@@ -109,3 +109,24 @@
   if (rc != DR_OK && msg && msg_cap > 0) snprintf(msg, msg_cap, "%s", dr_last_error());
   return rc;
 }
+
+extern "C" int dr_internal_s3_heads_run(int M, int K, const float* A, int lda, const float* A2, int lda2, int ksA,
+                                        int nh, const int* widths, void* const* W, void* const* bias, void* const* Y,
+                                        const int* ldy, void* wr, float* part, long long part_floats, long long* need,
+                                        void* stream, char* msg, int msg_cap) {
+  if (msg && msg_cap > 0) msg[0] = 0;
+  if (nh < 1 || nh > DR_S3_HEADS || !widths) return DR_E_INVALID;
+  if (need) {
+    need[0] = (long long)op_nt_split3_heads_ws_bytes(widths, nh, K);
+    need[1] = (long long)op_gemm_nt_split3_heads_part_floats(M, widths, nh, K);
+    need[2] = op_s3_heads_splits(M, K);
+  }
+  if (!A) return DR_OK;
+  S3Head h[DR_S3_HEADS];
+  for (int i = 0; i < nh; ++i)
+    h[i] = {(const float*)W[i], K, widths[i], bias ? (const float*)bias[i] : nullptr, (float*)Y[i], ldy[i]};
+  const int rc = op_gemm_nt_split3_heads(M, K, A, lda, A2, lda2, ksA, h, nh, wr, part, (size_t)part_floats,
+                                         (hipStream_t)stream);
+  if (rc != DR_OK && msg && msg_cap > 0) snprintf(msg, msg_cap, "%s", dr_last_error());
+  return rc;
+}
diff --git a/dreamer_amd/csrc/conv_split.hip b/dreamer_amd/csrc/conv_split.hip
--- a/dreamer_amd/csrc/conv_split.hip
+++ b/dreamer_amd/csrc/conv_split.hip
@@ -1997,6 +1997,130 @@
     DR_TRY(dr_check_launch("s3_finish"));
   }
   return DR_OK;
+}
+
+struct S3Group {
+  int nh, ntot;
+  int n0[DR_S3_HEADS + 1];
+  int ldw[DR_S3_HEADS], ldy[DR_S3_HEADS];
+  const float* W[DR_S3_HEADS];
+  const float* bias[DR_S3_HEADS];
+  float* Y[DR_S3_HEADS];
+};
+__device__ __forceinline__ int s3_group_head(const S3Group& r, int n) {
+  int h = 0;
+#pragma unroll
+  for (int i = 1; i < DR_S3_HEADS; ++i)
+    if (i < r.nh && n >= r.n0[i]) h = i;
+  return h;
+}
+
+__global__ __launch_bounds__(256) void k_nt_repack_split3_heads(S3Group r, int K, int Np, u16* __restrict__ wr) {
+  const long long i = (long long)blockIdx.x * 256 + threadIdx.x;
+  const int KC = (K + 31) / 32;
+  if (i >= (long long)KC * 32 * Np) return;
+  const int n = (int)(i / (KC * 32)), k = (int)(i - (long long)n * KC * 32);
+  unsigned hh = 0, mm = 0, ll = 0;
+  if (n < r.ntot && k < K) {
+    const int h = s3_group_head(r, n);
+    split3(r.W[h][(long long)(n - r.n0[h]) * r.ldw[h] + k], hh, mm, ll);
+  }
+  const long long plane = (long long)Np * 32;
+  const long long base = ((long long)(k >> 5) * 3 * Np + n) * 32 + (k & 31);
+  wr[base] = (u16)hh;
+  wr[base + plane] = (u16)mm;
+  wr[base + 2 * plane] = (u16)ll;
+}
+
+__global__ __launch_bounds__(256) void k_s3_finish_heads(S3Group r, int M, int splits, const float* __restrict__ part) {
+  const long long i4 = (long long)blockIdx.x * 256 + threadIdx.x;
+  const int N = r.ntot, N4 = N / 4;
+  if (i4 >= (long long)M * N4) return;
+  const int m = (int)(i4 / N4), n = 4 * (int)(i4 - (long long)m * N4);
+  f32x4 v = (f32x4){0.f, 0.f, 0.f, 0.f};
+  for (int sp = 0; sp < splits; ++sp) v += *reinterpret_cast<const f32x4*>(part + ((long long)sp * M + m) * N + n);
+  const int h = s3_group_head(r, n), nl = n - r.n0[h];
+  if (r.bias[h]) v += *reinterpret_cast<const f32x4*>(r.bias[h] + nl);
+  *reinterpret_cast<f32x4*>(r.Y[h] + (long long)m * r.ldy[h] + nl) = v;
+}
+
+int op_s3_heads_splits(int M, int K) {
+  (void)M;
+  const int nch = (K + 31) / 32;
+  int sp = 1;
+  while (sp < DR_S3_HEADS_SPLITS && nch / (2 * sp) >= 8) sp *= 2;
+  return sp;
+}
+
+bool op_gemm_nt_split3_heads_supported(int M, int K, const float* A, int lda, const float* A2, int lda2, int ksA,
+                                       const S3Head* heads, int nh) {
+  if (nh < 1 || nh > DR_S3_HEADS || !heads) return false;
+  long long ntot = 0;
+  for (int i = 0; i < nh; ++i) {
+    const S3Head& h = heads[i];
+    if (h.N < 4 || h.N % 4 || h.ldy % 4 || h.ldy < h.N || h.ldw < K || !h.W || !h.Y || ((uintptr_t)h.Y & 15) ||
+        ((uintptr_t)h.bias & 15))
+      return false;
+    ntot += h.N;
+  }
+  return ntot <= (1 << 16) && (long long)M * ntot < (1LL << 29) &&
+         op_gemm_nt_split3_supported(M, (int)ntot, K, A, lda, A2, lda2, ksA, 4);
+}
+
+static int s3_heads_ntot(const int* widths, int nh) {
+  int n = 0;
+  for (int i = 0; i < nh; ++i) n += widths[i];
+  return n;
+}
+size_t op_nt_split3_heads_ws_bytes(const int* widths, int nh, int K) {
+  return op_nt_split3_ws_bytes(s3_heads_ntot(widths, nh), K);
+}
+size_t op_gemm_nt_split3_heads_part_floats(int M, const int* widths, int nh, int K) {
+  return (size_t)op_s3_heads_splits(M, K) * M * s3_heads_ntot(widths, nh);
+}
+
+int op_gemm_nt_split3_heads(int M, int K, const float* A, int lda, const float* A2, int lda2, int ksA,
+                            const S3Head* heads, int nh, void* wr, float* part, size_t part_floats, hipStream_t s) {
+  if (!op_gemm_nt_split3_heads_supported(M, K, A, lda, A2, lda2, ksA, heads, nh) || !wr || !part ||
+      ((uintptr_t)wr & 15) || ((uintptr_t)part & 15)) {
+    dr_set_error("gemm_nt_split3_heads: unsupported problem (M=%d K=%d heads=%d)", M, K, nh);
+    return DR_E_INVALID;
+  }
+  S3Group r = {};
+  r.nh = nh;
+  for (int i = 0; i < nh; ++i) {
+    r.n0[i] = r.ntot;
+    r.ntot += heads[i].N;
+    r.ldw[i] = heads[i].ldw;
+    r.ldy[i] = heads[i].ldy;
+    r.W[i] = heads[i].W;
+    r.bias[i] = heads[i].bias;
+    r.Y[i] = heads[i].Y;
+  }
+  for (int i = nh; i <= DR_S3_HEADS; ++i) r.n0[i] = r.ntot;
+  const int N = r.ntot, Np = s3_np(N), splits = op_s3_heads_splits(M, K);
+  if ((size_t)splits * M * N > part_floats) {
+    dr_set_error("gemm_nt_split3_heads: workspace too small");
+    return DR_E_WORKSPACE;
+  }
+  const long long total = (long long)((K + 31) / 32) * 32 * Np;
+  hipLaunchKernelGGL(k_nt_repack_split3_heads, dim3((unsigned)((total + 255) / 256)), dim3(256), 0, s, r, K, Np,
+                     (u16*)wr);
+  DR_TRY(dr_check_launch("nt_repack_split3_heads"));
+  GemmS3 g = {M, N, K, ksA < K ? ksA : K, lda, lda2, N, 0, Np, A, A2, (const u16*)wr, nullptr, part, splits, part,
+              0, 0, INT_MAX, 0, nullptr};
+  const long long w256 = (long long)((M + 255) / 256) * ((N + 127) / 128) * 8 * splits;
+  if (w256 >= 2048) {
+    const int tiles = ((M + 255) / 256) * ((N + 127) / 128);
+    hipLaunchKernelGGL((k_gemm_split3<256, 128>), dim3(dr_xcd_grid(tiles), (unsigned)splits), dim3(512), 0, s, g);
+  } else {
+    const int tiles = ((M + 127) / 128) * ((N + 127) / 128);
+    hipLaunchKernelGGL((k_gemm_split3<128, 128>), dim3(dr_xcd_grid(tiles), (unsigned)splits), dim3(256), 0, s, g);
+  }
+  DR_TRY(dr_check_launch("gemm_nt_split3_heads"));
+  hipLaunchKernelGGL(k_s3_finish_heads, dim3((unsigned)(((long long)M * (N / 4) + 255) / 256)), dim3(256), 0, s, r, M,
+                     splits, part);
+  return dr_check_launch("s3_finish_heads");
 }
 
 static int s3_pad(int n) { return (n + 127) / 128 * 128; }
diff --git a/dreamer_amd/csrc/engine.hip b/dreamer_amd/csrc/engine.hip
--- a/dreamer_amd/csrc/engine.hip
+++ b/dreamer_amd/csrc/engine.hip
@@ -591,7 +591,7 @@
                               const float* z0, const float* h0, dr_noise noise, int deterministic, float* latents,
                               float* hiddens, float* actions, float* rewards, float* continues, float* mus,
                               float* sigmas, void* tape, void* ws, size_t ws_bytes, hipStream_t s) {
-  DR_REQUIRE(d && wm && ac && z0 && h0 && latents && hiddens && actions && rewards && continues && mus && sigmas &&
+  DR_REQUIRE(d && wm && ac && z0 && h0 && latents && hiddens && actions && !rewards == !continues && mus && sigmas &&
                  tape && B > 0 && H > 0,
              "null argument or empty batch");
   DR_TRY(dims_envelope(__func__, d, ENV_GRU | ENV_SAMPLER | ENV_ACTOR));
@@ -631,28 +631,67 @@
   }
   if (!unrolled) DR_TRY(imagine_launch_form(d, wm, ac, B, H, noise, nq, deterministic, latents, hiddens, actions, mus,
                                             sigmas, tp, w, split_gru, zg, s));
+  if (!rewards) return DR_OK;
   return imagine_heads(d, wm, B, H, latents, hiddens, rewards, continues, w, s);
 }
+
+static int imagine_heads_tail(const dr_dims* d, const dr_world_model* wm, int B, int H, float* rewards,
+                              float* continues, ImWs& w, hipStream_t s, bool keep0);
 
 static int imagine_heads(const dr_dims* d, const dr_world_model* wm, int B, int H, const float* latents,
                          const float* hiddens, float* rewards, float* continues, ImWs& w, hipStream_t s, bool keep0) {
   const int L = latent(d), Hd = d->hidden;
+  const int M1 = B * (H + 1);
+  if (s3_first_layer(d, M1, d->rew_h1, hiddens, Hd, latents, L) &&
+      s3_first_layer(d, M1, d->cont_h1, hiddens, Hd, latents, L)) {
+    const int sp = op_s3_heads_splits(M1, Hd + L);
+    DR_TRY(op_nt_repack_split3(d->rew_h1, Hd + L, wm->reward.l0.w, Hd + L, w.s3r, s));
+    DR_TRY(op_nt_repack_split3(d->cont_h1, Hd + L, wm->cont.l0.w, Hd + L, w.s3c, s));
+    DR_TRY(op_gemm_nt_split3_sk(M1, d->rew_h1, Hd + L, hiddens, Hd, latents, L, Hd, w.s3r, wm->reward.l0.b, 0,
+                                w.p1r, d->rew_h1, w.s3part, w.s3part_n, s, sp));
+    DR_TRY(op_gemm_nt_split3_sk(M1, d->cont_h1, Hd + L, hiddens, Hd, latents, L, Hd, w.s3c, wm->cont.l0.b, 0,
+                                w.p1c, d->cont_h1, w.s3part, w.s3part_n, s, sp));
+  } else {
+    GemmArgs p[2];
+    p[0] = lin2(M1, d->rew_h1, hiddens, Hd, Hd, latents, L, L, wm->reward.l0.w, wm->reward.l0.b, w.p1r, d->rew_h1);
+    p[1] = lin2(M1, d->cont_h1, hiddens, Hd, Hd, latents, L, L, wm->cont.l0.w, wm->cont.l0.b, w.p1c, d->cont_h1);
+    DR_TRY(gemm_launch(G_NT, AM_PLAIN, p, 2, s));
+  }
+  return imagine_heads_tail(d, wm, B, H, rewards, continues, w, s, keep0);
+}
+
+static bool g_heads_tail = true;
+static bool heads_tail_on(const dr_dims* d) { return g_heads_tail && d->precision != DR_PREC_BF16; }
+
+static void reward_cont_tails(const dr_dims* d, const dr_world_model* wm, int B, int H, float* rewards,
+                              float* continues, const ImWs& w, bool keep0, HeadTail ht[2]) {
+  const int M1 = B * (H + 1);
+  GemmArgs e[2];
+  e[0] = lin_ln(M1, d->buckets, d->rew_h2, nullptr, d->rew_h2, wm->reward.n4, wm->reward.l6.w, wm->reward.l6.b, nullptr,
+                d->buckets);
+  e[1] = lin_ln(M1, 1, d->cont_h2, nullptr, d->cont_h2, wm->cont.n4, wm->cont.l6.w, wm->cont.l6.b, continues, 1);
+  e[1].act = 2;
+  memset(ht, 0, 2 * sizeof(HeadTail));
+  ht[0].a = mlp2(M1, d->rew_h1, d->rew_h2, w.p1r, d->rew_h1, wm->reward.n1, wm->reward.l3, wm->reward.n4, e[0]);
+  ht[1].a = mlp2(M1, d->cont_h1, d->cont_h2, w.p1c, d->cont_h1, wm->cont.n1, wm->cont.l3, wm->cont.n4, e[1]);
+  ht[0].buckets = wm->buckets_rew;
+  ht[0].val = rewards;
+  for (int i = 0; i < 2; ++i) {
+    ht[i].rm_h1 = H + 1;
+    ht[i].rm_k0 = keep0 ? 0 : 1;
+  }
+}
+
+static int imagine_heads_tail(const dr_dims* d, const dr_world_model* wm, int B, int H, float* rewards,
+                              float* continues, ImWs& w, hipStream_t s, bool keep0) {
+  {
+    HeadTail ht[2];
+    reward_cont_tails(d, wm, B, H, rewards, continues, w, keep0, ht);
+    if (heads_tail_on(d) && heads_tail_ok(ht[0]) && heads_tail_ok(ht[1])) return heads_tail_launch(ht, 2, s);
+  }
   {
     const int M1 = B * (H + 1);
     GemmArgs p[2];
-    if (s3_first_layer(d, M1, d->rew_h1, hiddens, Hd, latents, L) &&
-        s3_first_layer(d, M1, d->cont_h1, hiddens, Hd, latents, L)) {
-      DR_TRY(op_nt_repack_split3(d->rew_h1, Hd + L, wm->reward.l0.w, Hd + L, w.s3r, s));
-      DR_TRY(op_nt_repack_split3(d->cont_h1, Hd + L, wm->cont.l0.w, Hd + L, w.s3c, s));
-      DR_TRY(op_gemm_nt_split3_sk(M1, d->rew_h1, Hd + L, hiddens, Hd, latents, L, Hd, w.s3r, wm->reward.l0.b, 0,
-                                  w.p1r, d->rew_h1, w.s3part, w.s3part_n, s));
-      DR_TRY(op_gemm_nt_split3_sk(M1, d->cont_h1, Hd + L, hiddens, Hd, latents, L, Hd, w.s3c, wm->cont.l0.b, 0,
-                                  w.p1c, d->cont_h1, w.s3part, w.s3part_n, s));
-    } else {
-      p[0] = lin2(M1, d->rew_h1, hiddens, Hd, Hd, latents, L, L, wm->reward.l0.w, wm->reward.l0.b, w.p1r, d->rew_h1);
-      p[1] = lin2(M1, d->cont_h1, hiddens, Hd, Hd, latents, L, L, wm->cont.l0.w, wm->cont.l0.b, w.p1c, d->cont_h1);
-      DR_TRY(gemm_launch(G_NT, AM_PLAIN, p, 2, s));
-    }
     p[0] = lin_ln(M1, d->buckets, d->rew_h2, w.p2r, d->rew_h2, wm->reward.n4, wm->reward.l6.w, wm->reward.l6.b, w.rlog,
                   d->buckets);
     p[1] = lin_ln(M1, 1, d->cont_h2, w.p2c, d->cont_h2, wm->cont.n4, wm->cont.l6.w, wm->cont.l6.b, w.clog, 1);
@@ -1029,6 +1068,9 @@
 }
 
 
+static int critic_tail(const dr_dims* d, const dr_critic* cr, int M, const CTape& t, float* logits, float* values,
+                       bool tape, hipStream_t s);
+
 extern "C" int dr_critic_fwd(const dr_dims* d, const dr_critic* cr, int M, const float* h, long long ldh,
                              const float* z, long long ldz, float* logits, float* values, void* tape, void* ws,
                              size_t ws_bytes, hipStream_t s) {
@@ -1068,13 +1110,48 @@
   DR_REQUIRE(tape || ws, "dr_critic_fwd needs a tape or a workspace");
   const int L = latent(d), Hd = d->hidden, c1 = d->critic_h1, c2 = d->critic_h2, nb = d->buckets;
   if (s3w && s3_first_layer(d, M, c1, h, ldh, z, ldz)) {
+    const int sp = s3part ? op_s3_heads_splits(M, Hd + L) : 0;
     DR_TRY(op_nt_repack_split3(c1, Hd + L, cr->net.l0.w, Hd + L, s3w, s));
     DR_TRY(op_gemm_nt_split3_sk(M, c1, Hd + L, h, (int)ldh, z, (int)ldz, Hd, s3w, cr->net.l0.b, 0, t.pre1, c1,
-                                s3part, s3part_n, s));
+                                s3part, s3part_n, s, sp));
   } else {
     GemmArgs g1 = lin2(M, c1, h, ldh, Hd, z, ldz, L, cr->net.l0.w, cr->net.l0.b, t.pre1, c1);
     give_splitk(g1, sk, skn);
     DR_TRY(run(G_NT, AM_PLAIN, g1, s));
+  }
+  return critic_tail(d, cr, M, t, logits, values, tape != nullptr, s);
+}
+
+static void critic_tail_args(const dr_dims* d, const dr_critic* cr, int M, const CTape& t, float* logits,
+                             float* values, bool tape, HeadTail& ht) {
+  const int c1 = d->critic_h1, c2 = d->critic_h2, nb = d->buckets;
+  float* lg = logits ? logits : (tape || !values) ? t.logits : nullptr;
+  GemmArgs e = lin_ln(M, nb, c2, nullptr, c2, cr->net.n4, cr->net.l6.w, cr->net.l6.b, lg, nb);
+  memset(&ht, 0, sizeof(HeadTail));
+  ht.a = mlp2(M, c1, c2, t.pre1, c1, cr->net.n1, cr->net.l3, cr->net.n4, e);
+  if (tape) {
+    ht.a.a1_out = t.x1; ht.a.ld_a1 = c1;
+    ht.a.pre2 = t.pre2; ht.a.ld_pre2 = c2;
+    ht.a.a2_out = t.x2; ht.a.ld_a2 = c2;
+  }
+  if (values) {
+    ht.buckets = cr->buckets;
+    ht.val = values;
+  }
+  ht.chain1 = 1;
+}
+
+static int critic_tail(const dr_dims* d, const dr_critic* cr, int M, const CTape& t, float* logits, float* values,
+                       bool tape, hipStream_t s) {
+  const int c1 = d->critic_h1, c2 = d->critic_h2, nb = d->buckets;
+  {
+    HeadTail ht;
+    critic_tail_args(d, cr, M, t, logits, values, tape, ht);
+    if (heads_tail_on(d) && heads_tail_ok(ht)) {
+      DR_TRY(heads_tail_launch(&ht, 1, s));
+      if (tape && logits && logits != t.logits) DR_TRY(copy2d(t.logits, nb, logits, nb, nb, M, s));
+      return DR_OK;
+    }
   }
   GemmArgs g2 = lin_ln(M, c2, c1, t.pre1, c1, cr->net.n1, cr->net.l3.w, cr->net.l3.b, t.pre2, c2);
   g2.a_out = t.x1; g2.ld_aout = c1;
@@ -1086,6 +1163,144 @@
   if (tape && logits && logits != t.logits) DR_TRY(copy2d(t.logits, nb, logits, nb, nb, M, s));
   if (values) DR_TRY(op_bucket_value(M, nb, lg, nb, cr->buckets, values, 1, s));
   return DR_OK;
+}
+
+struct HeadsWs {
+  void* planes;
+  float* part;
+  size_t part_n;
+};
+static void heads_widths(const dr_dims* d, int* wd) {
+  wd[0] = d->rew_h1; wd[1] = d->cont_h1; wd[2] = d->critic_h1; wd[3] = d->critic_h1;
+}
+static void headsws_carve(Carve& c, const dr_dims* d, int M, HeadsWs& w) {
+  int wd[4];
+  heads_widths(d, wd);
+  const int K = d->hidden + latent(d);
+  w.planes = c.raw(op_nt_split3_heads_ws_bytes(wd, 4, K));
+  w.part_n = op_gemm_nt_split3_heads_part_floats(M, wd, 4, K);
+  w.part = c.f((long long)w.part_n);
+}
+static bool heads_shape_ok(const dr_dims* d, int B, int H) {
+  if (!d || B < 1 || H < 1 || d->precision == DR_PREC_BF16) return false;
+  const long long M = (long long)B * (H + 1);
+  const int Hd = d->hidden, L = latent(d);
+  if (M < 1024 || M * std::max(Hd, L) >= (1LL << 31)) return false;
+  int wd[4];
+  heads_widths(d, wd);
+  for (int i = 0; i < 4; ++i)
+    if (wd[i] < 4 || wd[i] % 4) return false;
+  return Hd % 4 == 0 && L % 4 == 0 && d->buckets >= 1 && mlp2_widths_ok(d->rew_h1, d->rew_h2) &&
+         mlp2_widths_ok(d->cont_h1, d->cont_h2);
+}
+extern "C" int dr_heads_supported(const dr_dims* d, int B, int H) { return heads_shape_ok(d, B, H) ? 1 : 0; }
+extern "C" int dr_internal_s3_heads_splits(int M, int K) { return op_s3_heads_splits(M, K); }
+
+extern "C" size_t dr_heads_workspace_bytes(const dr_dims* d, int B, int H) {
+  if (!heads_shape_ok(d, B, H)) return 0;
+  Carve c(nullptr);
+  HeadsWs w;
+  headsws_carve(c, d, B * (H + 1), w);
+  return c.off;
+}
+
+extern "C" int dr_heads_fwd(const dr_dims* d, const dr_world_model* wm, const dr_critic* target,
+                            const dr_critic* online, int B, int H, const float* latents, const float* hiddens,
+                            float* rewards, float* continues, float* V_t, float* V_c, void* ctape, void* ws_im,
+                            size_t ws_im_bytes, void* ws_cr, size_t ws_cr_bytes, void* ws, size_t ws_bytes,
+                            hipStream_t s) {
+  DR_REQUIRE(d && wm && target && online && latents && hiddens && rewards && continues && V_t && V_c && ctape &&
+                 ws_im && ws_cr && ws && B > 0 && H > 0,
+             "null argument or empty batch");
+  if (!heads_shape_ok(d, B, H)) {
+    dr_set_error("dr_heads_fwd: shape outside the grouped heads (fp32 mode, B (H + 1) >= 1024, widths %% 4 == 0)");
+    return DR_E_UNSUPPORTED;
+  }
+  const int M = B * (H + 1), L = latent(d), Hd = d->hidden, c1 = d->critic_h1;
+  Carve ci(ws_im);
+  ImWs w;
+  imws_carve(ci, d, B, H, w);
+  WS_CHECK(ci, ws_im_bytes);
+  CTape tt, to;
+  {
+    Carve c(ws_cr);
+    ctape_carve(c, d, M, tt);
+    WS_CHECK(c, ws_cr_bytes);
+    Carve ct(ctape);
+    ctape_carve(ct, d, M, to);
+  }
+  Carve c(ws);
+  HeadsWs hw;
+  headsws_carve(c, d, M, hw);
+  WS_CHECK(c, ws_bytes);
+  const S3Head heads[4] = {{wm->reward.l0.w, Hd + L, d->rew_h1, wm->reward.l0.b, w.p1r, d->rew_h1},
+                           {wm->cont.l0.w, Hd + L, d->cont_h1, wm->cont.l0.b, w.p1c, d->cont_h1},
+                           {target->net.l0.w, Hd + L, c1, target->net.l0.b, tt.pre1, c1},
+                           {online->net.l0.w, Hd + L, c1, online->net.l0.b, to.pre1, c1}};
+  if (!op_gemm_nt_split3_heads_supported(M, Hd + L, hiddens, Hd, latents, L, Hd, heads, 4)) {
+    dr_set_error("dr_heads_fwd: operands outside the grouped first Linear (alignment)");
+    return DR_E_UNSUPPORTED;
+  }
+  GemmBf16Scope bf16_scope(false);
+  DR_TRY(op_gemm_nt_split3_heads(M, Hd + L, hiddens, Hd, latents, L, Hd, heads, 4, hw.planes, hw.part, hw.part_n, s));
+  {
+    HeadTail ht[4];
+    reward_cont_tails(d, wm, B, H, rewards, continues, w, false, ht);
+    critic_tail_args(d, target, M, tt, nullptr, V_t, false, ht[2]);
+    critic_tail_args(d, online, M, to, nullptr, V_c, true, ht[3]);
+    bool ok = heads_tail_on(d);
+    for (int i = 0; i < 4; ++i) ok = ok && heads_tail_ok(ht[i]);
+    if (ok) return heads_tail_launch(ht, 4, s);
+  }
+  DR_TRY(imagine_heads_tail(d, wm, B, H, rewards, continues, w, s, false));
+  DR_TRY(critic_tail(d, target, M, tt, nullptr, V_t, false, s));
+  return critic_tail(d, online, M, to, nullptr, V_c, true, s);
+}
+
+extern "C" int dr_internal_heads_tail_enable(int on) {
+  const int prev = g_heads_tail ? 1 : 0;
+  g_heads_tail = on != 0;
+  return prev;
+}
+extern "C" int dr_internal_heads_tail_run(int M, int nh, const int* v, void* const* p, int old_path, void* stream,
+                                          char* msg, int msg_cap) {
+  if (msg && msg_cap > 0) msg[0] = 0;
+  if (nh < 1 || nh > DR_HT_HEADS || !v || !p) return DR_E_INVALID;
+  hipStream_t s = (hipStream_t)stream;
+  HeadTail ht[DR_HT_HEADS];
+  memset(ht, 0, sizeof(ht));
+  for (int i = 0; i < nh; ++i) {
+    const int* vi = v + 8 * i;
+    auto P = [&](int k) { return (float*)p[16 * i + k]; };
+    const int K1 = vi[0], K2 = vi[1], N = vi[2];
+    GemmArgs e = gemm_args();
+    e.M = M; e.N = N; e.K = K2;
+    e.W = P(7); e.ldb = K2; e.bias = P(8);
+    e.Y = P(10); e.ldy = N; e.act = vi[3];
+    Mlp2Args& a = ht[i].a;
+    a.M = M; a.K1 = K1; a.K2 = K2;
+    a.X = P(0); a.ldx = K1;
+    a.ln1_g = P(1); a.ln1_b = P(2); a.W3 = P(3); a.b3 = P(4); a.ln4_g = P(5); a.ln4_b = P(6);
+    a.a1_out = P(12); a.ld_a1 = K1; a.pre2 = P(13); a.ld_pre2 = K2; a.a2_out = P(14); a.ld_a2 = K2;
+    a.e = e;
+    ht[i].buckets = P(9);
+    ht[i].val = P(11);
+    ht[i].rm_h1 = vi[4];
+    ht[i].rm_k0 = vi[5];
+    ht[i].chain1 = vi[6];
+  }
+  int rc = DR_OK;
+  if (!old_path) {
+    rc = heads_tail_launch(ht, nh, s);
+  } else {
+    for (int i = 0; i < nh && rc == DR_OK; ++i) {
+      rc = mlp2_launch(&ht[i].a, 1, s);
+      if (rc == DR_OK && ht[i].buckets)
+        rc = op_bucket_value(M, ht[i].a.e.N, ht[i].a.e.Y, ht[i].a.e.N, ht[i].buckets, ht[i].val, 1, s);
+    }
+  }
+  if (rc != DR_OK && msg && msg_cap > 0) snprintf(msg, msg_cap, "%s", dr_last_error());
+  return rc;
 }
 
 struct CBws {
diff --git a/dreamer_amd/csrc/gemm.h b/dreamer_amd/csrc/gemm.h
--- a/dreamer_amd/csrc/gemm.h
+++ b/dreamer_amd/csrc/gemm.h
@@ -96,4 +96,18 @@
   GemmArgs e;
 };
 bool mlp2_ok(const Mlp2Args& a);
+bool mlp2_widths_ok(int K1, int K2);
+
+#define DR_HT_HEADS 4
+#define DR_HT_NMAX 256
+struct alignas(16) HeadTail {
+  Mlp2Args a;
+  const float* buckets;
+  float* val;
+  int rm_h1, rm_k0;
+  int chain1;
+  int pad_;
+};
+bool heads_tail_ok(const HeadTail& h);
+int heads_tail_launch(const HeadTail* heads, int count, hipStream_t s);
 int mlp2_launch(const Mlp2Args* probs, int count, hipStream_t s);
diff --git a/dreamer_amd/csrc/gemm.hip b/dreamer_amd/csrc/gemm.hip
--- a/dreamer_amd/csrc/gemm.hip
+++ b/dreamer_amd/csrc/gemm.hip
@@ -1928,6 +1928,23 @@
   return o;
 }
 
+template <int LP>
+__device__ __forceinline__ f32x4 mlp2_tile1(const float (*ys)[LP], const float4 (&wv)[MLP2_KS], int K, int r, int q) {
+  const int ks = (K + 15) >> 4;
+  f32x4 c = (f32x4){0.f, 0.f, 0.f, 0.f};
+#pragma unroll
+  for (int s = 0; s < MLP2_KS; ++s) {
+    if (s < ks) {
+      const float4 a = *reinterpret_cast<const float4*>(&ys[r][16 * s + 4 * q]);
+      c = __builtin_amdgcn_mfma_f32_16x16x4f32(a.x, wv[s].x, c, 0, 0, 0);
+      c = __builtin_amdgcn_mfma_f32_16x16x4f32(a.y, wv[s].y, c, 0, 0, 0);
+      c = __builtin_amdgcn_mfma_f32_16x16x4f32(a.z, wv[s].z, c, 0, 0, 0);
+      c = __builtin_amdgcn_mfma_f32_16x16x4f32(a.w, wv[s].w, c, 0, 0, 0);
+    }
+  }
+  return c;
+}
+
 __global__ __launch_bounds__(512) void k_mlp2_tail(Mlp2Batch mb) {
   __shared__ Mlp2Args s_a;
   dr_stage_args(mb.p[blockIdx.z], s_a, threadIdx.x);
@@ -2089,6 +2106,9 @@
   }
 }
 
+bool mlp2_widths_ok(int K1, int K2) {
+  return !(K1 < 4 || K2 < 4 || K1 > MLP2_KMAX || K2 > MLP2_KMAX || K1 % 4 || K2 % 4);
+}
 bool mlp2_ok(const Mlp2Args& a) {
   const GemmArgs& g = a.e;
   const bool al = !(((uintptr_t)a.X | (uintptr_t)a.W3 | (uintptr_t)g.W | (uintptr_t)a.ln1_g | (uintptr_t)a.ln1_b |
@@ -2121,6 +2141,182 @@
   }
   hipLaunchKernelGGL(k_mlp2_tail, dim3(gx, gy, count), dim3(512), 0, s, mb);
   return dr_check_launch("mlp2_tail");
+}
+
+#define HT_RG 2
+#define HT_ROWS (16 * HT_RG)
+struct HeadTailBatch {
+  HeadTail p[DR_HT_HEADS];
+};
+
+__device__ __forceinline__ long long ht_row(const HeadTail& h, int m) {
+  if (h.rm_h1 <= 0) return m;
+  const int b = m / h.rm_h1, t = m - b * h.rm_h1;
+  return t < h.rm_k0 ? -1LL : (long long)b * (h.rm_h1 - h.rm_k0) + (t - h.rm_k0);
+}
+
+__global__ __launch_bounds__(512) void k_heads_tail(HeadTailBatch hb) {
+  __shared__ HeadTail s_h;
+  dr_stage_args(hb.p[blockIdx.y], s_h, threadIdx.x);
+  const Mlp2Args& a = s_h.a;
+  const GemmArgs& g = a.e;
+  const int M = dr_uni(a.M), K1 = dr_uni(a.K1), K2 = dr_uni(a.K2), N = dr_uni(g.N);
+  const int m0 = blockIdx.x * HT_ROWS;
+  if (m0 >= M) return;
+  const bool one = dr_uni(s_h.chain1) != 0;
+  const int tid = threadIdx.x, wave = tid >> 6, lane = tid & 63;
+  const int r = lane & 15, q = lane >> 4;
+  constexpr int LP = MLP2_KMAX + 8;
+  constexpr int SP = DR_HT_NMAX + 1;
+  constexpr int HSO = HT_ROWS * (LP > SP ? LP : SP);
+  __shared__ __attribute__((aligned(16))) float ys[HT_ROWS][LP];
+  __shared__ __attribute__((aligned(16))) float hso[HSO];
+  float(*hs)[LP] = reinterpret_cast<float(*)[LP]>(hso);
+  float(*so)[SP] = reinterpret_cast<float(*)[SP]>(hso);
+  const int k = 4 * lane;
+  const float* X = dr_uni(a.X);
+  const int ldx = dr_uni((int)a.ldx);
+  float4 xr[2 * HT_RG];
+#pragma unroll
+  for (int i = 0; i < 2 * HT_RG; ++i) {
+    const int m = m0 + wave + 8 * i;
+    const bool ok = m < M && k < K1;
+    xr[i] = dr_ld4(X, ok ? (unsigned)(m * ldx + k) : 0u);
+  }
+  const int nt3 = (K2 + 15) >> 4;
+  float4 w3[2][MLP2_KS];
+#pragma unroll
+  for (int i = 0; i < 2; ++i) {
+    const int n = (wave + 8 * i) * 16 + r;
+    mlp2_wload(w3[i], a.W3, K1, n, wave + 8 * i < nt3 && n < K2, K1, q);
+  }
+  {
+    const int KP = (K1 + 15) & ~15;
+#pragma unroll
+    for (int i = 0; i < 2 * HT_RG; ++i) {
+      const int rr = wave + 8 * i, m = m0 + rr;
+      const bool ok = m < M && k < K1;
+      const float4 y = mlp2_ln_silu(xr[i], ok, K1, a.ln1_g, a.ln1_b, k);
+      if (k < KP) *reinterpret_cast<float4*>(&ys[rr][k]) = y;
+      if (a.a1_out && ok) dr_st4(a.a1_out, (unsigned)(m * a.ld_a1 + k), y);
+    }
+  }
+  __syncthreads();
+#pragma unroll
+  for (int i = 0; i < 2; ++i) {
+    const int tj = wave + 8 * i;
+    if (tj < nt3) {
+      const int n = tj * 16 + r;
+      const float bv = (n < K2 && a.b3) ? dr_ld1(a.b3, (unsigned)n) : 0.f;
+#pragma unroll
+      for (int rg = 0; rg < HT_RG; ++rg) {
+        const f32x4 acc = one ? mlp2_tile1<LP>(ys + 16 * rg, w3[i], K1, r, q) : mlp2_tile<LP>(ys + 16 * rg, w3[i], K1, r, q);
+#pragma unroll
+        for (int e = 0; e < 4; ++e) {
+          const int ml = 16 * rg + 4 * q + e, m = m0 + ml;
+          const float v = (n < K2) ? acc[e] + bv : 0.f;
+          hs[ml][n] = v;
+          if (a.pre2 && m < M && n < K2) dr_g(a.pre2)[(long long)m * a.ld_pre2 + n] = v;
+        }
+      }
+    }
+  }
+  const int ntd = (N + 15) >> 4;
+  float4 w6[2][MLP2_KS];
+#pragma unroll
+  for (int i = 0; i < 2; ++i) {
+    const int n = (wave + 8 * i) * 16 + r;
+    mlp2_wload(w6[i], dr_uni(g.W), dr_uni((int)g.ldb), n, wave + 8 * i < ntd && n < N, K2, q);
+  }
+  __syncthreads();
+  {
+    const int KP = (K2 + 15) & ~15;
+    for (int rr = wave; rr < HT_ROWS; rr += 8) {
+      const int m = m0 + rr;
+      const bool ok = k < K2;
+      float4 x = ok ? *reinterpret_cast<const float4*>(&hs[rr][k]) : make_float4(0.f, 0.f, 0.f, 0.f);
+      float4 y = mlp2_ln_silu(x, ok, K2, a.ln4_g, a.ln4_b, k);
+      if (m >= M) y = make_float4(0.f, 0.f, 0.f, 0.f);
+      if (k < KP) *reinterpret_cast<float4*>(&ys[rr][k]) = y;
+      if (a.a2_out && ok && m < M) dr_st4(a.a2_out, (unsigned)(m * a.ld_a2 + k), y);
+    }
+  }
+  __syncthreads();
+#pragma unroll
+  for (int i = 0; i < 2; ++i) {
+    const int tj = wave + 8 * i;
+    if (tj < ntd) {
+      const int n = tj * 16 + r;
+      const float bv = (n < N && g.bias) ? dr_ld1(g.bias, (unsigned)n) : 0.f;
+#pragma unroll
+      for (int rg = 0; rg < HT_RG; ++rg) {
+        const f32x4 acc = one ? mlp2_tile1<LP>(ys + 16 * rg, w6[i], K2, r, q) : mlp2_tile<LP>(ys + 16 * rg, w6[i], K2, r, q);
+#pragma unroll
+        for (int e = 0; e < 4; ++e) so[16 * rg + 4 * q + e][n] = acc[e] + bv;
+      }
+    }
+  }
+  __syncthreads();
+  if (g.Y) {
+    for (int x = tid; x < HT_ROWS * N; x += 512) {
+      const int ml = x / N, nl = x - ml * N, m = m0 + ml;
+      if (m >= M) continue;
+      const long long o = ht_row(s_h, m);
+      if (o >= 0) dr_g(g.Y)[o * g.ldy + nl] = epi_act(g, so[ml][nl]);
+    }
+  }
+  if (s_h.buckets) {
+    const float* bk = dr_uni(s_h.buckets);
+    for (int rr = wave; rr < HT_ROWS; rr += 8) {
+      const int m = m0 + rr;
+      if (m >= M) break;
+      const float* l = so[rr];
+      float mx = -INFINITY;
+      for (int c = lane; c < N; c += 64) mx = fmaxf(mx, l[c]);
+      mx = wave_max(mx);
+      float se = 0.f;
+      for (int c = lane; c < N; c += 64) se += expf(l[c] - mx);
+      se = wave_sum(se);
+      float acc = 0.f;
+      for (int c = lane; c < N; c += 64) acc += (expf(l[c] - mx) / se) * dr_g(bk)[c];
+      acc = wave_sum(acc);
+      const long long o = ht_row(s_h, m);
+      if (lane == 0 && o >= 0) dr_g(s_h.val)[o] = dr_symexp(acc);
+    }
+  }
+}
+
+bool heads_tail_ok(const HeadTail& h) {
+  const Mlp2Args& a = h.a;
+  const GemmArgs& g = a.e;
+  const bool al = !(((uintptr_t)a.X | (uintptr_t)a.W3 | (uintptr_t)g.W | (uintptr_t)a.ln1_g | (uintptr_t)a.ln1_b |
+                     (uintptr_t)a.ln4_g | (uintptr_t)a.ln4_b | (uintptr_t)a.a1_out | (uintptr_t)a.a2_out) & 15);
+  return al && mlp2_widths_ok(a.K1, a.K2) && a.M >= 1 && a.X && a.W3 && g.W && a.ln1_g && a.ln1_b && a.ln4_g &&
+         a.ln4_b && a.ldx % 4 == 0 && a.ldx >= a.K1 && (long long)a.M * a.ldx < (1LL << 31) && g.ldb % 4 == 0 &&
+         g.ldb >= a.K2 && a.ld_a1 % 4 == 0 && a.ld_a2 % 4 == 0 && (long long)a.M * a.ld_a1 < (1LL << 31) &&
+         (long long)a.M * a.ld_a2 < (1LL << 31) && g.K == a.K2 && g.N >= 1 && g.N <= DR_HT_NMAX &&
+         g.epi == EPI_NONE && !g.accumulate && !g.addend && g.alpha == 1.0f && (g.Y || h.buckets) &&
+         (!h.buckets || h.val) && h.rm_h1 >= 0 && h.rm_k0 >= 0 && (h.rm_h1 == 0 || h.rm_k0 < h.rm_h1);
+}
+
+int heads_tail_launch(const HeadTail* heads, int count, hipStream_t s) {
+  if (count < 1 || count > DR_HT_HEADS) {
+    dr_set_error("heads_tail_launch: bad head count %d", count);
+    return DR_E_INVALID;
+  }
+  HeadTailBatch hb;
+  int M = 0;
+  for (int i = 0; i < count; ++i) {
+    if (!heads_tail_ok(heads[i])) {
+      const Mlp2Args& a = heads[i].a;
+      dr_set_error("heads_tail_launch: unsupported head %d (M=%d K1=%d K2=%d N=%d)", i, a.M, a.K1, a.K2, a.e.N);
+      return DR_E_INVALID;
+    }
+    hb.p[i] = heads[i];
+    M = std::max(M, heads[i].a.M);
+  }
+  hipLaunchKernelGGL(k_heads_tail, dim3(dr_cdiv(M, HT_ROWS), count), dim3(512), 0, s, hb);
+  return dr_check_launch("heads_tail");
 }
 
 
diff --git a/dreamer_amd/engine.py b/dreamer_amd/engine.py
--- a/dreamer_amd/engine.py
+++ b/dreamer_amd/engine.py
@@ -98,6 +98,10 @@
         self.ctape = torch.zeros(L.query("dr_critic_tape_bytes", d, M), dtype=torch.uint8, device=dev)
         self.ws_cr = hip.workspace(dev).get("e_cr", L.query("dr_critic_workspace_bytes", d, B, H))
         self.ws_cr2 = hip.workspace(dev).get("e_cr2", L.query("dr_critic_workspace_bytes", d, B, H))
+        self.heads_fused = bool(L.query("dr_heads_supported", d, B, H))
+        self.heads_done = False
+        if self.heads_fused:
+            self.ws_heads = hip.workspace(dev).get("e_heads", L.query("dr_heads_workspace_bytes", d, B, H))
         self.rng = hip.rng(dev)
         if self.explorer is not None:
             ex = self.explorer
@@ -130,10 +134,20 @@
             nz = hip.explicit_noise(q=q, eps=eps, device=self.dev)
         else:
             nz = L.dr_noise(None, None, self.rng.state.data_ptr(), self.rank * self.B, DREAM_STREAM)
+        fused = self.heads_fused
         L.call("dr_imagine_fwd", d, self.dr.world_model.packed(), self.dr.agent.actor_struct(), self.B, self.H,
                L.ptr(z0), L.ptr(h0), nz, int(deterministic), L.ptr(self.latents), L.ptr(self.hiddens),
-               L.ptr(self.actions), L.ptr(self.rewards), L.ptr(self.continues), L.ptr(self.mus),
-               L.ptr(self.sigmas), L.ptr(self.tape), L.ptr(self.ws_im), self.ws_im.numel(), hip.stream())
+               L.ptr(self.actions), None if fused else L.ptr(self.rewards), None if fused else L.ptr(self.continues),
+               L.ptr(self.mus), L.ptr(self.sigmas), L.ptr(self.tape), L.ptr(self.ws_im), self.ws_im.numel(),
+               hip.stream())
+        if fused:
+            ag = self.dr.agent
+            L.call("dr_heads_fwd", d, self.dr.world_model.packed(), ag.critic_struct(target=True), ag.critic_struct(),
+                   self.B, self.H, L.ptr(self.latents), L.ptr(self.hiddens), L.ptr(self.rewards),
+                   L.ptr(self.continues), L.ptr(self.V_t), L.ptr(self.V_c), L.ptr(self.ctape), L.ptr(self.ws_im),
+                   self.ws_im.numel(), L.ptr(self.ws_cr), self.ws_cr.numel(), L.ptr(self.ws_heads),
+                   self.ws_heads.numel(), hip.stream())
+        self.heads_done = fused
 
     def returns(self):
         ag, d, st = self.dr.agent, self.d, hip.stream()
@@ -149,8 +163,9 @@
             L.call("dr_state_entropy_fwd", d.hidden, dr.explore_knn, M, L.ptr(self.hiddens), d.hidden, g, M,
                    L.ptr(self.hiddens), d.hidden, g, None, None, None, L.ptr(self.rewards), self.H + 1, 1, self.H, 1,
                    dr.explore_extrinsic, dr.explore_scale, L.ptr(self.ws_knn), self.ws_knn.numel(), st)
-        L.call("dr_critic_fwd", d, ag.critic_struct(target=True), M, L.ptr(self.hiddens), d.hidden,
-               L.ptr(self.latents), L_, None, L.ptr(self.V_t), None, L.ptr(self.ws_cr), self.ws_cr.numel(), st)
+        if not self.heads_done:
+            L.call("dr_critic_fwd", d, ag.critic_struct(target=True), M, L.ptr(self.hiddens), d.hidden,
+                   L.ptr(self.latents), L_, None, L.ptr(self.V_t), None, L.ptr(self.ws_cr), self.ws_cr.numel(), st)
         L.call("dr_lambda_returns", self.B, self.H, L.ptr(self.rewards), L.ptr(self.continues), L.ptr(self.V_t),
                ag.gamma, ag.lambda_, L.ptr(self.R), st)
 
@@ -162,8 +177,9 @@
         M = B * (H + 1)
         L_ = d.rows * d.cols
         scale = 1.0 / float(B * self.wsize * H)
-        L.call("dr_critic_fwd", d, ag.critic_struct(), M, L.ptr(self.hiddens), d.hidden, L.ptr(self.latents), L_,
-               None, L.ptr(self.V_c), L.ptr(self.ctape), L.ptr(self.ws_cr), self.ws_cr.numel(), st)
+        if not self.heads_done:
+            L.call("dr_critic_fwd", d, ag.critic_struct(), M, L.ptr(self.hiddens), d.hidden, L.ptr(self.latents), L_,
+                   None, L.ptr(self.V_c), L.ptr(self.ctape), L.ptr(self.ws_cr), self.ws_cr.numel(), st)
         critic_args = (d, ag.critic_struct(), B, H, L.ptr(self.hiddens), L.ptr(self.latents), L.ptr(self.R),
                        L.ptr(self.ctape), scale, L.ptr(ag.loss_slot(1)), ag.critic_struct(grad=True),
                        L.ptr(self.ws_cr), self.ws_cr.numel())
@@ -186,9 +202,10 @@
     def _x_critic_fwd_and_prep(self):
         ag, d, st = self.dr.agent, self.d, hip.stream()
         M = self.B * (self.H + 1)
-        L.call("dr_critic_fwd", d, ag.critic_struct(), M, L.ptr(self.hiddens), d.hidden, L.ptr(self.latents),
-               d.rows * d.cols, None, L.ptr(self.V_c), L.ptr(self.ctape), L.ptr(self.ws_cr2), self.ws_cr2.numel(),
-               st)
+        if not self.heads_done:
+            L.call("dr_critic_fwd", d, ag.critic_struct(), M, L.ptr(self.hiddens), d.hidden, L.ptr(self.latents),
+                   d.rows * d.cols, None, L.ptr(self.V_c), L.ptr(self.ctape), L.ptr(self.ws_cr2),
+                   self.ws_cr2.numel(), st)
         L.call("dr_imagine_bwd_prep", d, self.dr.world_model.packed(), ag.actor_struct(), self.B, self.H, None,
                None, None, L.ptr(self.ws_im), self.ws_im.numel(), st)
 
@@ -315,8 +332,10 @@
         B, H = self.B, self.H
         M = B * (H + 1)
         scale = 1.0 / float(B * self.wsize * H)
-        L.call("dr_critic_fwd", d, ag.critic_struct(), M, L.ptr(self.hiddens), d.hidden, L.ptr(self.latents),
-               d.rows * d.cols, None, L.ptr(self.V_c), L.ptr(self.ctape), L.ptr(self.ws_cr), self.ws_cr.numel(), st)
+        if not self.heads_done:
+            L.call("dr_critic_fwd", d, ag.critic_struct(), M, L.ptr(self.hiddens), d.hidden, L.ptr(self.latents),
+                   d.rows * d.cols, None, L.ptr(self.V_c), L.ptr(self.ctape), L.ptr(self.ws_cr), self.ws_cr.numel(),
+                   st)
         self._actor_loss()
         L.call("dr_critic_loss_bwd", d, ag.critic_struct(), B, H, L.ptr(self.hiddens), L.ptr(self.latents),
                L.ptr(self.R), L.ptr(self.ctape), scale, L.ptr(ag.loss_slot(1)), ag.critic_struct(grad=True),
diff --git a/include/dreamer_hip.h b/include/dreamer_hip.h
--- a/include/dreamer_hip.h
+++ b/include/dreamer_hip.h
@@ -170,6 +170,12 @@
 int dr_critic_fwd(const dr_dims* d, const dr_critic* c, int M, const float* h, long long ldh, const float* z,
                   long long ldz, float* logits, float* values, void* tape, void* ws, size_t ws_bytes,
                   hipStream_t stream);
+int dr_heads_supported(const dr_dims* d, int B, int H);
+size_t dr_heads_workspace_bytes(const dr_dims* d, int B, int H);
+int dr_heads_fwd(const dr_dims* d, const dr_world_model* wm, const dr_critic* target, const dr_critic* online,
+                 int B, int H, const float* latents, const float* hiddens, float* rewards, float* continues,
+                 float* V_t, float* V_c, void* ctape, void* ws_im, size_t ws_im_bytes, void* ws_cr,
+                 size_t ws_cr_bytes, void* ws, size_t ws_bytes, hipStream_t stream);
 int dr_lambda_returns(int B, int H, const float* r, const float* c, const float* V, float gamma, float lam,
                       float* R, hipStream_t stream);
 int dr_update_S(int n, const float* R, float* S, float* norm_out, void* ws, size_t ws_bytes,
```

New measurement: 640,100 imagined latent-steps/s (median of 6 runs). 1.02x the previous value.
